# chenruduan/OAReactDiff

Hardware: AMD Instinct MI355X
Metric: denoising_steps_per_sec (higher is better)
Workload: dtype f32; 1 GPU; EGNNDynamics.forward (LEFTNet H=196 R=96 L=6), B=64 reactions/GPU x 3 objects x 23 atoms, complete graph per reaction (N=4416, E=300288), T=1000 sampler step shape; batch_per_gpu=64, atoms_per_object=23, parallelism=replica x1 (no collective), launch=eager

## Files before the change

### oareactdiff_amd/_capi.py

```python
from __future__ import annotations

import ctypes as C
import os

from .build import LIB

OARD_MAX_OBJECTS = 8
ABI_VERSION = 2040
OARD_OK, OARD_EINVAL, OARD_ENOTCOMPLETE, OARD_EHIP, OARD_ENOMEM = 0, -1, -2, -3, -4
ERRORS = {OARD_EINVAL: "invalid argument / unsupported configuration", OARD_ENOTCOMPLETE: "topology is not complete-per-sample",
          OARD_EHIP: "HIP runtime error", OARD_ENOMEM: "workspace too small"}

PREC_GCL_BF16X3, PREC_EQUI_BF16X3, PREC_TRAIN_BF16X3 = 1, 2, 4
TAP_S, TAP_VEC, TAP_EDGE, TAP_POS_FRAME, TAP_DPOS, TAP_HOUT, TAP_LABELS, TAP_NE1 = 1, 2, 3, 4, 5, 6, 7, 8

EXPORTS = ["oard_version", "oard_supported", "oard_param_count", "oard_packed_bytes", "oard_pack_weights",
           "oard_topology_create", "oard_topology_destroy", "oard_topology_num_nodes", "oard_topology_num_edges",
           "oard_topology_num_inner_edges", "oard_topology_num_samples", "oard_topology_check_edge_index",
           "oard_workspace_bytes", "oard_forward", "oard_active_inner_edges", "oard_debug_lin3u_table", "oard_sampler_step", "oard_sampler_step_dev", "oard_tap", "oard_debug_stop_after", "oard_debug_option", "oard_timing_enable", "oard_timing_reset",
           "oard_timing_get",
           "oard_topology_create_parts", "oard_topology_export", "oard_tape_bytes", "oard_tape_entry", "oard_forward_train",
           "oard_packed_bwd_bytes", "oard_pack_weights_bwd", "oard_gcl_backward_dx", "oard_edge_node_sums",
           "oard_equi_backward_dx", "oard_scalarize_backward", "oard_equi_msg_backward", "oard_lin3u_forward", "oard_lin3u_backward", "oard_wgrad_scratch_bytes", "oard_wgrad",
           "oard_train_scratch_bytes", "oard_train_scratch_poison", "oard_train_scratch_entry", "oard_train_tail_backward",
           "oard_train_layer_backward", "oard_train_init_backward", "oard_train_stage_backward",
           "oard_loss_prepare", "oard_loss_terms", "oard_adamw_step", "oard_adamw_step_dev", "oard_nan_replace",
           "oard_graph_create", "oard_graph_destroy", "oard_graph_num_nodes", "oard_graph_num_edges", "oard_graph_object_rows",
           "oard_graph_is_complete", "oard_graph_workspace_bytes", "oard_graph_forward", "oard_library_stream"]
STAGE_RECOMPUTE, STAGE_UPDATE, STAGE_MESSAGE, STAGE_GCL_NODE, STAGE_NODE_PRE, STAGE_GCL_EDGE, STAGE_EQUI_EDGE = range(7)
SCRATCH_XH, SCRATCH_XQ, SCRATCH_CR, SCRATCH_DCD, SCRATCH_DCR = range(1, 6)

TOPO_NODE_REF, TOPO_NODE_OBJ, TOPO_NODE_ROW, TOPO_NODE_SAMPLE, TOPO_NODE_TIDX, TOPO_SAMPLE_PTR, TOPO_GROUP_PTR, \
    TOPO_INNER_SRC, TOPO_INNER_TGT, TOPO_ROW_SRC, TOPO_ROW_TGT = range(1, 12)
TAPE_HIN, TAPE_GEO, TAPE_RBF, TAPE_PP0, TAPE_X1 = 1, 2, 3, 4, 5
TAPE_S_IN, TAPE_VEC_IN, TAPE_EW, TAPE_AGG, TAPE_S_MID, TAPE_Z1, TAPE_Z2, TAPE_ATT, TAPE_Z3, TAPE_ZD1, TAPE_CD, TAPE_S_A, TAPE_VEC_A = range(16, 29)


class OardConfig(C.Structure):
    _fields_ = [
        ("hidden", C.c_int32), ("num_radial", C.c_int32), ("num_layers", C.c_int32), ("in_hidden", C.c_int32),
        ("n_obj", C.c_int32), ("node_nf", C.c_int32 * OARD_MAX_OBJECTS), ("enc_alias", C.c_int32 * OARD_MAX_OBJECTS),
        ("condition_nf", C.c_int32), ("condition_time", C.c_int32), ("pos_dim", C.c_int32), ("cutoff", C.c_float),
        ("reflect_equiv", C.c_int32), ("precision", C.c_int32),
    ]


class OardError(RuntimeError):
    pass


def check(rc: int, what: str) -> None:
    if rc != OARD_OK:
        raise OardError(f"{what} failed: {ERRORS.get(rc, rc)}")


def ptr_array(tensors, n=None):
    if tensors is None:
        return None
    ptrs = [None if t is None else t.data_ptr() for t in tensors]
    return (C.c_void_p * (len(ptrs) if n is None else n))(*ptrs)


_lib = None


def lib() -> C.CDLL:
    global _lib
    if _lib is not None:
        return _lib
    if not os.path.exists(LIB):
        raise OardError(f"{LIB} not found: build it with `python -m oareactdiff_amd.build` "
                        "(there is no CPU fallback for the HIP backend)")
    L = C.CDLL(LIB)
    vp, i32, i64, sz = C.c_void_p, C.c_int32, C.c_int64, C.c_size_t
    cfgp = C.POINTER(OardConfig)
    L.oard_version.restype = C.c_int
    got = L.oard_version()
    if got != ABI_VERSION:
        raise OardError(f"{LIB} has ABI version {got}, this package expects {ABI_VERSION}: rebuild it "
                        "(`python -m oareactdiff_amd.build --force`, or the script that made the OARD_LIB build)")
    L.oard_supported.argtypes = [cfgp]; L.oard_supported.restype = C.c_int
    L.oard_param_count.argtypes = [cfgp]; L.oard_param_count.restype = sz
    L.oard_packed_bytes.argtypes = [cfgp]; L.oard_packed_bytes.restype = sz
    L.oard_pack_weights.argtypes = [cfgp, C.POINTER(vp), sz, vp, sz, vp]; L.oard_pack_weights.restype = C.c_int
    L.oard_topology_create.argtypes = [cfgp, C.POINTER(i64), C.POINTER(i64), i64, C.POINTER(vp)]
    L.oard_topology_create.restype = C.c_int
    L.oard_topology_destroy.argtypes = [vp]; L.oard_topology_destroy.restype = None
    for f in ("oard_topology_num_nodes", "oard_topology_num_edges", "oard_topology_num_inner_edges",
              "oard_topology_num_samples"):
        getattr(L, f).argtypes = [vp]; getattr(L, f).restype = i64
    L.oard_topology_check_edge_index.argtypes = [vp, vp, i64, vp, vp]; L.oard_topology_check_edge_index.restype = C.c_int
    L.oard_workspace_bytes.argtypes = [cfgp, vp]; L.oard_workspace_bytes.restype = sz
    L.oard_forward.argtypes = [cfgp, vp, vp, C.POINTER(vp), vp, C.c_int, vp, C.POINTER(vp), vp, sz, vp, vp]
    L.oard_forward.restype = C.c_int
    L.oard_debug_lin3u_table.argtypes = [cfgp, vp, C.c_int, vp, vp]; L.oard_debug_lin3u_table.restype = C.c_int
    L.oard_active_inner_edges.argtypes = [cfgp, vp, vp, sz, C.POINTER(i64), vp]; L.oard_active_inner_edges.restype = C.c_int
    L.oard_sampler_step.argtypes = [cfgp, vp, C.c_int, C.POINTER(vp), C.POINTER(vp), C.POINTER(vp), C.POINTER(vp),
                                    C.c_float, C.c_float, C.c_float, C.c_int, C.POINTER(vp), vp]
    L.oard_sampler_step.restype = C.c_int
    L.oard_sampler_step_dev.argtypes = [cfgp, vp, C.c_int, C.POINTER(vp), C.POINTER(vp), C.POINTER(vp), C.POINTER(vp), vp, C.c_int,
                                        C.POINTER(vp), vp]
    L.oard_sampler_step_dev.restype = C.c_int
    L.oard_tap.argtypes = [cfgp, vp, vp, C.c_int, C.c_int, vp, vp]; L.oard_tap.restype = C.c_int
    ci = C.c_int
    L.oard_topology_create_parts.argtypes = [cfgp, C.POINTER(i64), C.POINTER(i64), i64, ci, C.POINTER(vp)]
    L.oard_topology_create_parts.restype = ci
    L.oard_topology_export.argtypes = [vp, ci, vp, i64, vp]; L.oard_topology_export.restype = ci
    L.oard_tape_bytes.argtypes = [cfgp, vp]; L.oard_tape_bytes.restype = sz
    L.oard_tape_entry.argtypes = [cfgp, vp, ci, ci, C.POINTER(sz), C.POINTER(i64), C.POINTER(i64)]; L.oard_tape_entry.restype = ci
    L.oard_forward_train.argtypes = [cfgp, vp, vp, C.POINTER(vp), vp, ci, vp, C.POINTER(vp), vp, sz, vp, sz, vp, vp]
    L.oard_forward_train.restype = ci
    L.oard_packed_bwd_bytes.argtypes = [cfgp]; L.oard_packed_bwd_bytes.restype = sz
    L.oard_pack_weights_bwd.argtypes = [cfgp, C.POINTER(vp), sz, vp, sz, vp]; L.oard_pack_weights_bwd.restype = ci
    L.oard_gcl_backward_dx.argtypes = [cfgp, vp, vp, ci, vp, vp, vp, vp, vp, vp, vp, vp, vp]; L.oard_gcl_backward_dx.restype = ci
    L.oard_edge_node_sums.argtypes = [cfgp, vp, vp, vp, vp, vp]; L.oard_edge_node_sums.restype = ci
    L.oard_equi_backward_dx.argtypes = [cfgp, vp, vp, ci, vp, vp, vp, vp, vp]; L.oard_equi_backward_dx.restype = ci
    L.oard_scalarize_backward.argtypes = [cfgp, vp, vp, vp, vp, ci, vp, vp, vp, vp]; L.oard_scalarize_backward.restype = ci
    L.oard_equi_msg_backward.argtypes = [cfgp, vp, vp, ci, vp, vp, vp, vp, vp, vp, vp, vp, vp]; L.oard_equi_msg_backward.restype = ci
    L.oard_lin3u_forward.argtypes = [cfgp, vp, ci, vp, i64, vp, vp]; L.oard_lin3u_forward.restype = ci
    L.oard_lin3u_backward.argtypes = [cfgp, vp, ci, vp, vp, i64, vp, vp, vp, vp, vp, vp, vp]; L.oard_lin3u_backward.restype = ci
    L.oard_wgrad_scratch_bytes.argtypes = [ci, ci, i64]; L.oard_wgrad_scratch_bytes.restype = sz
    L.oard_wgrad.argtypes = [vp, ci, ci, ci, ci, ci, vp, ci, ci, ci, ci, ci, ci, i64, vp, vp, vp, sz, vp]; L.oard_wgrad.restype = ci
    pvp = C.POINTER(vp)
    L.oard_train_scratch_bytes.argtypes = [cfgp, vp]; L.oard_train_scratch_bytes.restype = sz
    L.oard_train_scratch_poison.argtypes = [cfgp, vp, vp, sz, vp]; L.oard_train_scratch_poison.restype = ci
    L.oard_train_scratch_entry.argtypes = [cfgp, vp, ci, C.POINTER(sz), C.POINTER(i64), C.POINTER(i64)]; L.oard_train_scratch_entry.restype = ci
    L.oard_train_tail_backward.argtypes = [cfgp, vp, vp, vp, vp, pvp, vp, vp, pvp, pvp, vp, sz, vp]; L.oard_train_tail_backward.restype = ci
    L.oard_train_layer_backward.argtypes = [cfgp, vp, vp, vp, vp, ci, vp, vp, vp, pvp, pvp, vp, sz, vp]; L.oard_train_layer_backward.restype = ci
    L.oard_train_init_backward.argtypes = [cfgp, vp, vp, vp, vp, pvp, vp, vp, pvp, pvp, vp, sz, vp]; L.oard_train_init_backward.restype = ci
    L.oard_train_stage_backward.argtypes = [cfgp, vp, vp, vp, vp, ci, ci, vp, vp, vp, vp, vp, vp, pvp, pvp, vp, sz, vp]
    L.oard_train_stage_backward.restype = ci
    L.oard_nan_replace.argtypes = [cfgp, vp, vp, pvp, pvp, vp]; L.oard_nan_replace.restype = ci
    pf, cf = C.POINTER(C.c_float), C.c_float
    L.oard_loss_prepare.argtypes = [cfgp, vp, pvp, pvp, pvp, pvp, vp, vp, ci, pf, pf, ci, ci, pvp, pvp, vp]; L.oard_loss_prepare.restype = ci
    L.oard_loss_terms.argtypes = [cfgp, vp, pvp, pvp, pvp, pvp, pvp, vp, vp, ci, pf, pf, pf, ci, ci, vp, vp, pvp, vp]; L.oard_loss_terms.restype = ci
    cd = C.c_double
    L.oard_adamw_step.argtypes = [vp, vp, vp, vp, vp, i64, cd, cd, cd, cd, cd, i64, ci, cd, vp]; L.oard_adamw_step.restype = ci
    L.oard_adamw_step_dev.argtypes = [vp, vp, vp, vp, vp, i64, cd, cd, cd, cd, cd, ci, ci, vp, ci, vp, vp, vp, vp]; L.oard_adamw_step_dev.restype = ci
    L.oard_library_stream.argtypes = [ci, pvp]; L.oard_library_stream.restype = ci
    L.oard_graph_create.argtypes = [cfgp, vp, vp, i64, vp, i64, pvp]; L.oard_graph_create.restype = ci
    L.oard_graph_destroy.argtypes = [vp]; L.oard_graph_destroy.restype = None
    L.oard_graph_num_nodes.argtypes = [vp]; L.oard_graph_num_nodes.restype = i64
    L.oard_graph_num_edges.argtypes = [vp]; L.oard_graph_num_edges.restype = i64
    L.oard_graph_object_rows.argtypes = [vp, ci]; L.oard_graph_object_rows.restype = i64
    L.oard_graph_is_complete.argtypes = [vp]; L.oard_graph_is_complete.restype = ci
    L.oard_graph_workspace_bytes.argtypes = [cfgp, vp]; L.oard_graph_workspace_bytes.restype = sz
    L.oard_graph_forward.argtypes = [cfgp, vp, pvp, sz, pvp, vp, ci, vp, pvp, vp, sz, vp, vp]; L.oard_graph_forward.restype = ci
    L.oard_debug_stop_after.argtypes = [C.c_int]; L.oard_debug_stop_after.restype = C.c_int
    L.oard_debug_option.argtypes = [C.c_char_p, C.c_int]; L.oard_debug_option.restype = C.c_int
    L.oard_timing_enable.argtypes = [C.c_int]; L.oard_timing_enable.restype = C.c_int
    L.oard_timing_reset.argtypes = []; L.oard_timing_reset.restype = C.c_int
    L.oard_timing_get.argtypes = [C.c_char_p, C.POINTER(C.c_double), C.POINTER(i64)]; L.oard_timing_get.restype = C.c_int
    for env, opt in (("OARD_GCL_VARIANT", b"gcl_variant"), ("OARD_EQUI_VARIANT", b"equi_variant"),
                     ("OARD_NODE_VARIANT", b"node_variant"), ("OARD_GCL_SKIP", b"gcl_skip"), ("OARD_EQUI_SKIP", b"equi_skip"), ("OARD_EQUI_L0_SKIP", b"equi_l0_skip"), ("OARD_GCL_MSUM", b"gcl_msum"), ("OARD_GCL_PERSIST", b"gcl_persist"), ("OARD_GCL_GRID", b"gcl_grid"), ("OARD_PARTS", b"parts"), ("OARD_SEQUENTIAL", b"sequential"), ("OARD_POISON", b"poison"), ("OARD_AUTO_SMALL", b"auto_small"), ("OARD_AUTO_TINY", b"auto_tiny"), ("OARD_NPB", b"npb"),
                     ("OARD_WGRAD_WGS", b"wgrad_wgs"), ("OARD_WGRAD_LDS", b"wgrad_lds"), ("OARD_WGRAD_T16", b"wgrad_t16"), ("OARD_WGRAD_QUEUE", b"wgrad_queue"), ("OARD_GATE_FOLD", b"gate_fold"), ("OARD_WGRAD_SHAPES", b"wgrad_shapes"), ("OARD_TRAIN_DUAL", b"train_dual"), ("OARD_SMALL_SPLIT", b"small_split"),
                     ("OARD_SKIP_FAMILIES", b"skip_families")):
        if os.environ.get(env) not in (None, ""):
            check(L.oard_debug_option(opt, int(os.environ[env])), f"oard_debug_option({opt.decode()})")
    _lib = L
    return L


def timing_get(family: str):
    ms, n = C.c_double(0.0), C.c_int64(0)
    check(lib().oard_timing_get(family.encode(), C.byref(ms), C.byref(n)), "oard_timing_get")
    return ms.value, n.value
```

### oareactdiff_amd/build.py

```python
from __future__ import annotations

import os
import subprocess
import sys

CSRC = os.path.join(os.path.dirname(os.path.abspath(__file__)), "csrc")
LIB = os.environ.get("OARD_LIB") or os.path.join(CSRC, "liboard_hip.so")
_EDGE = ["oard_engine.h", "oard_layout.h", "oard_kernels.h", "oard_edge_v1.h", "oard_inst.h"]
SOURCES = {
    "oard_hip.hip": None,
    "oard_general.hip": ["oard_general.h"],
    "oard_inst_gcl_p.hip": _EDGE + ["oard_edge_p.h"],
    "oard_inst_gcl_v1.hip": _EDGE + ["oard_node_v1.h", "oard_edge_small.h"],
    "oard_inst_b3.hip": _EDGE + ["oard_edge_b3.h"],
    "oard_inst_equi.hip": _EDGE + ["oard_node_v1.h", "oard_edge_bwd.h"],
    "oard_inst_wgrad.hip": _EDGE + ["oard_edge_bwd.h", "oard_wgrad_t16.h"],
    "oard_inst_node.hip": _EDGE + ["oard_node_v1.h", "oard_edge_bwd.h", "oard_node_bwd.h", "oard_rows.h"],
}
_OWNED = {"oard_general.h"}
_PUBLIC = os.path.join("..", "..", "include", "oard.h")


def _deps(src):
    own = SOURCES[src]
    hdrs = sorted(f for f in os.listdir(CSRC) if f.endswith(".h") and f not in _OWNED) if own is None else list(own)
    return [src] + hdrs + [_PUBLIC]


def _objdir():
    return os.path.join(os.path.dirname(os.path.abspath(LIB)), "build", os.path.basename(LIB))


def _obj(src):
    return os.path.join(_objdir(), os.path.splitext(src)[0] + ".o")


def _newer(paths, than):
    if not os.path.exists(than):
        return True
    t = os.path.getmtime(than)
    return any(os.path.getmtime(os.path.join(CSRC, f)) > t for f in paths)


def _stale() -> bool:
    return any(_newer(_deps(src), LIB) for src in SOURCES)


DEFAULT_DIMS = "196x96,32x8,32x32"


def dims_define(spec: str) -> str:
    pairs = []
    for item in spec.replace(" ", "").split(","):
        if not item:
            continue
        h, r = item.lower().split("x")
        h, r = int(h), int(r)
        if h % 4 or r % 4 or h < 16 or r < 4:
            raise ValueError(f"OARD_DIMS entry {item!r}: widths must be multiples of 4 (hidden >= 16)")
        if (h, r) not in pairs:
            pairs.append((h, r))
    if not pairs:
        raise ValueError("OARD_DIMS is empty")
    return "-DOARD_DIMS_LIST=" + "".join(f"X({h},{r})" for h, r in pairs)


def _dims_file() -> str:
    return LIB + ".dims"


def _built_dims() -> str:
    try:
        with open(_dims_file()) as f:
            return f.read().strip()
    except OSError:
        return ""


def build(force: bool = False, verbose: bool = False) -> str:
    dims = os.environ.get("OARD_DIMS", DEFAULT_DIMS)
    dims_define(dims)
    if not force and not _stale() and _built_dims() == dims:
        return LIB
    hipcc = os.environ.get("HIPCC", "/opt/rocm/bin/hipcc")
    if not os.path.exists(hipcc):
        hipcc = "hipcc"
    os.makedirs(_objdir(), exist_ok=True)
    flags = ["--offload-arch=gfx950", "-O3", "-std=c++17", "-fPIC", "-Wno-unused-result", dims_define(dims)]
    extra = os.environ.get("OARD_CXXFLAGS", "").split()
    tag = os.path.join(_objdir(), "flags.txt")
    flag_line = " ".join(flags + extra)
    try:
        same_flags = open(tag).read() == flag_line
    except OSError:
        same_flags = False
    todo = [src for src in SOURCES if force or not same_flags or _newer(_deps(src), _obj(src))]

    def compile_one(src):
        cmd = [hipcc] + flags + extra + ["-c", src, "-o", _obj(src)]
        if verbose:
            print(" ".join(cmd), file=sys.stderr)
        subprocess.run(cmd, cwd=CSRC, check=True)
    if todo:
        from concurrent.futures import ThreadPoolExecutor
        with ThreadPoolExecutor(max_workers=len(todo)) as pool:
            list(pool.map(compile_one, todo))
        with open(tag, "w") as f:
            f.write(flag_line)
    cmd = [hipcc, "--offload-arch=gfx950", "-shared", "-fPIC"] + [_obj(src) for src in SOURCES] + ["-o", LIB]
    if verbose:
        print(" ".join(cmd), file=sys.stderr)
    subprocess.run(cmd, cwd=CSRC, check=True)
    with open(_dims_file(), "w") as f:
        f.write(dims + "\n")
    return LIB


if __name__ == "__main__":
    print(build(force="--force" in sys.argv, verbose=True))
```

### oareactdiff_amd/csrc/oard_edge_v1.h

```cpp
#pragma once
#include "oard_kernels.h"

typedef __attribute__((address_space(3))) void* lds_ptr_t;
typedef const __attribute__((address_space(1))) void* gbl_ptr_t;
typedef int i4 __attribute__((ext_vector_type(4)));

OARD_DEV void glds16(const float* gsrc_lane, float* lds_chunk);
OARD_DEV void glds16u(const float* chunk_uniform, unsigned lane_byte_off, float* lds_chunk) {
    glds16(reinterpret_cast<const float*>(reinterpret_cast<const char*>(chunk_uniform) + lane_byte_off), lds_chunk);
}
OARD_DEV void glds16(const float* gsrc_lane, float* lds_chunk) {
#ifndef OARD_ABL_NODMA_INSTR
    __builtin_amdgcn_global_load_lds((gbl_ptr_t)gsrc_lane, (lds_ptr_t)lds_chunk, 16, 0, 0);
#else
    asm volatile("" :: "v"(gsrc_lane), "s"(lds_chunk));
#endif
}

OARD_DEV void phase_barrier() {
    asm volatile("s_waitcnt vmcnt(0)" ::: "memory");
#ifndef OARD_ABL_NOBARRIER
    __syncthreads();
#endif
}
// ... 344 lines not shown
    if (TRAIN) {
#pragma unroll
        for (int t = 0; t < HT; ++t) st_blk(tape.z1, e, D::HP, t, lane, h1[t]);
    }
#pragma unroll
    for (int t = 0; t < HT; ++t) h1[t] = silu4(h1[t]);
    const float h1_tail = TAIL1 ? tail_compact(h1[HT - 1], lane) : 0.f;

    f4 m[HT];
    f4 on[GP];
    f4 pz2[TRAIN ? GP : 1];
    float m_tail = 0.f;
#pragma unroll
    for (int p2 = 0; p2 < S::NP2; ++p2, ++p) {
        auto post = [&]() {
            TL(1);
            if (TRAIN && p2 > 0) {
#pragma unroll
                for (int gg = 0; gg < GP; ++gg)
                    if ((p2 - 1) * GP + gg < HT) st_blk(tape.z2, e, D::HP, (p2 - 1) * GP + gg, lane, pz2[gg]);
            }
            pf_begin(p + DIST);
            if (DO_S3 && p2 == S::NP2 - 1) {
#pragma unroll
                for (int gg = 0; gg < GP; ++gg)
                    on[gg] = gg < WB ? (DO_S1 ? ld_edge(erow + 16 * gg) : ld_f4(c0 + 16 * gg + 4 * g)) : f4zero();
            }
        };
        auto hook = [&]() { if (RING == 3 && bar_left > 0 && --bar_left == 0) { PHASE_BARRIER(); post(); } pf.tick(); };
        if (RING == 2) { PHASE_BARRIER(); post(); } else bar_left = BAR_AT;
#pragma unroll
        for (int gg = 0; gg < GP; ++gg) {
            const int tg = p2 * GP + gg;
            if (tg < S::NG2) {
                const f4 bias = A(p, gg * G2);
                TL(2);
                f4 acc;
                if (ROWS4 && tg >= HT - 1) {
                    acc = reduce_g(tg < HT ? chain_tile4<HT>(SL(p), gg * G2 + 1, h1, bias, hook)
                                           : chain_tile4<HT>(SL(p), gg * G2 + 1, m, bias, hook));
                    if (tg < HT && g != 0) acc = f4zero();
                } else {
                    acc = tg < HT ? chain_tile<HT, TAIL1>(SL(p), gg * G2 + 1, h1, bias, h1_tail, hook)
                                  : chain_tile<HT, TAIL1>(SL(p), gg * G2 + 1, m, bias, m_tail, hook);
                }
                TL(3);
                if (tg < HT) {
                    if (TRAIN) pz2[gg] = acc;
                    m[tg] = silu4(acc);
                    if (TAIL1 && tg == HT - 1) m_tail = tail_compact(m[HT - 1], lane);
                } else {
                    const float a = ROWS4 ? acc.x : __shfl(acc.x, lane & 15, 64);
                    if (TRAIN && g == 0) tape.att[e] = a;
                    const float gate = silu1(a);
#pragma unroll
                    for (int t = 0; t < HT; ++t) m[t] *= gate;
                    m_tail *= gate;
                }
            }
        }
        TL(4);
        if (RING == 3 && bar_left > 0) { bar_left = 0; PHASE_BARRIER(); post(); }
        pf.flush();
    }
    if (TRAIN) {
#pragma unroll
        for (int gg = 0; gg < GP; ++gg)
            if ((S::NP2 - 1) * GP + gg < HT) st_blk(tape.z2, e, D::HP, (S::NP2 - 1) * GP + gg, lane, pz2[gg]);
    }
    if (!DO_S3) {
        if (MSUM) st_msum<D>(mbuf, c, key, m, lane);
        else {
#pragma unroll
            for (int t = 0; t < HT; ++t) st_blk(mbuf, eid, D::HP, t, lane, m[t]);
        }
        PROBE_END(pf);
        TL_END();
        return;
    }
    f4 pend[GP], pendz[TRAIN ? GP : 1];
    f4 om[GP];
    auto s3_phase = [&](int p3, const f4 (&o)[GP], f4 (&onext)[GP]) {
        auto post = [&]() {
            TL(1);
            if (p3 == 0) {
                if (!MSUM) {
#pragma unroll
                    for (int t = 0; t < HT; ++t) st_blk(mbuf, eid, D::HP, t, lane, m[t]);
                }
            } else {
#pragma unroll
                for (int gg = 0; gg < GP; ++gg) {
                    st_f4(orow + 16 * ((p3 - 1) * GP + gg), pend[gg]);
                    if (TRAIN) st_f4(tape.z3 + e * D::WP + 4 * g + 16 * ((p3 - 1) * GP + gg), pendz[gg]);
                }
            }
            pf_begin(p + DIST);
            if (p3 + 1 < S::NP3) {
#pragma unroll
                for (int gg = 0; gg < GP; ++gg) {
                    const int t = (p3 + 1) * GP + gg;
                    if (t < WB)
                        onext[gg] = DO_S1 ? ld_edge(erow + 16 * t) : ld_f4(c0 + 16 * t + 4 * g);
                }
            }
        };
        auto hook = [&]() { if (RING == 3 && bar_left > 0 && --bar_left == 0) { PHASE_BARRIER(); post(); } pf.tick(); };
        if (RING == 2) { PHASE_BARRIER(); post(); } else bar_left = BAR_AT;
#pragma unroll
        for (int gg = 0; gg < GP; ++gg) {
            const int t = p3 * GP + gg;
            if (t < WB) {
                TL(2);
                const f4 z = chain_tile<HT, TAIL1>(SL(p), gg * G2 + 1, m, A(p, gg * G2), m_tail, hook);
                TL(3);
                if (TRAIN) pendz[gg] = z;
                pend[gg] = o[gg] + silu4(z);
            }
        }
        TL(4);
        if (RING == 3 && bar_left > 0) { bar_left = 0; PHASE_BARRIER(); post(); }
        if (MSUM && p3 == 0) st_msum<D>(mbuf, c, key, m, lane);
        pf.flush();
        ++p;
    };
    {
        int p3 = 0;
        for (; p3 + 1 < S::NP3; p3 += 2) { s3_phase(p3, on, om); s3_phase(p3 + 1, om, on); }
        if (p3 < S::NP3) s3_phase(p3, on, om);
    }
#pragma unroll
    for (int gg = 0; gg < GP; ++gg) {
        const int t = (S::NP3 - 1) * GP + gg;
        if (t < WB) {
            st_f4(orow + 16 * t, pend[gg]);
            if (TRAIN) st_f4(tape.z3 + e * D::WP + 4 * g + 16 * t, pendz[gg]);
        }
    }
    PROBE_END(pf);
    TL_END();
}

template <class D>
struct EquiStream {
    static constexpr int WB = D::WB, D1T = D::D1T, RB = D::RB, HT = D::HT;
    static constexpr int G1 = D1T, G2 = 1 + D1T + RB, NG2 = 3 * HT;
    static constexpr bool ROWS4 = (D::H % 16) >= 1 && (D::H % 16) <= 4;
    static constexpr int SLAB = G2 > G1 ? G2 : G1;
    static constexpr int NPH = WB + NG2;
    static constexpr int C1 = WB * G1, CHUNKS = C1 + NG2 * G2;
    static constexpr size_t LDS_BYTES = (size_t)2 * SLAB * 1024;
};

template <class D, int WAVES, bool TRAIN>
__global__ __launch_bounds__(WAVES * 64) void k_equi_edge_v1(TopoDev tp, const float* __restrict__ stream,
                                                             const float* __restrict__ dp0b,
                                                             const float* __restrict__ ew, const float* __restrict__ rbuf,
                                                             float* __restrict__ qbuf, float* __restrict__ zd1,
                                                             float* __restrict__ cdbuf, ActList al, int skip_mid) {
    extern __shared__ __attribute__((aligned(16))) float smem[];
    using S = EquiStream<D>;
    constexpr int WB = D::WB, D1T = D::D1T, RB = D::RB, HT = D::HT, G1 = S::G1, G2 = S::G2;
    const int lane = threadIdx.x & 63, g = lane >> 4;
    const int wave = __builtin_amdgcn_readfirstlane(threadIdx.x >> 6);

    SlabPrefetch<WAVES, S::SLAB, 0, 3> pf;
    pf.wave = wave;
    pf.lane_off = (unsigned)lane * 16u;
    const bool skip = !TRAIN && skip_mid != 0;
    auto pf_begin = [&](int ph) {
        pf.begin(stream, smem, ph, ph * G1, G1);
    };
    auto pf_begin_t2 = [&](int ph, int slot) {
        pf.begin(stream, smem, ph, S::C1 + slot * G2, slot < S::NG2 ? G2 : 0);
    };
    auto next_slot = [&](int i) -> int { return i + ((skip && i % 3 == 0) ? 2 : 1); };
    auto hook = [&]() { pf.tick(); };
    auto A = [&](int p, int j) -> f4 {
        return *reinterpret_cast<const f4*>(smem + ((size_t)(p & 1) * S::SLAB + j) * 256 + lane * 4);
    };
    auto SL = [&](int p) -> const float* { return smem + (size_t)(p & 1) * S::SLAB * 256 + lane * 4; };

    const long long n_cols = al.n != nullptr ? (long long)*al.n : tp.A;
    if ((long long)blockIdx.x * WAVES * 16 >= n_cols) return;
    const long long c = ((long long)blockIdx.x * WAVES + wave) * 16 + (lane & 15);
    const bool live = c < n_cols;
    const size_t a = (size_t)(live ? (al.rows != nullptr ? (long long)al.rows[c] : c) : tp.A);
    const float* erow = ew + (live ? a : (size_t)tp.E) * D::WP + 4 * g;
    f4 d1[D1T];
#pragma unroll
    for (int t = 0; t < D1T; ++t) d1[t] = ld_vec(dp0b, t, lane);
    f4 rb[RB];
#pragma unroll
    for (int b = 0; b < RB; ++b) rb[b] = ld_blk(rbuf, a, D::RP, b, lane);
    f4 xn = ld_f4(erow);
    pf_begin(0);
    pf.flush();

    int p = 0;
    for (int b = 0; b < WB; ++b, ++p) {
        phase_barrier();
        const f4 x = xn;
        if (b + 1 < WB) pf_begin(p + 1); else pf_begin_t2(p + 1, 0);
        if (b + 1 < WB) xn = ld_f4(erow + 16 * (b + 1));
        chain_kouter<D1T>(SL(p), 0, x, d1, hook);
        pf.flush();
    }
    if (TRAIN) {
#pragma unroll
        for (int t = 0; t < D1T; ++t) st_blk(zd1, a, D::D1P, t, lane, d1[t]);
    }
#pragma unroll
    for (int t = 0; t < D1T; ++t) d1[t] = silu4(d1[t]);

    float* qrow = qbuf + a * (size_t)(3 * D::HP) + 4 * g;
    float* cdrow = TRAIN ? cdbuf + a * (size_t)(3 * D::HP) + 4 * g : nullptr;
    f4 pend = f4zero(), pendc = f4zero();
    int pend_off = 0;
    auto t2_phase = [&](int i, auto rows4) {
        phase_barrier();
        if (i > 0) {
            st_f4(qrow + pend_off, pend);
            if (TRAIN) st_f4(cdrow + pend_off, pendc);
        }
        pf_begin_t2(p + 1, next_slot(i));
        const int tt = i / 3, th = i - 3 * tt;
        f4 cd, cr;
        if (decltype(rows4)::value) {
            cd = reduce_g(chain_tile4<D1T>(SL(p), 1, d1, A(p, 0), hook));
            cr = reduce_g(chain_tile4<RB>(SL(p), 1 + D1T, rb, f4zero(), hook));
            if (g != 0) { cd = f4zero(); cr = f4zero(); }
        } else {
            cd = chain_tile<D1T>(SL(p), 1, d1, A(p, 0), hook);
            cr = chain_tile<RB>(SL(p), 1 + D1T, rb, f4zero(), hook);
        }
        pf.flush();
        pend = cd * cr;
        if (TRAIN) pendc = cd;
        pend_off = th * D::HP + 16 * tt;
        ++p;
    };
    constexpr int N_FULL = S::ROWS4 ? S::NG2 - 3 : S::NG2;
    for (int i = 0; i < N_FULL; i = next_slot(i)) t2_phase(i, std::false_type{});
    for (int i = N_FULL; i < S::NG2; i = next_slot(i)) t2_phase(i, std::true_type{});
    st_f4(qrow + pend_off, pend);
    if (TRAIN) st_f4(cdrow + pend_off, pendc);
}

template <class D>
__global__ __launch_bounds__(256) void k_equi_agg_v1(TopoDev tp, const float* __restrict__ wb, LayerOff lo,
                                                     const float* __restrict__ qbuf, const float* __restrict__ xq,
                                                     const float* __restrict__ geo, const float* __restrict__ x1,
                                                     float* __restrict__ s, const float* __restrict__ vec_in,
                                                     float* __restrict__ vec_out, float* __restrict__ v2buf,
                                                     float* __restrict__ scal, float* __restrict__ vdot) {
    bool live; const ColId id = col_id(tp.N, live);
    if (!live) return;
    const int n = id.col, a0 = tp.act_ptr[n], cnt = tp.act_ptr[n + 1] - a0;
    const int mx = wave_max(cnt);
    const float inv_sqrt2 = 0.70710678118654752f, inv_sqrt3 = 0.57735026918962576f,
                inv_sqrt_h = 1.0f / sqrtf((float)D::H);
    f4 vx[3][D::HT], dx[D::HT];
#pragma unroll
    for (int t = 0; t < D::HT; ++t) { dx[t] = f4zero(); vx[0][t] = f4zero(); vx[1][t] = f4zero(); vx[2][t] = f4zero(); }
    for (int k = 0; k < mx; ++k)
        if (k < cnt) {
            const size_t a = (size_t)a0 + k;
            const int m = tp.act_src[a];
            const float* g = geo + a * GEO_STRIDE;
            const float ux = g[2], uy = g[3], uz = g[4];
            const float xc = lo.xcross ? 1.0f : 0.0f, cx = xc * g[5], cy = xc * g[6], cz = xc * g[7];
#pragma unroll
            for (int t = 0; t < D::HT; ++t) {
                const f4 q0 = ld_blk(qbuf, a, 3 * D::HP, t, id.lane);
                const f4 q1 = ld_blk(qbuf, a, 3 * D::HP, D::HT + t, id.lane);
                const f4 q2 = ld_blk(qbuf, a, 3 * D::HP, 2 * D::HT + t, id.lane);
                const f4 xs0 = ld_blk(xq, m, 3 * D::HP, t, id.lane) + ld_blk(xq, n, 3 * D::HP, t, id.lane);
                const f4 xs1 = ld_blk(xq, m, 3 * D::HP, D::HT + t, id.lane) + ld_blk(xq, n, 3 * D::HP, D::HT + t, id.lane);
                const f4 xs2 = ld_blk(xq, m, 3 * D::HP, 2 * D::HT + t, id.lane) + ld_blk(xq, n, 3 * D::HP, 2 * D::HT + t, id.lane);
                const f4 xm = xs0 * q0;
                dx[t] += xm;
                const f4 a2 = xs1 * q1 * inv_sqrt3, a3 = xs2 * q2;
                vx[0][t] += (ld_blk(vec_in, (size_t)m * 3 + 0, D::HP, t, id.lane) * a2 + a3 * ux + xm * cx) * inv_sqrt_h;
                vx[1][t] += (ld_blk(vec_in, (size_t)m * 3 + 1, D::HP, t, id.lane) * a2 + a3 * uy + xm * cy) * inv_sqrt_h;
                vx[2][t] += (ld_blk(vec_in, (size_t)m * 3 + 2, D::HP, t, id.lane) * a2 + a3 * uz + xm * cz) * inv_sqrt_h;
            }
        }
#pragma unroll
    for (int t = 0; t < D::HT; ++t) {
        const f4 sn = (ld_blk(s, n, D::HP, t, id.lane) + dx[t]) * inv_sqrt2;
        if (id.valid) st_blk(s, n, D::HP, t, id.lane, sn);
#pragma unroll
        for (int x = 0; x < 3; ++x) {
            vx[x][t] += ld_blk(vec_in, (size_t)n * 3 + x, D::HP, t, id.lane);
            if (id.valid) st_blk(vec_out, (size_t)n * 3 + x, D::HP, t, id.lane, vx[x][t]);
        }
    }
    const float fx = x1[n * 3], fy = x1[n * 3 + 1], fz = x1[n * 3 + 2];
    const float* l3 = wb + lo.l3u;
    for (int t = 0; t < D::HT; ++t) {
        f4 v1[3] = {f4zero(), f4zero(), f4zero()}, v2[3] = {f4zero(), f4zero(), f4zero()};
        const float* w1 = wb + lo.vp + ((size_t)t * D::HT * 64 + id.lane) * 4;
        const float* w2 = wb + lo.vp + ((size_t)(D::HT + t) * D::HT * 64 + id.lane) * 4;
#pragma unroll
        for (int b = 0; b < D::HT; ++b) {
            const f4 c1 = ld_f4(w1 + (size_t)b * 256), c2 = ld_f4(w2 + (size_t)b * 256);
#pragma unroll
            for (int x = 0; x < 3; ++x) {
                v1[x] = mma_chunk(c1, vx[x][b], v1[x]);
                v2[x] = mma_chunk(c2, vx[x][b], v2[x]);
            }
        }
        const f4 sc = v1[0] * fx + v1[1] * fy + v1[2] * fz;
        const f4 vd = (v1[0] * v2[0] + v1[1] * v2[1] + v1[2] * v2[2]) * inv_sqrt_h;
        f4 sca;
        const int f0 = 16 * t + 4 * id.g;
        sca.x = f0 + 0 < D::H ? lin3u(l3, sc.x) : 0.f;
        sca.y = f0 + 1 < D::H ? lin3u(l3, sc.y) : 0.f;
        sca.z = f0 + 2 < D::H ? lin3u(l3, sc.z) : 0.f;
        sca.w = f0 + 3 < D::H ? lin3u(l3, sc.w) : 0.f;
        if (id.valid) {
            st_blk(scal, n, D::HP, t, id.lane, sca);
            st_blk(vdot, n, D::HP, t, id.lane, vd);
            st_blk(v2buf, (size_t)n * 3 + 0, D::HP, t, id.lane, v2[0]);
            st_blk(v2buf, (size_t)n * 3 + 1, D::HP, t, id.lane, v2[1]);
            st_blk(v2buf, (size_t)n * 3 + 2, D::HP, t, id.lane, v2[2]);
        }
    }
}
```

### oareactdiff_amd/csrc/oard_hip.hip

```cpp
#include <algorithm>
#include <cmath>
#include <cstdio>
#include <cstring>
#include <map>
#include <string>
#include <vector>
#include <mutex>
#include <chrono>
#include <utility>

#include "oard_kernels.h"
#include "oard_edge_v1.h"
#include "oard_edge_p.h"
#include "oard_wgrad_t16.h"
#include "oard_edge_b3.h"
#ifdef OARD_EXPERIMENTS
#include "oard_edge_fp.h"
#endif
#include "oard_node_v1.h"
#include "oard_edge_small.h"
#include "oard_edge_bwd.h"
#include "oard_node_bwd.h"
#include "oard_rows.h"
#include "oard_plan.h"
#include "oard_inst.h"

#define OARD_VERSION 2040
#ifdef OARD_EXPERIMENTS
static constexpr bool kV0 = true;
#else
static constexpr bool kV0 = false;
#endif

#define HIP_TRY(x) do { hipError_t e_ = (x); if (e_ != hipSuccess) { \
    fprintf(stderr, "liboard_hip: %s failed: %s (%s:%d)\n", #x, hipGetErrorString(e_), __FILE__, __LINE__); \
    return OARD_EHIP; } } while (0)

namespace {
enum Family { F_GCL_EDGE = 0, F_EQUI_EDGE, F_NODE, F_INIT, F_OTHER, F_GCL_BWD, F_EQUI_BWD, F_WGRAD, F_COUNT };
const char* kFamilyNames[F_COUNT] = {"gcl_edge", "equi_edge", "node", "init", "other", "gcl_edge_bwd", "equi_edge_bwd", "wgrad"};
struct TimingRec { hipEvent_t a, b; int fam; };
struct Timing {
    bool on = false;
    std::vector<TimingRec> recs;
    std::vector<hipEvent_t> pool;
    double total_ms[F_COUNT] = {0};
    long long launches[F_COUNT] = {0};
    hipEvent_t get() {
        if (!pool.empty()) { hipEvent_t e = pool.back(); pool.pop_back(); return e; }
        hipEvent_t e; (void)hipEventCreate(&e); return e;
    }
    void flush() {
        for (auto& r : recs) {
            (void)hipEventSynchronize(r.b);
            float ms = 0.f;
            (void)hipEventElapsedTime(&ms, r.a, r.b);
            total_ms[r.fam] += ms; launches[r.fam] += 1;
            pool.push_back(r.a); pool.push_back(r.b);
        }
        recs.clear();
    }
} g_timing;
int g_stop_after = 0;
FwdOptions g_fwd;
int g_sequential = 0;
int g_npb = 0;
int g_poison = 0;
int g_gcl_msum_taken = 0;
int g_equi_l0_taken = 0;
int g_parts = 0;
int g_wgrad_shapes = 3;
int g_wgrad_t16 = 256;
int g_wgrad_lds = 256;
int g_wgrad_wgs = 512;
int g_skip_families = 0;

struct ScopedLaunch {
    hipStream_t st; hipEvent_t a; int fam; bool on;
    ScopedLaunch(int f, hipStream_t s) : st(s), fam(f), on(g_timing.on) {
        if (on) { a = g_timing.get(); (void)hipEventRecord(a, st); }
    }
    ~ScopedLaunch() {
        if (on) { hipEvent_t b = g_timing.get(); (void)hipEventRecord(b, st); g_timing.recs.push_back({a, b, fam}); }
    }
};
#define LAUNCH(fam, kern, grid, block, stream, ...) do { ScopedLaunch sl_(fam, stream); if (!((g_skip_families >> (fam)) & 1)) \
    hipLaunchKernelGGL(kern, dim3((unsigned)(grid)), dim3(block), 0, stream, __VA_ARGS__); } while (0)
#define LAUNCH2(fam, kern, gx, gy, block, stream, ...) do { ScopedLaunch sl_(fam, stream); if (!((g_skip_families >> (fam)) & 1)) \
    hipLaunchKernelGGL(kern, dim3((unsigned)(gx), (unsigned)(gy)), dim3(block), 0, stream, __VA_ARGS__); } while (0)

#ifndef OARD_DIMS_LIST
#define OARD_DIMS_LIST X(196, 96) X(32, 8) X(32, 32)
#endif

inline size_t align_up(size_t x, size_t a) { return (x + a - 1) / a * a; }
inline long long cdiv(long long a, long long b) { return (a + b - 1) / b; }

bool config_ok(const oard_config* c) {
    if (!c) return false;
    bool dims = false;
#define X(h, r) dims = dims || (c->hidden == (h) && c->num_radial == (r));
    OARD_DIMS_LIST
#undef X
    if (!dims) return false;
    if (c->num_layers < 1 || c->num_layers > OARD_MAX_LAYERS) return false;
    if (c->in_hidden < 1 || c->in_hidden > 16) return false;
    if (c->n_obj < 1 || c->n_obj > OARD_MAX_OBJECTS) return false;
    if (c->pos_dim != 3 || (c->reflect_equiv != 0 && c->reflect_equiv != 1)) return false;
    if (c->precision & ~(OARD_PREC_GCL_BF16X3 | OARD_PREC_EQUI_BF16X3 | OARD_PREC_TRAIN_BF16X3)) return false;
    const int emb = c->in_hidden - (c->condition_time ? 1 : 0) - (c->condition_nf > 0 ? c->condition_nf : 0);
    if (emb < 1) return false;
    for (int k = 0; k < c->n_obj; ++k) {
        const int d = c->node_nf[k] - 3;
        if (d < 1 || d > 16) return false;
        const int a = c->enc_alias[k];
        if (a < 0 || a >= c->n_obj || c->node_nf[a] != c->node_nf[k]) return false;
    }
    return true;
}
int embed_dim(const oard_config* c) {
    return c->in_hidden - (c->condition_time ? 1 : 0) - (c->condition_nf > 0 ? c->condition_nf : 0);
}

PackOff make_layout(const oard_config* c) {
    const RDims d(c->hidden, c->num_radial);
    PackOff po;
    memset(&po, 0, sizeof(po));
    size_t cur = 0;
    auto take = [&](size_t n) { size_t o = cur; cur = align_up(cur + n, 64); return o; };
    auto mat = [&](int MT, int KB) { return take((size_t)MT * KB * 256); };
    const int emb = embed_dim(c);
    po.emb = mat(d.HT, 1); po.emb_b = take(d.HP);
    po.nbemb = mat(d.HT, 1); po.nbemb_b = take(d.HP);
    po.s2v = mat(d.HT, d.HT); po.s2v_b = take(d.HP);
    po.rl0 = mat(d.HT, d.RB); po.rl0_b = take(d.HP);
    po.rl2 = mat(d.HT, d.HT); po.rl2_b = take(d.HP);
    po.lin3 = take((size_t)d.H4 * 5 + 1);
    po.pe0 = take((size_t)d.H2 * 3);
    po.pe1 = mat(d.HT, d.PB);
    po.embout = mat(1, d.HT); po.embout_b = take(16);
    po.v1p = mat(d.HT, d.HT); po.v2p = take(d.HP);
    po.un0 = mat(d.HT, 2 * d.HT); po.un0_b = take(d.HP);
    po.un2 = mat(1, d.HT); po.un2_b = take(16);
    po.c0row = take(d.WP);
    po.u0 = take(d.HP);
    po.rbf_means = take(d.RP); po.rbf_betas = take(d.RP);
    for (int k = 0; k < c->n_obj; ++k) {
        const int dd = c->node_nf[k] - 3;
        po.enc[k] = take((size_t)2 * dd * dd + 2 * dd + (size_t)emb * 2 * dd + emb);
        po.dec[k] = take((size_t)2 * dd * emb + 2 * dd + (size_t)dd * 2 * dd + dd);
    }
    for (int l = 0; l < c->num_layers; ++l) {
        LayerOff& lo = po.layer[l];
        lo.ln_g_w = take(d.HP); lo.ln_g_b = take(d.HP);
        lo.W1a = mat(d.HT, d.HT); lo.b1 = take(d.HP);
        lo.W1b = mat(d.HT, d.HT);
        lo.W1c = mat(d.HT, d.WB);
        lo.W2 = mat(d.HT, d.HT); lo.b2 = take(d.HP);
        lo.watt = take(d.HP); lo.batt = take(1);
        lo.W3 = mat(d.WB, d.HT); lo.b3 = take(d.WP);
        lo.nm0 = mat(d.HT, 2 * d.HT); lo.nm0b = take(d.HP);
        lo.nm1 = mat(d.HT, d.HT); lo.nm1b = take(d.HP);
        lo.ln_q_w = take(d.HP); lo.ln_q_b = take(d.HP);
        lo.xp0 = mat(d.HT, d.HT);
        lo.xp2 = mat(3 * d.HT, d.HT);
        lo.dp0 = mat(d.D1T, d.WB); lo.dp0b = take(d.D1P);
        lo.dp2 = mat(3 * d.HT, d.D1T); lo.dp2b = take(3 * d.HP);
        lo.rbfp = mat(3 * d.HT, d.RB);
        lo.vp = mat(2 * d.HT, d.HT);
        lo.xv0 = mat(d.HT, 2 * d.HT);
        lo.xv2 = mat(3 * d.HT, d.HT);
        lo.l3u = take(593);
        lo.l3t = take(L3T_FLOATS);
        lo.gcl_stream = take((size_t)(d.WB * d.HT + (d.HT + 1) * (d.HT + 1) + d.WB * (d.HT + 1)) * 256);
        lo.equi_stream = take((size_t)(d.WB * d.D1T + 3 * d.HT * (1 + d.D1T + d.RB)) * 256);
        {
            const int nbh = (d.HT + 1) / 2, nbw = (d.WB + 1) / 2;
            lo.gcl_b3 = take((size_t)(nbw * 3 * d.HT + (d.HT + 1) * (1 + 3 * nbh) + d.WB * (1 + 3 * nbh)) * 256);
            lo.equi_b3 = take((size_t)(nbw * 3 * d.D1T + ((d.RB + 1) / 2 + (d.D1T + 1) / 2) * 9 * d.HT) * 256);
        }
    }
    po.total = cur;
    po.signed_scal = c->reflect_equiv ? 0 : 1;
    for (int l = 0; l < c->num_layers; ++l) po.layer[l].xcross = c->reflect_equiv ? 0 : 1;
    return po;
}

struct ParamIdx {
    int emb_w, emb_b, embout_w, embout_b, means, betas, nbemb_w, nbemb_b, s2v_w, s2v_b, rl0_w, rl0_b, rl2_w, rl2_b,
        lin30_w, lin30_b, lin32_w, lin32_b, pe0_w, pe1_w;
    int gcl0, msg0, upd0, out0, enc0, dec0, count;
    explicit ParamIdx(const oard_config* c) {
        int i = 0;
        emb_w = i++; emb_b = i++; embout_w = i++; embout_b = i++; means = i++; betas = i++;
        nbemb_w = i++; nbemb_b = i++; s2v_w = i++; s2v_b = i++; rl0_w = i++; rl0_b = i++; rl2_w = i++; rl2_b = i++;
        lin30_w = i++; lin30_b = i++; lin32_w = i++; lin32_b = i++; pe0_w = i++; pe1_w = i++;
        i += 2;
        gcl0 = i; i += 14 * c->num_layers;
        msg0 = i; i += 9 * c->num_layers;
        upd0 = i; i += 9 * c->num_layers;
        i += 2;
        out0 = i; i += 6;
        enc0 = i; i += 4 * c->n_obj;
        dec0 = i; i += 4 * c->n_obj;
        count = i;
    }
};

struct Packer {
    const float* const* p; float* blob; hipStream_t st;
    std::vector<GenJob> jobs;
    long long blocks = 0;
    void push(GenJob j, size_t work) {
        j.block0 = blocks;
        blocks += cdiv((long long)std::max<size_t>(work, 1), 256);
        jobs.push_back(j);
    }
    void matrix(int src, int src_ld, int col_off, int msl, int msp, int ms, int ksl, int ksp, int ks, int MT, int KB,
                size_t dst, size_t tstride = 0, size_t bstride = 256, int perm_ht = 0, int transpose = 0, int tail_compact = 0,
                int rows4 = 0) {
        if (tstride == 0) tstride = (size_t)KB * 256;
        GenJob j;
        memset(&j, 0, sizeof(j));
        j.type = 0;
        j.m = PackJob{p[src], src_ld, col_off, msl, msp, ms, ksl, ksp, ks, MT, KB, dst, tstride, bstride, perm_ht, transpose, rows4, tail_compact};
        push(j, (size_t)MT * KB * 256);
    }
    void nat(int src, int src_ld, int col_off, int M, int K, int MT, int KB, size_t dst) {
        matrix(src, src_ld, col_off, M, MT * 16, 1, K, KB * 16, 1, MT, KB, dst);
    }
    void vec(int src, int sect_len, int sect_pad, int sects, int n_dst, size_t dst) {
        GenJob j;
        memset(&j, 0, sizeof(j));
        j.type = 1; j.src = src >= 0 ? p[src] : nullptr; j.dst = dst; j.sect_len = sect_len; j.sect_pad = sect_pad; j.sects = sects; j.n = n_dst;
        push(j, (size_t)n_dst);
    }
    void bias_chunks(int src, int sect_len, int sect_pad, int sects, int n_tiles, size_t dst, size_t tstride,
                     int perm_ht = 0) {
        GenJob j;
        memset(&j, 0, sizeof(j));
        j.type = 2; j.src = p[src]; j.dst = dst; j.sect_len = sect_len; j.sect_pad = sect_pad; j.sects = sects; j.n = n_tiles * 256;
        j.tstride = tstride; j.perm_ht = perm_ht;
        push(j, (size_t)n_tiles * 256);
    }
    void raw(int src, int n, size_t dst) {
        GenJob j;
        memset(&j, 0, sizeof(j));
        j.type = 3; j.src = p[src]; j.dst = dst; j.n = n;
        push(j, (size_t)n);
    }
    int flush() {
        if (jobs.empty()) return OARD_OK;
        struct Cached { std::vector<GenJob> host; GenJob* dev = nullptr; size_t cap = 0; };
        static std::mutex mu;
        static std::map<std::pair<const void*, int>, Cached> cache;
        int devid = 0;
        (void)hipGetDevice(&devid);
        const GenJob* table = nullptr;
        {
            std::lock_guard<std::mutex> lk(mu);
            Cached& c = cache[{(const void*)blob, devid}];
            const bool same = c.host.size() == jobs.size() && memcmp(c.host.data(), jobs.data(), jobs.size() * sizeof(GenJob)) == 0;
            if (!same) {
                HIP_TRY(hipStreamSynchronize(st));
                if (c.cap < jobs.size()) {
                    if (c.dev) (void)hipFree(c.dev);
                    HIP_TRY(hipMalloc((void**)&c.dev, jobs.size() * sizeof(GenJob)));
                    c.cap = jobs.size();
                }
                HIP_TRY(hipMemcpy(c.dev, jobs.data(), jobs.size() * sizeof(GenJob), hipMemcpyHostToDevice));
                c.host = jobs;
            }
            table = c.dev;
        }
        hipLaunchKernelGGL(k_pack_all, dim3((unsigned)blocks), dim3(256), 0, st, table, (int)jobs.size(), blob);
        jobs.clear();
        blocks = 0;
        return OARD_OK;
    }
};
#define OARD_SMALL_MAX_EDGES (512 * 16 * 16)
static WsOff make_ws(const oard_config* c, const TopoDev& td) {
    const RDims d(c->hidden, c->num_radial);
    const size_t N = td.N, E = td.E + 1, A = td.A + 1;
    WsOff w;
    size_t cur = 0;
    auto take = [&](size_t bytes) { size_t o = cur; cur = align_up(cur + bytes, 256); return o; };
    w.pos = take(N * 3 * 4); w.pf64 = take(N * 3 * 8); w.pf32 = take(N * 3 * 4); w.x1 = take(N * 3 * 4);
    w.pp0 = take(N * 4); w.labels = take(N * 4); w.hin = take(N * 16 * 4);
    w.zemb = take(N * d.HP * 4); w.nb = take(N * d.HP * 4); w.s = take(N * d.HP * 4); w.s1 = take(N * d.HP * 4);
    w.ne1 = take(N * 3 * d.HP * 4); w.xh = take(N * d.HP * 4); w.P = take(N * d.HP * 4); w.Q = take(N * d.HP * 4);
    w.xq = take(N * 3 * d.HP * 4); w.vec = take(N * 3 * d.HP * 4); w.vec2 = take(N * 3 * d.HP * 4); w.v2buf = take(N * 3 * d.HP * 4);
    w.sc0 = take(N * d.HP * 4); w.vdot = take(N * d.HP * 4);
    w.geo = take(A * GEO_STRIDE * 4); w.d64 = take(A * 8); w.rbuf = take(A * d.RP * 4);
    w.ew = take(E * d.WP * 4); w.mbuf = take(std::max(E, (size_t)(td.CI + td.CX) + 1) * d.HP * 4);
    w.xmsg = take(A * d.HP * 4); w.vmsg = take(A * 3 * d.HP * 4);
    w.dpos = take(N * 3 * 4); w.hout = take(N * 16 * 4);
    w.al_rows = take(A * 4); w.al_src = take(A * 4); w.al_pre = take(A * 4); w.al_cnt = take((size_t)cdiv((long long)td.A, 256) * 4 + 4); w.al_n = take(4);
    w.d1s = take((size_t)cdiv((long long)td.A, 128) * 8 * d.D1T * 1024);
    w.small_a = E <= (size_t)OARD_SMALL_MAX_EDGES ? take(A * d.D1P * 4) : 0;
    w.total = cur;
    return w;
}



template <class K>
int set_lds(K kernel, size_t bytes) {
    HIP_TRY(hipFuncSetAttribute((const void*)kernel, hipFuncAttributeMaxDynamicSharedMemorySize, (int)bytes));
    return OARD_OK;
}

#define LAUNCH_LDS(fam, kern, grid, block, lds, stream, ...) do { \
    static bool attr_done_[64] = {}; \
    int dev_ = 0; (void)hipGetDevice(&dev_); dev_ &= 63; \
    if (!attr_done_[dev_]) { int rc_ = set_lds(kern, lds); if (rc_ != OARD_OK) return rc_; attr_done_[dev_] = true; } \
    ScopedLaunch sl_(fam, stream); if (!((g_skip_families >> (fam)) & 1)) \
    hipLaunchKernelGGL(kern, dim3((unsigned)(grid)), dim3(block), lds, stream, __VA_ARGS__); } while (0)

static int device_cus() {
    static int cus[64] = {};
    int d = 0;
    (void)hipGetDevice(&d);
    d &= 63;
    if (!cus[d]) {
        int n = 0;
        if (hipDeviceGetAttribute(&n, hipDeviceAttributeMultiprocessorCount, d) != hipSuccess || n < 1) { (void)hipGetLastError(); n = 256; }
        cus[d] = n;
    }
    return cus[d];
}
struct GclArgs {
    const TopoDev& tp; const float* wb; const LayerOff& lo;
    const float *stream, *P, *Q, *u0, *c0; float *ew_in, *ew_out, *mbuf;
    GclTape tape; hipStream_t st;
};
template <class D, bool S1, bool S3>
int launch_gcl_v1s(const GclLaunch& L, bool msum, const GclArgs& a) {
    constexpr size_t RING3 = GclStream<D, 2>::LDS_BYTES / 2 * 3;
#define GCL_STREAMED(kern, waves, lds, w_) do { LAUNCH_LDS(F_GCL_EDGE, kern, L.grid, (waves) * 64, lds, a.st, a.tp, w_, a.P, a.Q, a.u0, a.c0, \
                                                           L.r0, L.r1, a.ew_in, a.ew_out, a.mbuf, a.tape); return OARD_OK; } while (0)
    switch ((int)L.shape) {
        case GCL_PERSIST:
            if (msum) GCL_STREAMED((k_gcl_edge_p<D, S1, S3, false, true>), 8, RING3, a.stream);
            GCL_STREAMED((k_gcl_edge_p<D, S1, S3>), 8, RING3, a.stream);
        case GCL_RING3:
            if (msum) GCL_STREAMED((k_gcl_edge_v1<D, 8, 2, S1, S3, false, true, 2, 3>), 8, RING3, a.stream);
            GCL_STREAMED((k_gcl_edge_v1<D, 8, 2, S1, S3, false, false, 2, 3>), 8, RING3, a.stream);
        case GCL_TRAIN_PERSIST: GCL_STREAMED((k_gcl_edge_p<D, S1, S3, true>), 8, RING3, a.stream);
        case GCL_TRAIN_RING3: GCL_STREAMED((k_gcl_edge_v1<D, 8, 2, S1, S3, true, false, 2, 3>), 8, RING3, a.stream);
        case GCL_B3: GCL_STREAMED((k_gcl_edge_b3<D, S1, S3>), 8, (GclB3Stream<D>::LDS_BYTES), a.wb + a.lo.gcl_b3);
        case GCL_TRAIN_B3: GCL_STREAMED((k_gcl_edge_b3<D, S1, S3, true>), 8, (GclB3Stream<D>::LDS_BYTES), a.wb + a.lo.gcl_b3);
        case GCL_W4: GCL_STREAMED((k_gcl_edge_v1<D, 4, 2, S1, S3, false>), 4, (GclStream<D, 2>::LDS_BYTES), a.stream);
        case GCL_SMALL:
            LAUNCH_LDS(F_GCL_EDGE, (k_gcl_edge_small<D, 8, S1, S3>), L.grid, 512, (GclSmall<D>::LDS_BYTES), a.st,
                       a.tp, a.wb, a.lo, a.P, a.Q, a.u0, a.c0, L.r0, L.r1, a.ew_out, a.mbuf);
            return OARD_OK;
#ifdef OARD_EXPERIMENTS
        case GCL_V0: LAUNCH(F_GCL_EDGE, (k_gcl_edge<D>), L.grid, 256, a.st, a.tp, a.wb, a.lo, a.P, a.Q, a.ew_in, a.mbuf); return OARD_OK;
        case GCL_X0 + 7: GCL_STREAMED((k_gcl_edge_v1<D, 8, 2, S1, S3, false>), 8, (GclStream<D, 2>::LDS_BYTES), a.stream);
        case GCL_X0 + 8: GCL_STREAMED((k_gcl_edge_v1<D, 8, 3, S1, S3, false>), 8, (GclStream<D, 3>::LDS_BYTES), a.stream);
        case GCL_X0 + 9: GCL_STREAMED((k_gcl_edge_v1<D, 8, 4, S1, S3, false>), 8, (GclStream<D, 4>::LDS_BYTES), a.stream);
        case GCL_X0 + 4: GCL_STREAMED((k_gcl_edge_fp<D, 8, 2, S1, S3, false>), 8, (GclRing<D, 2, 4>::LDS_BYTES), a.stream);
        case GCL_X0 + 5: GCL_STREAMED((k_gcl_edge_fp<D, 8, 2, S1, S3, false, 3>), 8, (GclRing<D, 2, 3>::LDS_BYTES), a.stream);
        case GCL_X0 + 10: GCL_STREAMED((k_gcl_edge_v1<D, 12, 1, S1, S3, false, false, 3>), 12, (GclStream<D, 1>::LDS_BYTES), a.stream);
        case GCL_X0 + 11: GCL_STREAMED((k_gcl_edge_v1<D, 12, 2, S1, S3, false, false, 3>), 12, (GclStream<D, 2>::LDS_BYTES), a.stream);
        case GCL_X0 + 12: GCL_STREAMED((k_gcl_edge_v1<D, 4, 1, S1, S3, false, false, 3>), 4, (GclStream<D, 1>::LDS_BYTES), a.stream);
#endif
        default: return OARD_EINVAL;
    }
#undef GCL_STREAMED
}
template <class D>
int launch_gcl_v1(const GclLayer& g, bool msum, const GclArgs& a) {
    for (int i = 0; i < g.n; ++i) {
        const GclLaunch& L = g.l[i];
        const int rc = L.s1 ? (L.s3 ? launch_gcl_v1s<D, true, true>(L, msum, a) : launch_gcl_v1s<D, true, false>(L, msum, a))
                            : (L.s3 ? launch_gcl_v1s<D, false, true>(L, msum, a) : launch_gcl_v1s<D, false, false>(L, msum, a));
        if (rc != OARD_OK) return rc;
    }
    return OARD_OK;
}
template <class D>
int launch_equi_v1(const FwdPlan& plan, int l, const TopoDev& tp, const float* wb, const LayerOff& lo, const float* stream, const float* dp0b,
                   const float* ew, const float* rbuf, float* qbuf, float* zd1, float* cd, hipStream_t st, float* d1s, float* small, ActList al) {
    const long long tiles = cdiv(tp.A, 16);
    switch (plan.equi) {
        case EQ_TRAIN_B3:
            LAUNCH_LDS(F_EQUI_EDGE, (k_equi_edge_b3<D, true>), cdiv(tp.A, 16 * 8), 8 * 64, (EquiB3Stream<D>::LDS_BYTES), st, tp, wb + lo.equi_b3,
                       dp0b, wb + lo.dp2b, ew, rbuf, qbuf, d1s, zd1, cd, ActList{});
            return OARD_OK;
        case EQ_TRAIN:
            LAUNCH_LDS(F_EQUI_EDGE, (k_equi_edge_v1<D, 8, true>), cdiv(tp.A, 16 * 8), 8 * 64, (EquiStream<D>::LDS_BYTES), st,
                       tp, stream, dp0b, ew, rbuf, qbuf, zd1, cd, ActList{}, 0);
            return OARD_OK;
        case EQ_SMALL_SPLIT:
            LAUNCH_LDS(F_EQUI_EDGE, (k_equi_small_s1<D, 8>), tiles * cdiv(D::D1T, 8), 512, (size_t)D::WB * 1024, st, tp, wb, lo, ew, small);
            LAUNCH_LDS(F_EQUI_EDGE, (k_equi_small_s2<D, 8>), tiles * cdiv(3 * D::HT, 8), 512, (size_t)(D::D1T + D::RB) * 1024, st,
                       tp, wb, lo, (const float*)small, rbuf, qbuf);
            return OARD_OK;
        case EQ_SMALL:
            LAUNCH_LDS(F_EQUI_EDGE, (k_equi_edge_small<D, 8>), tiles, 512, (EquiSmall<D>::LDS_BYTES), st, tp, wb, lo, ew, rbuf, qbuf);
            return OARD_OK;
        case EQ_B3:
            LAUNCH_LDS(F_EQUI_EDGE, (k_equi_edge_b3<D>), cdiv(tp.A, 16 * 8), 8 * 64, (EquiB3Stream<D>::LDS_BYTES), st, tp, wb + lo.equi_b3,
                       dp0b, wb + lo.dp2b, ew, rbuf, qbuf, d1s, nullptr, nullptr, al);
            return OARD_OK;
        case EQ_W4:
            LAUNCH_LDS(F_EQUI_EDGE, (k_equi_edge_v1<D, 4, false>), cdiv(tp.A, 16 * 4), 4 * 64, (EquiStream<D>::LDS_BYTES), st,
                       tp, stream, dp0b, ew, rbuf, qbuf, nullptr, nullptr, al, 0);
            return OARD_OK;
        case EQ_W8:
            LAUNCH_LDS(F_EQUI_EDGE, (k_equi_edge_v1<D, 8, false>), cdiv(tp.A, 16 * 8), 8 * 64, (EquiStream<D>::LDS_BYTES), st,
                       tp, stream, dp0b, ew, rbuf, qbuf, nullptr, nullptr, al, plan.l0_skip && l == 0 ? 1 : 0);
            return OARD_OK;
        default: return OARD_EINVAL;
    }
}

struct TapeOff {
    size_t hin, geo, rbuf, pp0, x1;
    size_t s_in[OARD_MAX_LAYERS + 1], vec_in[OARD_MAX_LAYERS + 1];
    size_t agg[OARD_MAX_LAYERS], s_mid[OARD_MAX_LAYERS];
    size_t s_a[OARD_MAX_LAYERS], vec_a[OARD_MAX_LAYERS];
    size_t ew[OARD_MAX_LAYERS + 1];
    size_t z1[OARD_MAX_LAYERS], z2[OARD_MAX_LAYERS], att[OARD_MAX_LAYERS], z3[OARD_MAX_LAYERS];
    size_t zd1[OARD_MAX_LAYERS], cd[OARD_MAX_LAYERS];
    size_t total;
};
static TapeOff make_tape(const oard_config* c, const TopoDev& td) {
    const RDims d(c->hidden, c->num_radial);
    const size_t N = td.N, E = td.E + 1, A = td.A + 1;
    TapeOff t;
    memset(&t, 0, sizeof(t));
    size_t cur = 0;
    auto take = [&](size_t bytes) { size_t o = cur; cur = align_up(cur + bytes, 256); return o; };
    t.hin = take(N * 16 * 4); t.geo = take(A * GEO_STRIDE * 4); t.rbuf = take(A * d.RP * 4); t.pp0 = take(N * 4); t.x1 = take(N * 3 * 4);
    for (int l = 0; l <= c->num_layers; ++l) {
        t.s_in[l] = take(N * d.HP * 4); t.vec_in[l] = take(N * 3 * d.HP * 4); t.ew[l] = take(E * d.WP * 4);
        if (l == c->num_layers) break;
        t.agg[l] = take(N * d.HP * 4); t.s_mid[l] = take(N * d.HP * 4);
        t.s_a[l] = take(N * d.HP * 4); t.vec_a[l] = take(N * 3 * d.HP * 4);
        t.z1[l] = take(E * d.HP * 4); t.z2[l] = take(E * d.HP * 4); t.att[l] = take(E * 4); t.z3[l] = take(E * d.WP * 4);
        t.zd1[l] = take(A * d.D1P * 4); t.cd[l] = take(A * 3 * d.HP * 4);
    }
    t.total = cur;
    return t;
}

template <class D>
static int forward_impl(const FwdOptions& opt, const oard_config* c, const TopoPart* topo, const float* wb, const float* const* xh,
                        const float* t, int t_scalar, const float* cond, float* const* out, char* ws, char* tape,
                        int* status, hipStream_t st) {
    const TopoDev& tp = topo->d;
    const PackOff po = make_layout(c);
    const WsOff w = make_ws(c, tp);
    const bool train = tape != nullptr;
    const TapeOff to = train ? make_tape(c, tp) : TapeOff{};
    const int emb = embed_dim(c);
    float* pos = (float*)(ws + w.pos); double* pf64 = (double*)(ws + w.pf64); float* pf32 = (float*)(ws + w.pf32);
    auto slot = [&](size_t ws_off, size_t tape_off) -> float* { return train ? (float*)(tape + tape_off) : (float*)(ws + ws_off); };
    float* x1 = slot(w.x1, to.x1); float* pp0 = slot(w.pp0, to.pp0); int* labels = (int*)(ws + w.labels);
    float* hin = slot(w.hin, to.hin); float* zemb = (float*)(ws + w.zemb); float* nb = (float*)(ws + w.nb);
    float* s = (float*)(ws + w.s); float* s1 = (float*)(ws + w.s1); float* ne1 = (float*)(ws + w.ne1);
    float* xhb = (float*)(ws + w.xh); float* P = (float*)(ws + w.P); float* Q = (float*)(ws + w.Q);
    float* xq = (float*)(ws + w.xq); float* vec = slot(w.vec, to.vec_in[0]); float* v2buf = (float*)(ws + w.v2buf);
    float* scal = (float*)(ws + w.sc0); float* vdot = (float*)(ws + w.vdot);
    float* geo = slot(w.geo, to.geo); double* d64 = (double*)(ws + w.d64); float* rbuf = slot(w.rbuf, to.rbuf);
    float* mbuf = (float*)(ws + w.mbuf); float* xmsg = (float*)(ws + w.xmsg);
    float* vmsg = (float*)(ws + w.vmsg); float* dpos = (float*)(ws + w.dpos); float* hout = (float*)(ws + w.hout);
    auto ew_at = [&](int l) -> float* { return train ? (float*)(tape + to.ew[l]) : (float*)(ws + w.ew); };
    float* ew = ew_at(0);
    auto s_at = [&](int l) -> float* { return train ? (float*)(tape + to.s_in[l]) : s; };
    auto s_mid_at = [&](int l) -> float* { return train ? (float*)(tape + to.s_mid[l]) : s; };

    ObjPtrs op;
    memset(&op, 0, sizeof(op));
    for (int k = 0; k < c->n_obj; ++k) {
        op.xh[k] = xh[k]; op.out[k] = out[k]; op.node_nf[k] = c->node_nf[k]; op.enc[k] = po.enc[k]; op.dec[k] = po.dec[k];
    }
    const long long N = tp.N, E = tp.E, A = tp.A;
    const unsigned gN = (unsigned)cdiv(N, 64), gA = (unsigned)cdiv(A, 64);
    const double cutoff = (double)c->cutoff;
    const FwdPlan plan = make_fwd_plan({opt, c->precision, train, topo->conc, tp.npb, device_cus(), A, E, tp.CI, tp.CX, c->num_layers, w.small_a != 0});
    const bool msum = plan.msum, use_al = plan.use_al, nv1 = plan.node != NODE_V0;
    const int stop_after = train ? 0 : g_stop_after;
    int* al_cnt = (int*)(ws + w.al_cnt);
    const ActList al = use_al ? ActList{(const int*)(ws + w.al_rows), (const int*)(ws + w.al_src), (const int*)(ws + w.al_pre), (const int*)(ws + w.al_n)}
                              : ActList{nullptr, nullptr, nullptr, nullptr};
    if (!use_al) HIP_TRY(hipMemsetAsync(ws + w.al_n, 0xff, sizeof(int), st));
    LAUNCH(F_OTHER, k_prep, cdiv(N, 128), 128, st, tp, op, wb, pos, hin, t, t_scalar, cond,
           c->condition_nf > 0 ? c->condition_nf : 0, c->condition_time, emb);
    LAUNCH(F_INIT, k_geom, tp.n_groups, 64, st, tp, (const float*)pos, cutoff, pf64, pf32, x1, pp0, labels);
    if (plan.fill_edges || stop_after == 1)
        LAUNCH(F_INIT, k_fill_edges, std::min<long long>(cdiv((E - A + 1) * (D::WP / 4), 256), 8192), 256, st,
               wb + po.c0row, ew + (size_t)A * D::WP, E - A + 1, D::WP);
    if (A > 0) {
        LAUNCH(F_INIT, k_edge_geo, cdiv(A, 256), 256, st, tp, (const float*)pos, (const double*)pf64, cutoff, geo, d64, use_al ? al_cnt : nullptr);
        if (use_al) LAUNCH(F_INIT, k_active_list, cdiv(A, 256), 256, st, tp, (const float*)geo, (const int*)al_cnt, (int*)al.rows, (int*)al.src, (int*)al.pre, (int*)al.n);
        LAUNCH(F_INIT, k_rbf, cdiv(A * D::RP, 256), 256, st, tp, (const double*)d64, (const float*)geo,
               wb + po.rbf_means, wb + po.rbf_betas, cutoff, rbuf, ew, D::R, D::RP, D::H, D::WP);
    }
    LAUNCH(F_INIT, (k_node_embed<D>), gN, 256, st, tp, wb, po, (const float*)hin, zemb, nb);
    if (A > 0) LAUNCH(F_INIT, (k_radial_lin<D>), gA, 256, st, tp, wb, po, (const float*)rbuf, (const float*)geo, ew);
    constexpr int NW = D::HT <= 16 ? D::HT : 8;
    const unsigned gNb = (unsigned)cdiv(N, tp.npb);
    if (plan.init_v1) {
        LAUNCH(F_INIT, (k_neighbor_v1<D, NW>), gNb, NW * 64, st, tp, wb, po, (const float*)zemb, (const float*)nb, (const float*)ew, s_at(0), s1);
        LAUNCH(F_INIT, (k_s2v_agg_v1<D, NW>), gNb, NW * 64, st, tp, (const float*)s1, (const float*)ew, (const float*)geo, ne1);
    } else if constexpr (kV0) {
        LAUNCH(F_INIT, (k_neighbor<D>), gN, 256, st, tp, wb, po, (const float*)zemb, (const float*)nb, (const float*)ew, s_at(0), s1);
        LAUNCH(F_INIT, (k_s2v_agg<D>), gN, 256, st, tp, (const float*)s1, (const float*)ew, (const float*)geo, ne1);
    } else return OARD_EINVAL;
    if (A > 0) LAUNCH2(F_INIT, (k_scalarize<D>), gA, (plan.scalarize_tiles ? D::HT : 1), 256, st, tp, wb, po, (const float*)ne1, (const float*)geo, ew);
    HIP_TRY(hipMemsetAsync(vec, 0, (size_t)N * 3 * D::HP * sizeof(float), st));
    if (stop_after == 1) return OARD_OK;

    float* vec2 = (float*)(ws + w.vec2);
    float* vcur = vec;
    float* vnext = vec2;
    g_gcl_msum_taken = msum;
    for (int l = 0; l < c->num_layers; ++l) {
        const LayerOff lo = po.layer[l];
        const unsigned gN16 = (unsigned)cdiv(N, tp.npb);
        float* ew_in = ew_at(l);
        float* ew_out = ew_at(l + 1);
        if (train) vnext = (float*)(tape + to.vec_in[l + 1]);

        if (nv1) LAUNCH(F_NODE, (k_node_pre_v1<D, NW>), gN16, NW * 64, st, tp, wb, po, lo, (const float*)s_at(l), (const float*)pp0, xhb, P, Q);
        else if constexpr (kV0) LAUNCH(F_NODE, (k_node_pre<D>), gN, 256, st, tp, wb, po, lo, (const float*)s, (const float*)pp0, xhb, P, Q);
        else return OARD_EINVAL;
        GclTape gt{};
        if (train) gt = GclTape{(float*)(tape + to.z1[l]), (float*)(tape + to.z2[l]), (float*)(tape + to.att[l]), (float*)(tape + to.z3[l])};
        int rc = launch_gcl_v1<D>(plan.gcl_at(l), msum, GclArgs{tp, wb, lo, wb + lo.gcl_stream, P, Q, wb + po.u0, wb + po.c0row, ew_in, ew_out, mbuf, gt, st});
        if (rc != OARD_OK) return rc;
        const bool rows = plan.node == NODE_ROWS;
        if (nv1 && rows) LAUNCH(F_NODE, (k_gcl_node_v1<D, NW, true>), gN16, NW * 64, st, tp, wb, lo, (const float*)xhb, (const float*)mbuf, s_mid_at(l), xq,
                                train ? (float*)(tape + to.agg[l]) : nullptr);
        else if (nv1 && msum) LAUNCH(F_NODE, (k_gcl_node_v1<D, NW, false, true>), gN16, NW * 64, st, tp, wb, lo, (const float*)xhb, (const float*)mbuf, s_mid_at(l), xq,
                                     (float*)nullptr);
        else if (nv1) LAUNCH(F_NODE, (k_gcl_node_v1<D, NW, false>), gN16, NW * 64, st, tp, wb, lo, (const float*)xhb, (const float*)mbuf, s_mid_at(l), xq,
                             train ? (float*)(tape + to.agg[l]) : nullptr);
        else if constexpr (kV0) LAUNCH(F_NODE, (k_gcl_node<D>), gN, 256, st, tp, wb, lo, (const float*)xhb, (const float*)mbuf, s, xq);
        else return OARD_EINVAL;
        if (stop_after == 100 + 10 * l + 1) { topo->vec_final = (size_t)((char*)vcur - ws); return OARD_OK; }
        if (plan.equi == EQ_V0) {
            if constexpr (kV0) {
                if (A > 0) LAUNCH(F_EQUI_EDGE, (k_equi_edge<D>), gA, 256, st, tp, wb, lo, (const float*)ew_out, (const float*)rbuf,
                                  (const float*)geo, (const float*)xq, (const float*)vcur, xmsg, vmsg);
                LAUNCH(F_NODE, (k_equi_agg<D>), gN, 256, st, tp, wb, lo, (const float*)xmsg, (const float*)vmsg, (const float*)x1,
                       s, vcur, v2buf, scal, vdot);
            } else return OARD_EINVAL;
        } else {
            const bool l0_skip = l == 0 && plan.l0_skip;
            if (l == 0) g_equi_l0_taken = l0_skip;
            if (A > 0) {
                rc = launch_equi_v1<D>(plan, l, tp, wb, lo, wb + lo.equi_stream, wb + lo.dp0b, ew_out, rbuf, vmsg,
                                       train ? (float*)(tape + to.zd1[l]) : nullptr, train ? (float*)(tape + to.cd[l]) : nullptr, st,
                                       (float*)(ws + w.d1s), (float*)(ws + w.small_a), al);
                if (rc != OARD_OK) return rc;
            }
#define EQUI_NODE_V1(D_, ROWS_, XC_) LAUNCH(F_NODE, (k_equi_node_v1<D_, NW, ROWS_, XC_>), gN16, NW * 64, st, tp, wb, lo, (const float*)vmsg, \
                       (const float*)xq, (const float*)geo, (const float*)x1, (const float*)s_mid_at(l), s_at(l + 1), (const float*)vcur, vnext, \
                       train ? (float*)(tape + to.s_a[l]) : nullptr, train ? (float*)(tape + to.vec_a[l]) : nullptr, al)
            if (nv1 && rows) {
                if (lo.xcross) EQUI_NODE_V1(D, true, true); else EQUI_NODE_V1(D, true, false);
            } else if (nv1 && l0_skip) {
                if (lo.xcross) EQUI_NODE_V1(Layer0<D>, false, true); else EQUI_NODE_V1(Layer0<D>, false, false);
            } else if (nv1) {
                if (lo.xcross) EQUI_NODE_V1(D, false, true); else EQUI_NODE_V1(D, false, false);
            } else if constexpr (kV0) {
                LAUNCH(F_NODE, (k_equi_agg_v1<D>), gN, 256, st, tp, wb, lo, (const float*)vmsg, (const float*)xq,
                       (const float*)geo, (const float*)x1, s, (const float*)vcur, vnext, v2buf, scal, vdot);
            } else return OARD_EINVAL;
            std::swap(vcur, vnext);
        }
        if constexpr (kV0) {
            if (!nv1) LAUNCH(F_NODE, (k_equi_upd<D>), gN, 256, st, tp, wb, lo, (const float*)scal, (const float*)vdot,
                             (const float*)v2buf, s, vcur);
        }
        if (stop_after == 100 + 10 * l + 2) { topo->vec_final = (size_t)((char*)vcur - ws); return OARD_OK; }
    }
    if (!train) topo->vec_final = (size_t)((char*)vcur - ws);
    if (train) {
        ZeroRows z;
        z.count = 0;
        auto add = [&](size_t off, size_t row, int ld) {
            if (z.count == 64) { LAUNCH(F_OTHER, k_zero_rows, 64, 256, st, z); z.count = 0; }
            z.p[z.count] = (float*)(tape + off) + row * (size_t)ld; z.n[z.count] = ld; ++z.count;
        };
        for (int l = 0; l <= c->num_layers; ++l) {
            add(to.ew[l], (size_t)E, D::WP);
            if (l == c->num_layers) break;
            add(to.z1[l], (size_t)E, D::HP); add(to.z2[l], (size_t)E, D::HP); add(to.att[l], (size_t)E, 1); add(to.z3[l], (size_t)E, D::WP);
            add(to.zd1[l], (size_t)A, D::D1P); add(to.cd[l], (size_t)A, 3 * D::HP);
        }
        add(to.geo, (size_t)A, GEO_STRIDE); add(to.rbuf, (size_t)A, D::RP);
        if (z.count > 0) LAUNCH(F_OTHER, k_zero_rows, z.count, 256, st, z);
    }
    if (plan.init_v1)
        LAUNCH(F_NODE, (k_out_v1<D, NW>), gNb, NW * 64, st, tp, wb, po, (const float*)s_at(c->num_layers), (const float*)vcur, dpos, hout, status);
    else if constexpr (kV0)
        LAUNCH(F_NODE, (k_out<D>), gN, 256, st, tp, wb, po, (const float*)s, (const float*)vcur, dpos, hout, status);
    else return OARD_EINVAL;
    LAUNCH(F_OTHER, k_post, cdiv(N, 128), 128, st, tp, op, wb, (const float*)dpos, (const float*)hout, emb);
    HIP_TRY(hipGetLastError());
    return OARD_OK;
}

template <class F> static int dispatch_dims(const oard_config* c, F&& f) {
#define X(h, r) if (c->hidden == (h) && c->num_radial == (r)) { f(Dims<(h), (r)>{}); return 0; }
    OARD_DIMS_LIST
#undef X
    return OARD_EINVAL;
}
#define DISPATCH_DIMS(c, CALL)                                                                         \
    do {                                                                                               \
        if (dispatch_dims((c), [&](auto d_) { using D = decltype(d_); CALL; }) != 0) return OARD_EINVAL; \
    } while (0)

struct BwdLayerOff { size_t gcl, equi, watt; };
struct BwdOff { BwdLayerOff layer[OARD_MAX_LAYERS]; size_t total; };
static BwdOff make_bwd_layout(const oard_config* c) {
    const RDims d(c->hidden, c->num_radial);
    BwdOff b;
    memset(&b, 0, sizeof(b));
    size_t cur = 0;
    auto take = [&](size_t n) { size_t o = cur; cur = align_up(cur + n, 64); return o; };
    for (int l = 0; l < c->num_layers; ++l) {
        b.layer[l].gcl = take((size_t)(2 * d.WB * d.HT + d.HT * d.HT) * 256);
        b.layer[l].equi = take((size_t)(3 * d.HT * d.D1T + d.WB * d.D1T) * 256);
        b.layer[l].watt = take(d.HP);
    }
    b.total = cur;
    return b;
}
template <class D>
static int gcl_backward_impl(const oard_config* c, const TopoDev& tp, const float* pb, const BwdLayerOff& bl, int layer,
                             const char* tape, const TapeOff& to, const float* dagg, float* dew, float* dz3, float* mout,
                             float* dz2, float* da, float* dz1, hipStream_t st, float* gate_part = nullptr, long long* gate_rows = nullptr) {
    GclBwdArgs a;
    a.gate_part = gate_part;
    a.z1 = (const float*)(tape + to.z1[layer]); a.z2 = (const float*)(tape + to.z2[layer]);
    a.att = (const float*)(tape + to.att[layer]); a.z3 = (const float*)(tape + to.z3[layer]);
    a.dagg = dagg; a.watt = pb + bl.watt; a.dew = dew; a.dz3 = dz3; a.mout = mout; a.dz2 = dz2; a.da = da; a.dz1 = dz1;
    const float* stream = pb + bl.gcl;
    const bool last = layer == c->num_layers - 1;
    const long long r_full = last ? tp.A : tp.E;
    long long rows = 0;
    if (r_full > 0) {
        LAUNCH_LDS(F_GCL_BWD, (k_gcl_edge_bwd<D, 8, 2, true>), cdiv(r_full, 128), 512, (GclBwdStream<D, 2>::LDS_BYTES), st,
                   tp, stream, 0LL, r_full, a);
        rows += cdiv(r_full, 128) * 8;
    }
    if (last && tp.E > tp.A) {
        if (a.gate_part) a.gate_part += (size_t)rows * D::HP;
        LAUNCH_LDS(F_GCL_BWD, (k_gcl_edge_bwd<D, 8, 2, false>), cdiv(tp.E - tp.A, 128), 512, (GclBwdStream<D, 2>::LDS_BYTES), st,
                   tp, stream, tp.A, tp.E, a);
        rows += cdiv(tp.E - tp.A, 128) * 8;
    }
    if (gate_rows) *gate_rows = rows;
    HIP_TRY(hipGetLastError());
    return OARD_OK;
}

template <class D>
static int equi_backward_impl(const TopoDev& tp, const float* stream, const float* dcd, const float* zd1, float* dew,
                              float* dzd1, hipStream_t st) {
    LAUNCH_LDS(F_EQUI_BWD, (k_equi_edge_bwd<D, 8>), cdiv(tp.A, 128), 512, (EquiBwdStream<D>::LDS_BYTES), st, tp, stream, dcd,
               zd1, dew, dzd1);
    HIP_TRY(hipGetLastError());
    return OARD_OK;
}

#ifndef OARD_SCAL_BWD_WAVES
#define OARD_SCAL_BWD_WAVES 2
#endif
template <class D>
static int scalarize_backward_impl(const oard_config* c, const TopoDev& tp, const float* wb, const char* tape, const TapeOff& to,
                                   const float* ne1, int ld, const float* dew, float* dne1, float* part, hipStream_t st) {
    const PackOff po = make_layout(c);
    constexpr int NW = OARD_SCAL_BWD_WAVES;
    if (po.signed_scal)
        LAUNCH(F_INIT, (k_scalarize_bwd<D, NW, true>), tp.N, NW * 64, st, tp, wb + po.lin3, ne1, ld, (const float*)(tape + to.geo), dew, dne1, part);
    else
        LAUNCH(F_INIT, (k_scalarize_bwd<D, NW, false>), tp.N, NW * 64, st, tp, wb + po.lin3, ne1, ld, (const float*)(tape + to.geo), dew, dne1, part);
    HIP_TRY(hipGetLastError());
    return OARD_OK;
}

template <class D>
static int equi_msg_backward_impl(const oard_config* c, const TopoDev& tp, const char* tape, const TapeOff& to, int layer, const float* xq, const float* cr,
                                  const float* gs, const float* gv, float* dcd, float* dcr, float* dxq, float* dvec, hipStream_t st) {
    const Strided3 xq3{xq, 3 * D::H, D::H}, vec3{(const float*)(tape + to.vec_in[layer]), 3 * D::HP, D::HP}, cr3{cr, 3 * D::H, D::H},
        gv3{gv, 3 * D::H, D::H};
    LAUNCH(F_NODE, (k_equi_msg_bwd<D>), tp.N, 256, st, tp, (const float*)(tape + to.geo), xq3, vec3, (const float*)(tape + to.cd[layer]), cr3,
           gs, D::H, gv3, dcd, dcr, dxq, dvec, D::H, c->reflect_equiv ? 0 : 1);
    HIP_TRY(hipGetLastError());
    return OARD_OK;
}

struct WgradPlan { int transposed, NT, nPB, nQG, PP, QP, gy; long long rpc; int n_chunks; int lds, PBW, QGW; };
struct WglShape { int NT, PBW, QGW; };
static const WglShape kWglShapes[2] = {{7, 4, 2}, {8, 4, 2}};
static WgradPlan wgrad_plan(int ncY, int ncX, long long rows) {
    WgradPlan p;
    p.transposed = ncX > ncY ? 1 : 0;
    const int ncP = p.transposed ? ncX : ncY, ncQ = p.transposed ? ncY : ncX;
    const int nQT = (int)cdiv(ncQ, 16);
    p.NT = (cdiv(nQT, 7) * 7 <= cdiv(nQT, 8) * 8) ? 7 : 8;
    p.nPB = (int)cdiv(ncP, 64); p.nQG = (int)cdiv(nQT, p.NT);
    p.PP = p.nPB * 64; p.QP = p.nQG * p.NT * 16;
// ... 232 lines not shown
}

struct TablePool {
    struct Free { void* p; size_t cap; };
    struct Pending { void* p; size_t cap; hipEvent_t ev[4]; int n_ev; int kind; };
    std::mutex m;
    std::vector<Free> free_[2];
    std::vector<Pending> pending;
    std::vector<hipEvent_t> spare_events;
};
static TablePool& table_pool() {
    static TablePool pools[64];
    int d = 0;
    (void)hipGetDevice(&d);
    return pools[d & 63];
}
static void pool_raw_free(void* p, int kind) { if (kind == 0) (void)hipFree(p); else (void)hipHostFree(p); }
static void pool_collect(TablePool& tp) {
    for (size_t i = 0; i < tp.pending.size();) {
        TablePool::Pending& q = tp.pending[i];
        bool done = true;
        for (int k = 0; k < q.n_ev && done; ++k) done = hipEventQuery(q.ev[k]) == hipSuccess;
        if (!done) { ++i; continue; }
        for (int k = 0; k < q.n_ev; ++k) tp.spare_events.push_back(q.ev[k]);
        tp.free_[q.kind].push_back({q.p, q.cap});
        tp.pending[i] = tp.pending.back();
        tp.pending.pop_back();
    }
    (void)hipGetLastError();
}
static void* pool_alloc(size_t bytes, size_t* cap, int kind = 0) {
    TablePool& tp = table_pool();
    std::lock_guard<std::mutex> lk(tp.m);
    pool_collect(tp);
    std::vector<TablePool::Free>& fl = tp.free_[kind];
    int best = -1;
    for (int i = 0; i < (int)fl.size(); ++i)
        if (fl[i].cap >= bytes && fl[i].cap <= 2 * bytes + (1u << 20) && (best < 0 || fl[i].cap < fl[best].cap)) best = i;
    if (best >= 0) {
        void* p = fl[best].p;
        *cap = fl[best].cap;
        fl[best] = fl.back();
        fl.pop_back();
        return p;
    }
    while (fl.size() > 16) {
        pool_raw_free(fl.front().p, kind);
        fl.erase(fl.begin());
    }
    void* p = nullptr;
    *cap = align_up(bytes + bytes / 8, (size_t)1 << 16);
    const hipError_t e = kind == 0 ? hipMalloc(&p, *cap) : hipHostMalloc(&p, *cap, hipHostMallocDefault);
    if (e != hipSuccess) { (void)hipGetLastError(); return nullptr; }
    return p;
}
static void pool_release(void* p, size_t cap, const hipStream_t* streams, int n_streams, bool sync_device, int kind = 0) {
    if (!p) return;
    TablePool& tp = table_pool();
    std::lock_guard<std::mutex> lk(tp.m);
    if (sync_device) { (void)hipDeviceSynchronize(); tp.free_[kind].push_back({p, cap}); return; }
    TablePool::Pending q{p, cap, {}, 0, kind};
    hipStream_t all[5] = {device_streams()[2]};
    int n = 1;
    for (int k = 0; k < n_streams && k < 4; ++k) if (streams[k] != all[0]) all[n++] = streams[k];
    for (int k = 0; k < n && q.n_ev < 4; ++k) {
        hipEvent_t e = nullptr;
        if (!tp.spare_events.empty()) { e = tp.spare_events.back(); tp.spare_events.pop_back(); }
        else if (hipEventCreateWithFlags(&e, hipEventDisableTiming) != hipSuccess) { (void)hipDeviceSynchronize(); tp.free_[kind].push_back({p, cap}); return; }
        (void)hipEventRecord(e, all[k]);
        q.ev[q.n_ev++] = e;
    }
    if (n > 4) { (void)hipDeviceSynchronize(); }
    tp.pending.push_back(q);
}
struct UploadItem { const void* src; size_t bytes; size_t off; };
static int pool_upload(void* dev, const std::vector<UploadItem>& items, size_t total, void** stage_out, size_t* stage_cap) {
    char* stage = (char*)pool_alloc(total, stage_cap, 1);
    if (!stage) return OARD_EHIP;
    for (const UploadItem& it : items) memcpy(stage + it.off, it.src, it.bytes);
    if (hipMemcpyAsync(dev, stage, total, hipMemcpyHostToDevice, device_streams()[2]) != hipSuccess) {
        (void)hipGetLastError();
        pool_release(stage, *stage_cap, nullptr, 0, true, 1);
        return OARD_EHIP;
    }
    *stage_out = stage;
    return OARD_OK;
}
static void topo_touch(const oard_topology* tp, hipStream_t st) {
    if (!tp) return;
    for (int i = 0; i < tp->n_used; ++i) if (tp->used_on[i] == st) return;
    if (tp->ready) (void)hipStreamWaitEvent(st, tp->ready, 0);
    if (tp->n_used < 4) tp->used_on[tp->n_used++] = st; else tp->used_many = true;
}

static int build_part(const oard_config* c, const int64_t* cm, const int64_t* nfs, int N_all, const std::vector<int>& obj_start,
                      const std::vector<int>& dense, const std::vector<long long>& ref_ptr_ref, int lo, int hi,
                      TopoPart& part, int& max_group, int& max_ns) {
    const int n_obj = c->n_obj, B = hi - lo;
    std::vector<int> order;
    for (int i = 0; i < N_all; ++i) if (dense[i] >= lo && dense[i] < hi) order.push_back(i);
    std::stable_sort(order.begin(), order.end(), [&](int a, int b) {
        if (dense[a] != dense[b]) return dense[a] < dense[b];
        return nfs[a] < nfs[b];
    });
    const int N = (int)order.size();
    if (N < 1) return OARD_EINVAL;
    std::vector<int> node_obj(N), node_row(N), node_ref(N), node_tidx(N), node_sample(N), sample_ptr(B + 1, 0),
        grp_ptr((size_t)B * n_obj + 1, 0), edge_ptr(N), act_ptr(N + 1, 0);
    for (int n = 0; n < N; ++n) {
        const int r = order[n], sb = dense[r] - lo;
        node_ref[n] = r; node_obj[n] = (int)nfs[r]; node_row[n] = r - obj_start[nfs[r]];
        node_tidx[n] = (int)cm[r]; node_sample[n] = sb;
        sample_ptr[sb + 1]++;
        grp_ptr[(size_t)sb * n_obj + nfs[r] + 1]++;
    }
    for (int b = 0; b < B; ++b) sample_ptr[b + 1] += sample_ptr[b];
    for (size_t q = 0; q < (size_t)B * n_obj; ++q) grp_ptr[q + 1] += grp_ptr[q];
    long long E = 0, A = 0;
    for (int b = 0; b < B; ++b) {
        const long long ns = sample_ptr[b + 1] - sample_ptr[b];
        max_ns = std::max(max_ns, (int)ns);
        for (int n = sample_ptr[b]; n < sample_ptr[b + 1]; ++n) { edge_ptr[n] = (int)E; E += ns - 1; }
        if (E > 0x7fffffffLL) return OARD_EINVAL;
    }
    for (size_t q = 0; q < (size_t)B * n_obj; ++q) {
        const long long ng = grp_ptr[q + 1] - grp_ptr[q];
        max_group = std::max(max_group, (int)ng);
        A += ng * (ng - 1);
    }
    if (max_group > OARD_MAX_GROUP || A > 0x7fffffffLL) return OARD_EINVAL;
    std::vector<int> edge_src((size_t)E + 1, 0), edge_tgt((size_t)E + 1, 0);
    for (int b = 0; b < B; ++b) {
        const int s0 = sample_ptr[b], s1 = sample_ptr[b + 1];
        for (int n = s0; n < s1; ++n) {
            size_t e = (size_t)edge_ptr[n];
            for (int m = s0; m < s1; ++m) if (m != n) { edge_src[e] = n; edge_tgt[e] = m; ++e; }
        }
    }
    std::vector<int> act_src((size_t)A + 1, 0), act_tgt((size_t)A + 1, 0), act_edge((size_t)A + 1, (int)E);
    {
        size_t a = 0;
        for (int n = 0; n < N; ++n) {
            const int q = node_sample[n] * n_obj + node_obj[n];
            const int g0 = grp_ptr[q], g1 = grp_ptr[q + 1], s0 = sample_ptr[node_sample[n]];
            act_ptr[n] = (int)a;
            for (int m = g0; m < g1; ++m) if (m != n) {
                act_src[a] = m; act_tgt[a] = n;
                act_edge[a] = edge_ptr[m] + (n - s0) - (n > m ? 1 : 0);
                ++a;
            }
        }
        act_ptr[N] = (int)a;
    }
    std::vector<int> edge_row((size_t)std::max<long long>(E, 1), -1), row_src((size_t)E + 1, 0), row_tgt((size_t)E + 1, 0),
        row_eid((size_t)E + 1, (int)E);
    {
        for (long long a = 0; a < A; ++a) {
            edge_row[act_edge[a]] = (int)a; row_src[a] = act_src[a]; row_tgt[a] = act_tgt[a]; row_eid[a] = act_edge[a];
        }
        long long r = A;
        for (long long e = 0; e < E; ++e)
            if (edge_row[e] < 0) { edge_row[e] = (int)r; row_src[r] = edge_src[e]; row_tgt[r] = edge_tgt[e]; row_eid[r] = (int)e; ++r; }
    }
    std::vector<long long> ref_edge_ptr(N);
    for (int n = 0; n < N; ++n) ref_edge_ptr[n] = ref_ptr_ref[node_ref[n]];
    std::vector<int> col_row, col_info, node_cols((size_t)N * 4, 0);
    long long CI = 0, CX = 0;
    {
        auto pad16 = [&]() { while (col_row.size() % 16) col_row.push_back((int)E); };
        for (int b = 0; b < B; ++b) {
            for (int n = sample_ptr[b]; n < sample_ptr[b + 1]; ++n) {
                const int q = node_sample[n] * n_obj + node_obj[n];
                const int g0 = grp_ptr[q], g1 = grp_ptr[q + 1];
                node_cols[4 * (size_t)n + 0] = (int)col_row.size();
                for (int m = g0; m < g1; ++m) if (m != n) col_row.push_back(act_ptr[m] + (n - g0) - (n > m ? 1 : 0));
                node_cols[4 * (size_t)n + 1] = (int)col_row.size();
            }
            pad16();
        }
        CI = (long long)col_row.size();
        for (int b = 0; b < B; ++b) {
            const int ns = sample_ptr[b + 1] - sample_ptr[b];
            for (int n = sample_ptr[b]; n < sample_ptr[b + 1]; ++n) {
                node_cols[4 * (size_t)n + 2] = (int)col_row.size();
                for (long long e = edge_ptr[n]; e < (long long)edge_ptr[n] + ns - 1; ++e) if (edge_row[e] >= A) col_row.push_back(edge_row[e]);
                node_cols[4 * (size_t)n + 3] = (int)col_row.size();
            }
            pad16();
        }
        CX = (long long)col_row.size() - CI;
        if (CI + CX > 0x7fffffffLL - 256) return OARD_EINVAL;
        if (col_row.empty()) col_row.push_back((int)E);
        col_info.resize(col_row.size() * 4);
        for (size_t k = 0; k < col_row.size(); ++k) {
            const int r = col_row[k];
            col_info[4 * k] = r; col_info[4 * k + 1] = row_src[r]; col_info[4 * k + 2] = row_tgt[r];
            col_info[4 * k + 3] = r == (int)E ? -1 : row_src[r] + 1;
        }
    }

    std::vector<UploadItem> items;
    size_t cur = 0;
    auto add = [&](const void* p, size_t bytes) { UploadItem it{p, bytes, cur}; cur = align_up(cur + bytes, 256); items.push_back(it); return it.off; };
    const size_t o_obj = add(node_obj.data(), N * 4), o_row = add(node_row.data(), N * 4), o_ref = add(node_ref.data(), N * 4),
                 o_tidx = add(node_tidx.data(), N * 4), o_smp = add(node_sample.data(), N * 4),
                 o_sptr = add(sample_ptr.data(), (B + 1) * 4), o_eptr = add(edge_ptr.data(), N * 4),
                 o_esrc = add(edge_src.data(), edge_src.size() * 4), o_etgt = add(edge_tgt.data(), edge_tgt.size() * 4),
                 o_gptr = add(grp_ptr.data(), grp_ptr.size() * 4), o_aptr = add(act_ptr.data(), (N + 1) * 4),
                 o_asrc = add(act_src.data(), act_src.size() * 4), o_atgt = add(act_tgt.data(), act_tgt.size() * 4),
                 o_aedge = add(act_edge.data(), act_edge.size() * 4), o_rptr = add(ref_edge_ptr.data(), N * 8),
                 o_erow = add(edge_row.data(), edge_row.size() * 4), o_rsrc = add(row_src.data(), row_src.size() * 4),
                 o_rtgt = add(row_tgt.data(), row_tgt.size() * 4), o_reid = add(row_eid.data(), row_eid.size() * 4),
                 o_crow = add(col_info.data(), col_info.size() * 4), o_ncol = add(node_cols.data(), node_cols.size() * 4);
    size_t cap = 0;
    char* dev = (char*)pool_alloc(cur, &cap);
    if (!dev) return OARD_EHIP;
    if (int rc = pool_upload(dev, items, cur, &part.stage, &part.stage_cap)) { pool_release(dev, cap, nullptr, 0, false); return rc; }
    part.dev_cap = cap;
    part.dev_block = dev;
    TopoDev& d = part.d;
    d.N = N; d.B = B; d.n_obj = n_obj; d.n_groups = B * n_obj; d.E = E; d.A = A;
    d.node_obj = (const int*)(dev + o_obj); d.node_row = (const int*)(dev + o_row); d.node_ref = (const int*)(dev + o_ref);
    d.node_tidx = (const int*)(dev + o_tidx); d.node_sample = (const int*)(dev + o_smp); d.sample_ptr = (const int*)(dev + o_sptr);
    d.edge_ptr = (const int*)(dev + o_eptr); d.edge_src = (const int*)(dev + o_esrc); d.edge_tgt = (const int*)(dev + o_etgt);
    d.grp_ptr = (const int*)(dev + o_gptr); d.act_ptr = (const int*)(dev + o_aptr); d.act_src = (const int*)(dev + o_asrc);
    d.act_tgt = (const int*)(dev + o_atgt); d.act_edge = (const int*)(dev + o_aedge);
    d.ref_edge_ptr = (const long long*)(dev + o_rptr);
    d.edge_row = (const int*)(dev + o_erow); d.row_src = (const int*)(dev + o_rsrc); d.row_tgt = (const int*)(dev + o_rtgt);
    d.row_eid = (const int*)(dev + o_reid);
    d.CI = CI; d.CX = CX; d.col_info = (const int*)(dev + o_crow); d.node_cols = (const int*)(dev + o_ncol);
    return OARD_OK;
}

int oard_topology_create(const oard_config* c, const int64_t* cm, const int64_t* nfs, int64_t n_nodes,
                         oard_topology** out) {
    return oard_topology_create_parts(c, cm, nfs, n_nodes, g_parts, out);
}

int oard_topology_create_parts(const oard_config* c, const int64_t* cm, const int64_t* nfs, int64_t n_nodes,
                               int parts, oard_topology** out) {
    if (!config_ok(c) || !cm || !nfs || !out || n_nodes < 1 || n_nodes > (1 << 24)) return OARD_EINVAL;
    const int N = (int)n_nodes, n_obj = c->n_obj;
    std::vector<int> obj_start(n_obj + 1, 0);
    for (int i = 0; i < N; ++i) {
        if (nfs[i] < 0 || nfs[i] >= n_obj) return OARD_EINVAL;
        if (i > 0 && nfs[i] < nfs[i - 1]) return OARD_EINVAL;
        obj_start[nfs[i] + 1]++;
    }
    for (int k = 0; k < n_obj; ++k) obj_start[k + 1] += obj_start[k];
    std::vector<int64_t> samples(cm, cm + N);
    std::sort(samples.begin(), samples.end());
    samples.erase(std::unique(samples.begin(), samples.end()), samples.end());
    const int B = (int)samples.size();
    if (samples.front() < 0 || samples.back() > (1 << 30)) return OARD_EINVAL;
    std::vector<int> dense(N), ns_of(B, 0);
    for (int i = 0; i < N; ++i) {
        dense[i] = (int)(std::lower_bound(samples.begin(), samples.end(), cm[i]) - samples.begin());
        ns_of[dense[i]]++;
    }
    std::vector<long long> ref_ptr_ref(N);
    long long E_all = 0;
    for (int r = 0; r < N; ++r) { ref_ptr_ref[r] = E_all; E_all += ns_of[dense[r]] - 1; }

    int n_parts = parts > 0 ? parts : (B >= 32 ? 4 : (B >= 16 ? 2 : 1));
    n_parts = std::max(1, std::min(std::min(n_parts, OARD_MAX_PARTS), B));
    oard_topology* tp = new oard_topology();
    (void)hipGetDevice(&tp->device);
    tp->n_obj = n_obj; tp->B = B; tp->n_parts = n_parts;
    {
        std::vector<int> tab(2 * (size_t)N), seen(B, 0);
        for (int r = 0; r < N; ++r) { tab[r] = dense[r]; tab[(size_t)N + r] = seen[dense[r]]++; }
        const size_t b_int = 2 * (size_t)N * sizeof(int), b_all = align_up(b_int, 8) + (size_t)N * sizeof(long long);
        tp->ref_block = pool_alloc(b_all, &tp->ref_cap);
        if (!tp->ref_block) { delete tp; return OARD_EHIP; }
        const std::vector<UploadItem> ref_items = {{tab.data(), b_int, 0}, {ref_ptr_ref.data(), (size_t)N * sizeof(long long), align_up(b_int, 8)}};
        if (int rc = pool_upload(tp->ref_block, ref_items, b_all, &tp->ref_stage, &tp->ref_stage_cap)) { oard_topology_destroy(tp); return rc; }
        tp->ref_sample = (const int*)tp->ref_block; tp->ref_rank = tp->ref_sample + N;
        tp->ref_ptr = (const long long*)((char*)tp->ref_block + align_up(b_int, 8));
        tp->N_ref = N;
    }
    for (int k = 0; k <= n_obj && k <= OARD_MAX_OBJECTS; ++k) tp->obj_start[k] = obj_start[k];
    for (int p = 0; p < n_parts; ++p) {
        const int lo = (int)((long long)B * p / n_parts), hi = (int)((long long)B * (p + 1) / n_parts);
        int rc = build_part(c, cm, nfs, N, obj_start, dense, ref_ptr_ref, lo, hi, tp->parts[p], tp->max_group, tp->max_ns);
        if (rc != OARD_OK) { oard_topology_destroy(tp); return rc; }
        tp->N += tp->parts[p].d.N; tp->E += tp->parts[p].d.E; tp->A += tp->parts[p].d.A;
        tp->parts[p].conc = n_parts;
    }
    {
        const int npb = g_npb > 0 ? g_npb : (int)std::max<long long>(1, std::min<long long>(16, cdiv(tp->N, 256)));
        for (int p = 0; p < n_parts; ++p) tp->parts[p].d.npb = npb;
    }
    if (n_parts > 1) {
        HIP_TRY(hipEventCreateWithFlags(&tp->ev_fork, hipEventDisableTiming));
        for (int p = 1; p < n_parts; ++p) {
            tp->side[p] = device_streams()[(p - 1) % 3];
            if (!tp->side[p]) { oard_topology_destroy(tp); return OARD_EHIP; }
            HIP_TRY(hipEventCreateWithFlags(&tp->ev_join[p], hipEventDisableTiming));
        }
    }
    HIP_TRY(hipEventCreateWithFlags(&tp->ready, hipEventDisableTiming));
    HIP_TRY(hipEventRecord(tp->ready, device_streams()[2]));
    *out = tp;
    return OARD_OK;
}

void oard_topology_destroy(oard_topology* tp) {
    if (!tp) return;
    int cur = tp->device;
    (void)hipGetDevice(&cur);
    if (cur != tp->device) (void)hipSetDevice(tp->device);
    struct Restore { int cur, dev; ~Restore() { if (cur != dev) (void)hipSetDevice(cur); } } restore_{cur, tp->device};
    for (int p = 0; p < OARD_MAX_PARTS; ++p) {
        pool_release(tp->parts[p].dev_block, tp->parts[p].dev_cap, tp->used_on, tp->n_used, tp->used_many);
        pool_release(tp->parts[p].stage, tp->parts[p].stage_cap, nullptr, 0, false, 1);
        if (tp->ev_join[p]) (void)hipEventDestroy(tp->ev_join[p]);
    }
    if (tp->ev_fork) (void)hipEventDestroy(tp->ev_fork);
    pool_release(tp->ref_block, tp->ref_cap, tp->used_on, tp->n_used, tp->used_many);
    pool_release(tp->ref_stage, tp->ref_stage_cap, nullptr, 0, false, 1);
    if (tp->ready) (void)hipEventDestroy(tp->ready);
    delete tp;
}
int64_t oard_topology_num_nodes(const oard_topology* tp) { return tp ? tp->N : 0; }
int64_t oard_topology_num_edges(const oard_topology* tp) { return tp ? tp->E : 0; }
int64_t oard_topology_num_inner_edges(const oard_topology* tp) { return tp ? tp->A : 0; }
int64_t oard_topology_num_samples(const oard_topology* tp) { return tp ? tp->B : 0; }

int oard_topology_check_edge_index(const oard_topology* tp, const int64_t* ei, int64_t n_edges, int32_t* ok,
                                   oard_stream_t stream) {
    topo_touch(tp, (hipStream_t)stream);
    if (!tp || !ok) return OARD_EINVAL;
    hipStream_t st = (hipStream_t)stream;
    const int one = (n_edges == tp->E) ? 1 : 0;
    HIP_TRY(hipMemcpyAsync(ok, &one, sizeof(int), hipMemcpyHostToDevice, st));
    HIP_TRY(hipStreamSynchronize(st));
    if (one && tp->E > 0) {
        if (!ei) return OARD_EINVAL;
        unsigned* bitmap = nullptr;
        const size_t words = (size_t)cdiv(tp->E, 32);
        HIP_TRY(hipMalloc(&bitmap, words * sizeof(unsigned)));
        hipError_t e1 = hipMemsetAsync(bitmap, 0, words * sizeof(unsigned), st);
        if (e1 == hipSuccess) {
            hipLaunchKernelGGL(k_check_edge_set, dim3((unsigned)cdiv(n_edges, 256)), dim3(256), 0, st, tp->ref_sample, tp->ref_rank,
                               tp->ref_ptr, tp->N_ref, (const long long*)ei, (long long)n_edges, bitmap, (int*)ok);
            e1 = hipGetLastError();
        }
        const hipError_t e2 = hipStreamSynchronize(st);
        (void)hipFree(bitmap);
        HIP_TRY(e1);
        HIP_TRY(e2);
    }
    return OARD_OK;
}

static size_t ws_total(const oard_config* c, const oard_topology* tp) {
    size_t cur = 0;
    for (int p = 0; p < tp->n_parts; ++p) {
        const_cast<TopoPart&>(tp->parts[p]).ws_off = cur;
        cur = align_up(cur + make_ws(c, tp->parts[p].d).total, 4096);
    }
    return cur;
}
size_t oard_workspace_bytes(const oard_config* c, const oard_topology* tp) {
    if (!config_ok(c) || !tp) return 0;
    return ws_total(c, tp);
}

int oard_debug_lin3u_table(const oard_config* c, const void* packed, int layer, float* out, oard_stream_t stream) {
    static_assert(OARD_L3T_FLOATS == L3T_FLOATS, "include/oard.h and csrc/oard_layout.h disagree on the table size");
    if (!config_ok(c) || !packed || !out || layer < 0 || layer >= c->num_layers) return OARD_EINVAL;
    const PackOff po = make_layout(c);
    HIP_TRY(hipMemcpyAsync(out, (const float*)packed + po.layer[layer].l3t, (size_t)L3T_FLOATS * sizeof(float), hipMemcpyDeviceToDevice,
                           (hipStream_t)stream));
    return OARD_OK;
}

int oard_active_inner_edges(const oard_config* c, const oard_topology* topo, const void* ws, size_t ws_bytes, int64_t* n_active,
                            oard_stream_t stream) {
    if (!config_ok(c) || !topo || !ws || !n_active) return OARD_EINVAL;
    if (ws_bytes < ws_total(c, topo)) return OARD_ENOMEM;
    hipStream_t st = (hipStream_t)stream;
    long long total = 0;
// ... 647 lines not shown
}

int oard_nan_replace(const oard_config* c, const oard_topology* topo, const int32_t* status, const float* const* noise,
                     float* const* out, oard_stream_t stream) {
    topo_touch(topo, (hipStream_t)stream);
    if (!config_ok(c) || !topo || !status || !noise || !out || c->n_obj != topo->n_obj) return OARD_EINVAL;
    NanPtrs np;
    memset(&np, 0, sizeof(np));
    for (int k = 0; k < c->n_obj; ++k) { np.noise[k] = noise[k]; np.out[k] = out[k]; np.node_nf[k] = c->node_nf[k]; }
    for (int p = 0; p < topo->n_parts; ++p)
        LAUNCH(F_OTHER, k_nan_replace, cdiv(topo->parts[p].d.N, 128), 128, (hipStream_t)stream, topo->parts[p].d, np, (const int*)status);
    HIP_TRY(hipGetLastError());
    return OARD_OK;
}

static LossCfg make_loss_cfg(const oard_config* c, const float* norm_values, const float* norm_biases, const float* scales, int pos_only,
                             int fixed_mask, int T) {
    LossCfg lc;
    memset(&lc, 0, sizeof(lc));
    for (int i = 0; i < 3; ++i) { lc.norm_value[i] = norm_values ? norm_values[i] : 1.0f; lc.norm_bias[i] = norm_biases ? norm_biases[i] : 0.0f; }
    for (int k = 0; k < c->n_obj; ++k) lc.scale[k] = scales ? scales[k] : 1.0f;
    lc.pos_only = pos_only; lc.fixed_mask = fixed_mask; lc.T = T;
    return lc;
}
int oard_loss_prepare(const oard_config* c, const oard_topology* topo, const float* const* pos, const int64_t* const* one_hot,
                      const int64_t* const* charge, const float* const* noise, const float* t_int, const float* gamma, int T,
                      const float* norm_values, const float* norm_biases, int pos_only, int fixed_mask, float* const* z,
                      float* const* eps, oard_stream_t stream) {
    topo_touch(topo, (hipStream_t)stream);
    if (!config_ok(c) || !topo || topo->n_parts != 1 || !pos || !one_hot || !charge || !noise || !t_int || !gamma || !z || !eps)
        return OARD_EINVAL;
    LossPtrs lp;
    memset(&lp, 0, sizeof(lp));
    for (int k = 0; k < c->n_obj; ++k) {
        if (c->node_nf[k] < 5 || c->node_nf[k] - 4 > 16) return OARD_EINVAL;
        lp.pos[k] = pos[k]; lp.one_hot[k] = (const long long*)one_hot[k]; lp.charge[k] = (const long long*)charge[k];
        lp.noise[k] = noise[k]; lp.z[k] = z[k]; lp.eps[k] = eps[k]; lp.node_nf[k] = c->node_nf[k];
    }
    const TopoDev& tp = topo->parts[0].d;
    LAUNCH(F_OTHER, k_loss_prep, cdiv(tp.N, 128), 128, (hipStream_t)stream, tp, lp,
           make_loss_cfg(c, norm_values, norm_biases, nullptr, pos_only, fixed_mask, T), t_int, gamma);
    HIP_TRY(hipGetLastError());
    return OARD_OK;
}
int oard_loss_terms(const oard_config* c, const oard_topology* topo, const float* const* eps, const float* const* net,
                    const float* const* z, const int64_t* const* one_hot, const int64_t* const* charge, const float* t_int,
                    const float* gamma, int T, const float* norm_values, const float* norm_biases, const float* scales, int pos_only,
                    int B, float* nll, float* terms, float* const* dnet, oard_stream_t stream) {
    topo_touch(topo, (hipStream_t)stream);
    if (!config_ok(c) || !topo || topo->n_parts != 1 || !eps || !net || !z || !one_hot || !charge || !t_int || !gamma || !nll || !terms ||
        !dnet || B < 1)
        return OARD_EINVAL;
    LossPtrs lp;
    memset(&lp, 0, sizeof(lp));
    for (int k = 0; k < c->n_obj; ++k) {
        if (c->node_nf[k] < 5 || c->node_nf[k] - 4 > 16) return OARD_EINVAL;
        lp.eps[k] = (float*)eps[k]; lp.net[k] = net[k]; lp.z[k] = (float*)z[k]; lp.one_hot[k] = (const long long*)one_hot[k];
        lp.charge[k] = (const long long*)charge[k]; lp.dnet[k] = dnet[k]; lp.node_nf[k] = c->node_nf[k];
    }
    const TopoDev& tp = topo->parts[0].d;
    LAUNCH(F_OTHER, k_loss_terms, tp.B, 64, (hipStream_t)stream, tp, lp, make_loss_cfg(c, norm_values, norm_biases, scales, pos_only, 0, T),
           t_int, gamma, B, nll, terms);
    HIP_TRY(hipGetLastError());
    return OARD_OK;
}
int oard_adamw_step(float* param, const float* grad, float* exp_avg, float* exp_avg_sq, float* max_exp_avg_sq, int64_t n, double lr,
                    double beta1, double beta2, double eps, double weight_decay, int64_t step, int amsgrad, double grad_scale,
                    oard_stream_t stream) {
    if (!param || !grad || !exp_avg || !exp_avg_sq || (amsgrad && !max_exp_avg_sq) || n < 0 || step < 1) return OARD_EINVAL;
    if (n == 0) return OARD_OK;
    const double bc1 = 1.0 - pow(beta1, (double)step), bc2 = 1.0 - pow(beta2, (double)step);
    LAUNCH(F_OTHER, k_adamw, cdiv(n, 256), 256, (hipStream_t)stream, param, grad, exp_avg, exp_avg_sq, max_exp_avg_sq, (long long)n,
           (float)(1.0 - lr * weight_decay), (float)(1.0 - beta1), (float)beta2, (float)(1.0 - beta2), (float)eps, (float)(lr / bc1),
           (float)(1.0 / sqrt(bc2)), amsgrad, (float)grad_scale);
    HIP_TRY(hipGetLastError());
    return OARD_OK;
}

int oard_adamw_step_dev(float* param, const float* grad, float* exp_avg, float* exp_avg_sq, float* max_exp_avg_sq, int64_t n, double lr,
                        double beta1, double beta2, double eps, double weight_decay, int amsgrad, int clip, double* clip_state,
                        int capacity, const float* grad_norm, const float* flag, float* out4, oard_stream_t stream) {
    if (!param || !grad || !exp_avg || !exp_avg_sq || (amsgrad && !max_exp_avg_sq) || n < 0 || !clip_state || capacity < 1 || capacity > 64 ||
        !grad_norm || !flag || !out4)
        return OARD_EINVAL;
    LAUNCH(F_OTHER, k_clip_decide, 1, 64, (hipStream_t)stream, clip_state, capacity, grad_norm, flag, clip, lr, beta1, beta2, eps, weight_decay, out4);
    if (n > 0)
        LAUNCH(F_OTHER, k_adamw_dev, cdiv(n, 256), 256, (hipStream_t)stream, param, grad, exp_avg, exp_avg_sq, max_exp_avg_sq, (long long)n, amsgrad,
               reinterpret_cast<const AdamScal*>(clip_state + 4 + capacity));
    HIP_TRY(hipGetLastError());
    return OARD_OK;
}

int oard_train_scratch_entry(const oard_config* c, const oard_topology* topo, int which, size_t* offset_bytes, int64_t* rows,
                             int64_t* row_floats) {
    if (!config_ok(c) || !topo || topo->n_parts != 1 || !offset_bytes || !rows || !row_floats) return OARD_EINVAL;
    const TopoDev& d = topo->parts[0].d;
    const TrainWs w = make_train_ws(c, d);
    const RDims r(c->hidden, c->num_radial);
    switch (which) {
        case OARD_SCRATCH_XH: *offset_bytes = w.xh; *rows = d.N; *row_floats = r.HP; break;
        case OARD_SCRATCH_XQ: *offset_bytes = w.xq; *rows = d.N; *row_floats = 3 * r.HP; break;
        case OARD_SCRATCH_CR: *offset_bytes = w.cr; *rows = d.A + 1; *row_floats = 3 * r.HP; break;
        case OARD_SCRATCH_DCD: *offset_bytes = w.dcd; *rows = d.A + 1; *row_floats = 3 * r.HP; break;
        case OARD_SCRATCH_DCR: *offset_bytes = w.dcr; *rows = d.A + 1; *row_floats = 3 * r.HP; break;
        default: return OARD_EINVAL;
    }
    return OARD_OK;
}

int oard_tap(const oard_config* c, const oard_topology* topo, const void* ws_, int which, int layer, float* dst,
             oard_stream_t stream) {
    topo_touch(topo, (hipStream_t)stream);
    if (!config_ok(c) || !topo || !ws_ || !dst || layer != 0) return OARD_EINVAL;
    const RDims d(c->hidden, c->num_radial);
    ws_total(c, topo);
    hipStream_t st = (hipStream_t)stream;
    for (int p = 0; p < topo->n_parts; ++p) {
        const TopoDev& tp = topo->parts[p].d;
        const WsOff w = make_ws(c, tp);
        const char* ws = (const char*)ws_ + topo->parts[p].ws_off;
        auto nodes = [&](const float* src, int ld, int sections, int sect_pad, int sect_len) {
            const long long tot = (long long)tp.N * sections * sect_len;
            hipLaunchKernelGGL(k_tap_nodes, dim3((unsigned)cdiv(tot, 256)), dim3(256), 0, st, tp, src, ld, sections, sect_pad, sect_len, dst);
        };
        switch (which) {
            case OARD_TAP_S: nodes((const float*)(ws + w.s), d.HP, 1, d.HP, d.H); break;
            case OARD_TAP_VEC: nodes((const float*)(ws + topo->parts[p].vec_final), 3 * d.HP, 3, d.HP, d.H); break;
            case OARD_TAP_NE1: nodes((const float*)(ws + w.ne1), 3 * d.HP, 3, d.HP, d.H); break;
            case OARD_TAP_POS_FRAME: nodes((const float*)(ws + w.pf32), 3, 1, 3, 3); break;
            case OARD_TAP_DPOS: nodes((const float*)(ws + w.dpos), 3, 1, 3, 3); break;
            case OARD_TAP_HOUT: nodes((const float*)(ws + w.hout), 16, 1, 16, c->in_hidden); break;
            case OARD_TAP_LABELS:
                hipLaunchKernelGGL(k_tap_labels, dim3((unsigned)cdiv(tp.N, 256)), dim3(256), 0, st, tp, (const int*)(ws + w.labels), dst);
                break;
            case OARD_TAP_EDGE:
                if (tp.E > 0)
                    hipLaunchKernelGGL(k_tap_edges, dim3((unsigned)cdiv(tp.E * d.W, 256)), dim3(256), 0, st, tp,
                                       (const float*)(ws + w.ew), d.WP, d.W, dst);
                break;
            default: return OARD_EINVAL;
        }
    }
    HIP_TRY(hipGetLastError());
    return OARD_OK;
}

int oard_debug_stop_after(int code) { g_stop_after = code; return OARD_OK; }
int oard_debug_option(const char* name, int value) {
    if (!name) return OARD_EINVAL;
    static const struct { const char* name; int* value; } table[] = {
        {"gcl_variant", &g_fwd.gcl_variant}, {"equi_variant", &g_fwd.equi_variant}, {"node_variant", &g_fwd.node_variant},
        {"auto_small", &g_fwd.auto_small}, {"auto_tiny", &g_fwd.auto_tiny}, {"small_split", &g_fwd.small_split},
        {"gcl_persist", &g_fwd.gcl_persist}, {"gcl_grid", &g_fwd.gcl_grid}, {"gcl_skip", &g_fwd.gcl_skip}, {"equi_skip", &g_fwd.equi_skip},
        {"equi_l0_skip", &g_fwd.equi_l0_skip}, {"gcl_msum", &g_fwd.gcl_msum},
        {"skip_families", &g_skip_families}, {"parts", &g_parts}, {"sequential", &g_sequential}, {"poison", &g_poison}, {"npb", &g_npb},
        {"wgrad_wgs", &g_wgrad_wgs}, {"wgrad_t16", &g_wgrad_t16}, {"wgrad_queue", &g_wgrad_queue}, {"gate_fold", &g_gate_fold},
        {"wgrad_lds", &g_wgrad_lds}, {"wgrad_shapes", &g_wgrad_shapes}, {"train_dual", &g_train_dual}};
    if (strcmp(name, "experiments") == 0) return kV0 ? OARD_OK : OARD_EINVAL;
    if (strcmp(name, "gcl_msum_taken") == 0) return g_gcl_msum_taken ? OARD_OK : OARD_EINVAL;
    if (strcmp(name, "equi_l0_taken") == 0) return g_equi_l0_taken ? OARD_OK : OARD_EINVAL;
    for (const auto& e : table) {
        if (strcmp(name, e.name) != 0) continue;
        if (!kV0 && value == 0 && strstr(name, "_variant")) return OARD_EINVAL;
        *e.value = e.value == &g_wgrad_shapes ? value & 3 : value;
        return OARD_OK;
    }
    return OARD_EINVAL;
}
#ifdef OARD_PHASE_PROBE
int oard_debug_probe_read(unsigned long long* out8) {
    if (!out8) return OARD_EINVAL;
    HIP_TRY(hipDeviceSynchronize());
    HIP_TRY(hipMemcpyFromSymbol(out8, HIP_SYMBOL(g_phase_probe), 8 * sizeof(unsigned long long)));
    unsigned long long z[8] = {};
    HIP_TRY(hipMemcpyToSymbol(HIP_SYMBOL(g_phase_probe), z, sizeof(z)));
    return OARD_OK;
}
#endif
#ifdef OARD_TIMELINE
int oard_debug_timeline_read(long long* out, int waves) {
    if (!out || waves < 1 || waves > 16) return OARD_EINVAL;
    HIP_TRY(hipDeviceSynchronize());
    HIP_TRY(hipMemcpyFromSymbol(out, HIP_SYMBOL(g_timeline), (size_t)waves * TL_MAX * sizeof(long long)));
    return OARD_OK;
}
#endif
#ifdef OARD_EXPERIMENTS
int oard_debug_fp_timeouts(unsigned int* out) {
    if (!out) return OARD_EINVAL;
    HIP_TRY(hipDeviceSynchronize());
    HIP_TRY(hipMemcpyFromSymbol(out, HIP_SYMBOL(g_fp_timeouts), sizeof(unsigned int)));
    return OARD_OK;
}
#endif
int oard_timing_enable(int on) { g_timing.on = on != 0; return OARD_OK; }
int oard_timing_reset(void) {
    g_timing.flush();
    for (int f = 0; f < F_COUNT; ++f) { g_timing.total_ms[f] = 0; g_timing.launches[f] = 0; }
    return OARD_OK;
}
int oard_timing_get(const char* family, double* total_ms, int64_t* launches) {
    if (!family || !total_ms || !launches) return OARD_EINVAL;
    g_timing.flush();
    for (int f = 0; f < F_COUNT; ++f)
        if (strcmp(family, kFamilyNames[f]) == 0) { *total_ms = g_timing.total_ms[f]; *launches = g_timing.launches[f]; return OARD_OK; }
    return OARD_EINVAL;
}

}
```

### oareactdiff_amd/csrc/oard_inst.h

```cpp
#pragma once
#if !defined(OARD_EXPERIMENTS) && !defined(OARD_SINGLE_TU)

#define OARD_UNPAREN(...) __VA_ARGS__
#ifdef OARD_INST_DEFINE
#define OARD_INST(K, ARGS) template __global__ void OARD_UNPAREN K ARGS;
#else
#define OARD_INST(K, ARGS) extern template __global__ void OARD_UNPAREN K ARGS;
#endif
#ifndef OARD_DIMS_LIST
#define OARD_DIMS_LIST X(196, 96) X(32, 8) X(32, 32)
#endif
#define OARD_BOOL4(M, D) M(D, true, true) M(D, false, true) M(D, true, false) M(D, false, false)

#define OARD_NW(h) (((h) + 15) / 16 <= 16 ? ((h) + 15) / 16 : 8)
#define OARD_A_GCL (TopoDev, const float*, const float*, const float*, const float*, const float*, long long, long long, const float*, float*, float*, GclTape)

#if !defined(OARD_INST_DEFINE) || defined(OARD_INST_UNIT_GCL_P)
#define OARD_I_GCL_P(D, S1, S3) OARD_INST((k_gcl_edge_p<OARD_UNPAREN D, S1, S3, false>), OARD_A_GCL) OARD_INST((k_gcl_edge_p<OARD_UNPAREN D, S1, S3, true>), OARD_A_GCL) \
    OARD_INST((k_gcl_edge_p<OARD_UNPAREN D, S1, S3, false, true>), OARD_A_GCL)
#define X(h, r) OARD_BOOL4(OARD_I_GCL_P, (Dims<h, r>))
OARD_DIMS_LIST
#undef X
#endif

#if !defined(OARD_INST_DEFINE) || defined(OARD_INST_UNIT_GCL_V1)
#define OARD_I_GCL_V1(D, S1, S3) \
    OARD_INST((k_gcl_edge_v1<OARD_UNPAREN D, 8, 2, S1, S3, false, false, 2, 3>), OARD_A_GCL) OARD_INST((k_gcl_edge_v1<OARD_UNPAREN D, 8, 2, S1, S3, true, false, 2, 3>), OARD_A_GCL) \
    OARD_INST((k_gcl_edge_v1<OARD_UNPAREN D, 8, 2, S1, S3, false, true, 2, 3>), OARD_A_GCL) \
    OARD_INST((k_gcl_edge_v1<OARD_UNPAREN D, 4, 2, S1, S3, false, false, 2, 2>), OARD_A_GCL) \
    OARD_INST((k_gcl_edge_small<OARD_UNPAREN D, 8, S1, S3>), (TopoDev, const float*, LayerOff, const float*, const float*, const float*, const float*, long long, long long, float*, float*))
#define X(h, r) OARD_BOOL4(OARD_I_GCL_V1, (Dims<h, r>))
OARD_DIMS_LIST
#undef X
#endif

#if !defined(OARD_INST_DEFINE) || defined(OARD_INST_UNIT_B3)
#define OARD_A_EQUI_B3 (TopoDev, const float*, const float*, const float*, const float*, const float*, float*, float*, float*, float*, ActList)
#define OARD_I_GCL_B3(D, S1, S3) OARD_INST((k_gcl_edge_b3<OARD_UNPAREN D, S1, S3, false>), OARD_A_GCL) OARD_INST((k_gcl_edge_b3<OARD_UNPAREN D, S1, S3, true>), OARD_A_GCL)
#define X(h, r) OARD_BOOL4(OARD_I_GCL_B3, (Dims<h, r>)) OARD_INST((k_equi_edge_b3<Dims<h, r>, false>), OARD_A_EQUI_B3) OARD_INST((k_equi_edge_b3<Dims<h, r>, true>), OARD_A_EQUI_B3)
OARD_DIMS_LIST
#undef X
#endif

#if !defined(OARD_INST_DEFINE) || defined(OARD_INST_UNIT_EQUI)
#define OARD_A_EQUI (TopoDev, const float*, const float*, const float*, const float*, float*, float*, float*, ActList, int)
#define OARD_A_EQUI_NODE (TopoDev, const float*, LayerOff, const float*, const float*, const float*, const float*, const float*, float*, const float*, float*, float*, float*, ActList)
#define X(h, r) \
    OARD_INST((k_equi_edge_v1<Dims<h, r>, 8, false>), OARD_A_EQUI) OARD_INST((k_equi_edge_v1<Dims<h, r>, 8, true>), OARD_A_EQUI) \
    OARD_INST((k_equi_edge_v1<Dims<h, r>, 4, false>), OARD_A_EQUI) \
    OARD_INST((k_equi_node_v1<Dims<h, r>, OARD_NW(h), false, false>), OARD_A_EQUI_NODE) OARD_INST((k_equi_node_v1<Dims<h, r>, OARD_NW(h), false, true>), OARD_A_EQUI_NODE) \
    OARD_INST((k_equi_node_v1<Dims<h, r>, OARD_NW(h), true, false>), OARD_A_EQUI_NODE) OARD_INST((k_equi_node_v1<Dims<h, r>, OARD_NW(h), true, true>), OARD_A_EQUI_NODE) \
    OARD_INST((k_equi_node_v1<Layer0<Dims<h, r> >, OARD_NW(h), false, false>), OARD_A_EQUI_NODE) OARD_INST((k_equi_node_v1<Layer0<Dims<h, r> >, OARD_NW(h), false, true>), OARD_A_EQUI_NODE) \
    OARD_INST((k_gcl_edge_bwd<Dims<h, r>, 8, 2, true>), (TopoDev, const float*, long long, long long, GclBwdArgs)) \
    OARD_INST((k_gcl_edge_bwd<Dims<h, r>, 8, 2, false>), (TopoDev, const float*, long long, long long, GclBwdArgs)) \
    OARD_INST((k_equi_edge_bwd<Dims<h, r>, 8>), (TopoDev, const float*, const float*, const float*, float*, float*))
OARD_DIMS_LIST
#undef X
#endif

#if !defined(OARD_INST_DEFINE) || defined(OARD_INST_UNIT_NODE)
#define OARD_A_GCL_NODE (TopoDev, const float*, LayerOff, const float*, const float*, float*, float*, float*)
#define OARD_A_OUT (TopoDev, const float*, PackOff, const float*, const float*, float*, float*, int*)
#define OARD_A_SCAL_BWD (TopoDev, const float*, const float*, int, const float*, const float*, float*, float*)
#define OARD_A_MSG_BWD (TopoDev, const float*, Strided3, Strided3, const float*, Strided3, const float*, int, Strided3, float*, float*, float*, float*, int, int, int)
#define X(h, r) \
    OARD_INST((k_gcl_node_v1<Dims<h, r>, OARD_NW(h), false>), OARD_A_GCL_NODE) OARD_INST((k_gcl_node_v1<Dims<h, r>, OARD_NW(h), true>), OARD_A_GCL_NODE) \
    OARD_INST((k_gcl_node_v1<Dims<h, r>, OARD_NW(h), false, true>), OARD_A_GCL_NODE) \
    OARD_INST((k_out_v1<Dims<h, r>, OARD_NW(h)>), OARD_A_OUT) \
    OARD_INST((k_scalarize_bwd<Dims<h, r>, 2, false>), OARD_A_SCAL_BWD) OARD_INST((k_scalarize_bwd<Dims<h, r>, 2, true>), OARD_A_SCAL_BWD) \
    OARD_INST((k_equi_msg_bwd<Dims<h, r> >), OARD_A_MSG_BWD)
OARD_DIMS_LIST
#undef X
OARD_INST((k_lin3u_bwd_fused<4>), (const float*, const float*, const float*, long long, float*, float*))
#define OARD_I_ROWS(KB, EPI) OARD_INST((k_rows_dense<KB, EPI, 8>), (RowsDense)) OARD_INST((k_rows_dense_long<KB, EPI, 8, 4>), (RowsDense))
OARD_I_ROWS(13, 0) OARD_I_ROWS(13, 2) OARD_I_ROWS(13, 3) OARD_I_ROWS(7, 3) OARD_I_ROWS(6, 0) OARD_I_ROWS(6, 1) OARD_I_ROWS(4, 1) OARD_I_ROWS(4, 3)
OARD_INST((k_rows_dense<26, 1, 8>), (RowsDense)) OARD_INST((k_rows_dense<26, 3, 8>), (RowsDense))
OARD_INST((k_rows_dense2<13, 1, 8, 13>), (RowsDense2)) OARD_INST((k_rows_dense2<13, 2, 8, 13>), (RowsDense2))
OARD_INST((k_rows_dense2<26, 1, 8, 13>), (RowsDense2)) OARD_INST((k_rows_dense2<39, 2, 8, 13>), (RowsDense2))
#endif

#if !defined(OARD_INST_DEFINE) || defined(OARD_INST_UNIT_WGRAD)
#define OARD_A_WG (const float*, int, int, const float*, int, int, long long, long long, long long, int, int, float*, float*, float*)
OARD_INST((k_wgrad_t16<4, 7, false>), (WgtArgs)) OARD_INST((k_wgrad_t16<4, 7, true>), (WgtArgs)) OARD_INST((k_wgrad_t16<5, 3, false>), (WgtArgs))
OARD_INST((k_wgrad_t16<5, 5, true>), (WgtArgs)) OARD_INST((k_wgrad_t16<5, 7, true>), (WgtArgs)) OARD_INST((k_wgrad_t16<6, 5, false>), (WgtArgs))
OARD_INST((k_wgrad_t16<6, 7, false>), (WgtArgs))
OARD_INST((k_wgrad<false, 7>), OARD_A_WG) OARD_INST((k_wgrad<false, 8>), OARD_A_WG) OARD_INST((k_wgrad<true, 7>), OARD_A_WG) OARD_INST((k_wgrad<true, 8>), OARD_A_WG)
OARD_INST((k_wgrad_lds<false, 7, 4, 2>), OARD_A_WG) OARD_INST((k_wgrad_lds<false, 8, 4, 2>), OARD_A_WG)
OARD_INST((k_wgrad_lds<true, 7, 4, 2>), OARD_A_WG) OARD_INST((k_wgrad_lds<true, 8, 4, 2>), OARD_A_WG)
#endif

#endif
```

### oareactdiff_amd/csrc/oard_kernels.h

```cpp
#pragma once
#include "oard_engine.h"
#include "oard_layout.h"

#define GEO_STRIDE 12
#define EPSF 1e-6

struct ColId {
    int lane, g, col;
    bool valid;
    long long c;
};
OARD_DEV ColId col_id(long long ncols, bool& wave_live) {
    ColId id;
    id.lane = threadIdx.x & 63;
    id.g = id.lane >> 4;
    const long long cb = (long long)blockIdx.x * 4 + (threadIdx.x >> 6);
    wave_live = cb * 16 < ncols;
    const long long c = cb * 16 + (id.lane & 15);
    id.valid = c < ncols;
    id.c = id.valid ? c : (ncols > 0 ? ncols - 1 : 0);
    id.col = (int)id.c;
    return id;
}

// ... 345 lines not shown
    const long long a = (long long)blockIdx.x * blockDim.x + threadIdx.x;
    if (blk_cnt != nullptr) {
        int in = 0;
        if (a < tp.A) {
            const int i = tp.act_src[a], j = tp.act_tgt[a];
            const double rx = (double)pos[i * 3] - (double)pos[j * 3], ry = (double)pos[i * 3 + 1] - (double)pos[j * 3 + 1],
                         rz = (double)pos[i * 3 + 2] - (double)pos[j * 3 + 2];
            in = sqrt(rx * rx + ry * ry + rz * rz) < cutoff ? 1 : 0;
        }
        const int cnt = __syncthreads_count(in);
        if (threadIdx.x == 0) blk_cnt[blockIdx.x] = cnt;
    }
    if (a >= tp.A) return;
    const int i = tp.act_src[a], j = tp.act_tgt[a];
    const double rx = (double)pos[i * 3] - (double)pos[j * 3], ry = (double)pos[i * 3 + 1] - (double)pos[j * 3 + 1],
                 rz = (double)pos[i * 3 + 2] - (double)pos[j * 3 + 2];
    const double m = sqrt(rx * rx + ry * ry + rz * rz) < cutoff ? 1.0 : 0.0;
    const double ax = pf64[i * 3], ay = pf64[i * 3 + 1], az = pf64[i * 3 + 2];
    const double bx = pf64[j * 3], by = pf64[j * 3 + 1], bz = pf64[j * 3 + 2];
    const double dx = ax - bx, dy = ay - by, dz = az - bz;
    const double dist = sqrt(dx * dx + dy * dy + dz * dz);
    const double nr = dist + EPSF;
    double ux = dx / nr, uy = dy / nr, uz = dz / nr;
    double cx = ay * bz - az * by, cy = az * bx - ax * bz, cz = ax * by - ay * bx;
    const double cn = sqrt(cx * cx + cy * cy + cz * cz) + EPSF;
    cx /= cn; cy /= cn; cz /= cn;
    double vx = uy * cz - uz * cy, vy = uz * cx - ux * cz, vz = ux * cy - uy * cx;
    const double d = dist * m;
    const double env = 0.5 * (cos(d * M_PI / cutoff) + 1.0);
    float* g = geo + a * GEO_STRIDE;
    g[0] = (float)d; g[1] = (float)env;
    g[2] = (float)(ux * m); g[3] = (float)(uy * m); g[4] = (float)(uz * m);
    g[5] = (float)(cx * m); g[6] = (float)(cy * m); g[7] = (float)(cz * m);
    g[8] = (float)(vx * m); g[9] = (float)(vy * m); g[10] = (float)(vz * m);
    g[11] = (float)m;
    d64[a] = d;
}

__device__ inline void lin3u_f64(const float* __restrict__ p, double x, double& f, double& df) {
    double h[48], dh[48];
    for (int k = 0; k < 48; ++k) {
        const double w = (double)p[3 * k], z = w * x + (double)p[144 + k], s = 1.0 / (1.0 + exp(-z));
        h[k] = z * s; dh[k] = w * s * (1.0 + z * (1.0 - s));
    }
    f = (double)p[592]; df = 0.0;
    for (int j = 0; j < 8; ++j) {
        double z = (double)p[576 + j], dz = 0.0;
        for (int k = 0; k < 48; ++k) { const double w = (double)p[192 + j * 48 + k]; z += w * h[k]; dz += w * dh[k]; }
        const double s = 1.0 / (1.0 + exp(-z));
        f += (double)p[584 + j] * z * s; df += (double)p[584 + j] * dz * s * (1.0 + z * (1.0 - s));
    }
}
OARD_DEV float lin3u_table_eval(const float* __restrict__ tab, float x) {
    const float u = x * (1.0f / L3T_H), fl = floorf(u), t = u - fl;
    const int i = (int)fl + L3T_N / 2;
    const float f0 = tab[2 * i], d0 = tab[2 * i + 1], f1 = tab[2 * i + 2], d1 = tab[2 * i + 3];
    const float t2 = t * t, t3 = t2 * t;
    return (2.f * t3 - 3.f * t2 + 1.f) * f0 + (t3 - 2.f * t2 + t) * d0 + (3.f * t2 - 2.f * t3) * f1 + (t3 - t2) * d1;
}
struct L3tJobs { size_t l3u[OARD_MAX_LAYERS], l3t[OARD_MAX_LAYERS]; };
OARD_KERNEL __global__ __launch_bounds__(256) void k_lin3u_table_fill(float* __restrict__ blob, L3tJobs j) {
    const float* p = blob + j.l3u[blockIdx.y];
    float* tab = blob + j.l3t[blockIdx.y];
    const int i = blockIdx.x * 256 + threadIdx.x;
    double f, df;
    lin3u_f64(p, ((double)i - L3T_N / 2) * (double)L3T_H, f, df);
    tab[2 * i] = (float)f; tab[2 * i + 1] = (float)(df * (double)L3T_H);
    if (i == 0) {
        lin3u_f64(p, (double)L3T_X, f, df);
        tab[2 * L3T_N] = (float)f; tab[2 * L3T_N + 1] = (float)(df * (double)L3T_H);
        tab[2 * (L3T_N + 1)] = 0.f; tab[2 * (L3T_N + 1) + 1] = 0.f; tab[2 * (L3T_N + 1) + 2] = 0.f; tab[2 * (L3T_N + 1) + 3] = 0.f;
    }
}
OARD_KERNEL __global__ __launch_bounds__(256) void k_lin3u_table_check(float* __restrict__ blob, L3tJobs j) {
    __shared__ float red_e[256], red_f[256];
    const float* p = blob + j.l3u[blockIdx.y];
    float* tab = blob + j.l3t[blockIdx.y];
    const int i = blockIdx.x * 256 + threadIdx.x, t = threadIdx.x;
    const double x = ((double)i - L3T_N / 2 + 0.5) * (double)L3T_H;
    double f, df;
    lin3u_f64(p, x, f, df);
    red_e[t] = fabsf(lin3u_table_eval(tab, (float)x) - (float)f);
    red_f[t] = fmaxf(fabsf(tab[2 * i]), fabsf((float)f));
    __syncthreads();
    for (int d = 128; d >= 1; d >>= 1) {
        if (t < d) { red_e[t] = fmaxf(red_e[t], red_e[t + d]); red_f[t] = fmaxf(red_f[t], red_f[t + d]); }
        __syncthreads();
    }
    if (t == 0) {
        unsigned* u = reinterpret_cast<unsigned*>(tab + 2 * (L3T_N + 1));
        atomicMax(u + 1, __float_as_uint(red_e[0]));
        atomicMax(u + 2, __float_as_uint(red_f[0]));
        __threadfence();
        if (atomicAdd(u + 3, 1u) == gridDim.x - 1) {
            __threadfence();
            const float e = __uint_as_float(atomicMax(u + 1, 0u)), fm = __uint_as_float(atomicMax(u + 2, 0u));
            tab[2 * (L3T_N + 1)] = (e <= 2e-7f * fmaxf(fm, 1e-30f) && fm < 3e38f) ? 1.0f : 0.0f;
        }
    }
}
struct ZeroRows { float* p[64]; int n[64]; int count; };
OARD_KERNEL __global__ __launch_bounds__(256) void k_zero_rows(ZeroRows z) {
    if ((int)blockIdx.x >= z.count) return;
    float* p = z.p[blockIdx.x];
    for (int i = threadIdx.x; i < z.n[blockIdx.x]; i += 256) p[i] = 0.f;
}
OARD_KERNEL __global__ __launch_bounds__(256) void k_active_list(TopoDev tp, const float* __restrict__ geo, const int* __restrict__ blk_cnt,
                                                     int* __restrict__ rows, int* __restrict__ src, int* __restrict__ pre, int* __restrict__ n_act) {
    __shared__ int red[256];
    __shared__ int wsum[4];
    int base = 0;
    for (int b = threadIdx.x; b < (int)blockIdx.x; b += 256) base += blk_cnt[b];
    red[threadIdx.x] = base;
    __syncthreads();
    for (int d = 128; d >= 1; d >>= 1) {
        if ((int)threadIdx.x < d) red[threadIdx.x] += red[threadIdx.x + d];
        __syncthreads();
    }
    base = red[0];
    const long long a = (long long)blockIdx.x * 256 + threadIdx.x;
    const bool on = a < tp.A && geo[a * GEO_STRIDE + 11] > 0.f;
    const unsigned long long bal = __ballot(on);
    const int lane = threadIdx.x & 63, wave = threadIdx.x >> 6;
    const int in_wave = __popcll(bal & ((1ull << lane) - 1ull));
    if (lane == 0) wsum[wave] = __popcll(bal);
    __syncthreads();
    int off = base + in_wave;
    for (int w = 0; w < wave; ++w) off += wsum[w];
    if (a < tp.A) pre[a] = off;
    if (on) { rows[off] = (int)a; src[off] = tp.act_src[a]; }
    if (a == tp.A - 1) { const int tot = off + (on ? 1 : 0); pre[tp.A] = tot; *n_act = tot; }
}
OARD_KERNEL __global__ void k_rbf(TopoDev tp, const double* __restrict__ d64, const float* __restrict__ geo,
                      const float* __restrict__ means, const float* __restrict__ betas, double cutoff,
                      float* __restrict__ rbuf, float* __restrict__ ew, int R, int RP, int H, int WP) {
    const long long i = (long long)blockIdx.x * blockDim.x + threadIdx.x;
    if (i >= tp.A * RP) return;
    const long long a = i / RP;
    const int k = (int)(i % RP);
    float v = 0.f;
    if (k < R) {
        const double d = d64[a], m = (double)geo[a * GEO_STRIDE + 11];
        double rb = 0.5 * (cos(d * M_PI / cutoff) + 1.0);
        rb = d < cutoff ? rb : 0.0;
        const double q = exp(-d) - (double)means[k];
        v = (float)(rb * exp(-(double)betas[k] * q * q) * m);
        ew[(size_t)a * WP + 3 * H + k] = v;
        if (k == 0)
            for (int c = 3 * H + R; c < WP; ++c) ew[(size_t)a * WP + c] = 0.f;
    }
    rbuf[i] = v;
}

OARD_KERNEL __global__ void k_fill_edges(const float* __restrict__ c0, float* __restrict__ ew, long long E, int WP) {
    const int per = WP / 4;
    const long long total = E * per;
    for (long long i = (long long)blockIdx.x * blockDim.x + threadIdx.x; i < total; i += (long long)gridDim.x * blockDim.x)
        st_f4(ew + i * 4, ld_f4(c0 + (i % per) * 4));
}

template <class D>
__global__ __launch_bounds__(256) void k_node_embed(TopoDev tp, const float* __restrict__ wb, PackOff po,
                                                    const float* __restrict__ hin, float* __restrict__ zemb,
                                                    float* __restrict__ nb) {
    bool live; const ColId id = col_id(tp.N, live);
    if (!live) return;
    f4 in[1] = {ld_blk(hin, id.c, 16, 0, id.lane)};
    f4 v[D::HT];
#pragma unroll
    for (int t = 0; t < D::HT; ++t) {
        f4 z = dense_tile<1>(wb + po.emb, t, in, id.lane, ld_vec(wb + po.emb_b, t, id.lane));
        if (id.valid) st_blk(zemb, id.c, D::HP, t, id.lane, z);
        v[t] = dense_tile<1>(wb + po.nbemb, t, in, id.lane, ld_vec(wb + po.nbemb_b, t, id.lane));
    }
    layer_norm<D::HT, D::H, false>(v, nullptr, nullptr, id.lane);
    if (id.valid)
#pragma unroll
        for (int t = 0; t < D::HT; ++t) st_blk(nb, id.c, D::HP, t, id.lane, v[t]);
}

template <class D>
__global__ __launch_bounds__(256) void k_radial_lin(TopoDev tp, const float* __restrict__ wb, PackOff po,
                                                    const float* __restrict__ rbuf, const float* __restrict__ geo,
                                                    float* __restrict__ ew) {
    bool live; const ColId id = col_id(tp.A, live);
    if (!live) return;
    f4 rb[D::RB];
#pragma unroll
    for (int b = 0; b < D::RB; ++b) rb[b] = ld_blk(rbuf, id.c, D::RP, b, id.lane);
    f4 h1[D::HT];
    dense_regs<D::RB, D::HT, true, true>(wb + po.rl0, wb + po.rl0_b, rb, h1, id.lane);
    const float env = geo[id.c * GEO_STRIDE + 1];
    const size_t row = (size_t)id.c * D::WP + 2 * D::H;
#pragma unroll
    for (int t = 0; t < D::HT; ++t) {
        f4 f = dense_tile<D::HT>(wb + po.rl2, t, h1, id.lane, ld_vec(wb + po.rl2_b, t, id.lane));
        if (id.valid && 16 * t + 4 * id.g < D::H) st_f4(ew + row + 16 * t + 4 * id.g, f * env);
    }
}

template <class D>
__global__ __launch_bounds__(256) void k_neighbor(TopoDev tp, const float* __restrict__ wb, PackOff po,
                                                  const float* __restrict__ zemb, const float* __restrict__ nb,
                                                  const float* __restrict__ ew, float* __restrict__ s,
                                                  float* __restrict__ s1) {
    bool live; const ColId id = col_id(tp.N, live);
    if (!live) return;
    const int n = id.col, smp = tp.node_sample[n], s0 = tp.sample_ptr[smp], ns = tp.sample_ptr[smp + 1] - s0;
    f4 acc[D::HT];
#pragma unroll
    for (int t = 0; t < D::HT; ++t) acc[t] = f4zero();
    const int mx = wave_max(ns);
    for (int k = 0; k < mx; ++k) {
        const int m = s0 + k;
        if (k < ns && m != n) {
            const int r = tp.edge_row[tp.edge_ptr[m] + (n - s0) - (n > m ? 1 : 0)];
            const float* frow = (r < tp.A ? ew + (size_t)r * D::WP : wb + po.c0row) + 2 * D::H;
#pragma unroll
            for (int t = 0; t < D::HT; ++t)
                if (16 * t + 4 * id.g < D::H)
                    acc[t] += ld_f4(frow + 16 * t + 4 * id.g) * ld_blk(nb, m, D::HP, t, id.lane);
        }
    }
#pragma unroll
    for (int t = 0; t < D::HT; ++t) acc[t] += ld_blk(zemb, n, D::HP, t, id.lane);
    if (id.valid)
#pragma unroll
        for (int t = 0; t < D::HT; ++t) st_blk(s, n, D::HP, t, id.lane, acc[t]);
    f4 y[D::HT];
    dense_regs<D::HT, D::HT, false, true>(wb + po.s2v, wb + po.s2v_b, acc, y, id.lane);
    layer_norm<D::HT, D::H, false>(y, nullptr, nullptr, id.lane);
    if (id.valid)
#pragma unroll
        for (int t = 0; t < D::HT; ++t) st_blk(s1, n, D::HP, t, id.lane, silu4(y[t]));
}

template <class D>
__global__ __launch_bounds__(256) void k_s2v_agg(TopoDev tp, const float* __restrict__ s1, const float* __restrict__ ew,
                                                 const float* __restrict__ geo, float* __restrict__ ne1) {
    bool live; const ColId id = col_id(tp.N, live);
    if (!live) return;
    const int n = id.col, a0 = tp.act_ptr[n], cnt = tp.act_ptr[n + 1] - a0;
    const int mx = wave_max(cnt);
    const bool fok = true;
    for (int t = 0; t < D::HT; ++t) {
        f4 ax = f4zero(), ay = f4zero(), az = f4zero();
        if (16 * t + 4 * id.g < D::H && fok) {
            for (int k = 0; k < mx; ++k) {
                if (k < cnt) {
                    const int a = a0 + k, m = tp.act_src[a];
                    const float* g = geo + (size_t)a * GEO_STRIDE;
                    const f4 p = ld_f4(ew + (size_t)a * D::WP + 2 * D::H + 16 * t + 4 * id.g) *
                                 ld_blk(s1, m, D::HP, t, id.lane);
                    ax += p * g[2]; ay += p * g[3]; az += p * g[4];
                }
            }
        }
        if (id.valid) {
            st_blk(ne1, (size_t)n * 3 + 0, D::HP, t, id.lane, ax);
            st_blk(ne1, (size_t)n * 3 + 1, D::HP, t, id.lane, ay);
            st_blk(ne1, (size_t)n * 3 + 2, D::HP, t, id.lane, az);
        }
    }
}

template <class D>
__global__ __launch_bounds__(256) void k_scalarize(TopoDev tp, const float* __restrict__ wb, PackOff po,
                                                   const float* __restrict__ ne1, const float* __restrict__ geo,
                                                   float* __restrict__ ew) {
    bool live; const ColId id = col_id(tp.A, live);
    if (!live) return;
    const long long a = id.c;
    const int ni = tp.act_src[a], nj = tp.act_tgt[a];
    const float* g = geo + (size_t)a * GEO_STRIDE;
    const float env = g[1];
    const float ux = g[2], uy = g[3], uz = g[4], cx = g[5], cy = g[6], cz = g[7], vx = g[8], vy = g[9], vz = g[10];
    const float* l3 = wb + po.lin3;
    const float* w0 = l3;
    const float* b0 = l3 + D::H4 * 3;
    const float* w2 = b0 + D::H4;
    const float b2 = w2[D::H4];
    const size_t row = (size_t)a * D::WP;
    for (int t = blockIdx.y; t < D::HT; t += gridDim.y) {
        if (16 * t + 4 * id.g >= D::H) continue;
#pragma unroll
        for (int side = 0; side < 2; ++side) {
            const int node = side == 0 ? ni : nj;
            const f4 n0 = ld_blk(ne1, (size_t)node * 3 + 0, D::HP, t, id.lane);
            const f4 n1 = ld_blk(ne1, (size_t)node * 3 + 1, D::HP, t, id.lane);
            const f4 n2 = ld_blk(ne1, (size_t)node * 3 + 2, D::HP, t, id.lane);
            const f4 S0 = n0 * ux + n1 * uy + n2 * uz;
            f4 S1 = n0 * cx + n1 * cy + n2 * cz;
            const f4 S2 = n0 * vx + n1 * vy + n2 * vz;
            if (!po.signed_scal) S1 = (f4){fabsf(S1.x), fabsf(S1.y), fabsf(S1.z), fabsf(S1.w)};
            f4 o = (f4){b2, b2, b2, b2};
            for (int k = 0; k < D::H4; ++k) {
                const float wa = w0[3 * k], wbb = w0[3 * k + 1], wc = w0[3 * k + 2], bb = b0[k], ww = w2[k];
                o += silu4(S0 * wa + S1 * wbb + S2 * wc + bb) * ww;
            }
            o = (o + S0) * env;
            if (id.valid) st_f4(ew + row + side * D::H + 16 * t + 4 * id.g, o);
        }
    }
}

template <class D>
__global__ __launch_bounds__(256) void k_node_pre(TopoDev tp, const float* __restrict__ wb, PackOff po, LayerOff lo,
                                                  const float* __restrict__ s, const float* __restrict__ pp0,
                                                  float* __restrict__ xh, float* __restrict__ P, float* __restrict__ Q) {
    bool live; const ColId id = col_id(tp.N, live);
    if (!live) return;
    const int n = id.col;
    const float pp = pp0[n];
    f4 hid[D::PB];
#pragma unroll
    for (int b = 0; b < D::PB; ++b) {
        const int k0 = 16 * b + 4 * id.g;
        const float* w = wb + po.pe0;
        hid[b].x = k0 + 0 < D::H2 ? silu1(w[(k0 + 0) * 3] * pp) : 0.f;
        hid[b].y = k0 + 1 < D::H2 ? silu1(w[(k0 + 1) * 3] * pp) : 0.f;
        hid[b].z = k0 + 2 < D::H2 ? silu1(w[(k0 + 2) * 3] * pp) : 0.f;
        hid[b].w = k0 + 3 < D::H2 ? silu1(w[(k0 + 3) * 3] * pp) : 0.f;
    }
    f4 v[D::HT];
#pragma unroll
    for (int t = 0; t < D::HT; ++t)
        v[t] = ld_blk(s, n, D::HP, t, id.lane) + dense_tile<D::PB>(wb + po.pe1, t, hid, id.lane, f4zero());
    layer_norm<D::HT, D::H, true>(v, wb + lo.ln_g_w, wb + lo.ln_g_b, id.lane);
#pragma unroll
    for (int t = 0; t < D::HT; ++t)
        if (id.valid) st_blk(xh, n, D::HP, t, id.lane, v[t]);
    for (int t = 0; t < D::HT; t += 1) {
        f4 p = ld_vec(wb + lo.b1, t, id.lane), q = f4zero();
        p = dense_tile<D::HT>(wb + lo.W1a, t, v, id.lane, p);
        q = dense_tile<D::HT>(wb + lo.W1b, t, v, id.lane, q);
        if (id.valid) { st_blk(P, n, D::HP, t, id.lane, p); st_blk(Q, n, D::HP, t, id.lane, q); }
    }
}

template <class D>
__global__ __launch_bounds__(256) void k_gcl_node(TopoDev tp, const float* __restrict__ wb, LayerOff lo,
                                                  const float* __restrict__ xh, const float* __restrict__ mbuf,
                                                  float* __restrict__ s, float* __restrict__ xq) {
    bool live; const ColId id = col_id(tp.N, live);
    if (!live) return;
    const int n = id.col, smp = tp.node_sample[n];
    const int deg = tp.sample_ptr[smp + 1] - tp.sample_ptr[smp] - 1;
    const size_t e0 = (size_t)tp.edge_ptr[n];
    f4 in[2 * D::HT];
#pragma unroll
// ... 318 lines not shown
```

### oareactdiff_amd/csrc/oard_layout.h

```cpp
#pragma once
#include <hip/hip_runtime.h>
#include <stdint.h>
#include <stddef.h>
#include "../../include/oard.h"

#define OARD_MAX_LAYERS 16
#define OARD_MAX_GROUP 1024

template <int H_, int R_>
struct Dims {
    static constexpr int H = H_, R = R_;
    static constexpr int HT = (H + 15) / 16, HP = HT * 16;
    static constexpr int W = 3 * H + R, WB = (W + 15) / 16, WP = WB * 16;
    static constexpr int RB = (R + 15) / 16, RP = RB * 16;
    static constexpr int H2 = H / 2, PB = (H2 + 15) / 16, PP = PB * 16;
    static constexpr int D1T = (3 * H + 15) / 16, D1P = D1T * 16;
    static constexpr int H4 = H / 4;
    static_assert(H % 4 == 0 && R % 4 == 0, "feature widths must be multiples of 4");
};

struct RDims {
    int H, R, HT, HP, W, WB, WP, RB, RP, H2, PB, PP, D1T, D1P, H4;
    explicit RDims(int h, int r) {
        H = h; R = r; HT = (H + 15) / 16; HP = HT * 16; W = 3 * H + R; WB = (W + 15) / 16; WP = WB * 16;
        RB = (R + 15) / 16; RP = RB * 16; H2 = H / 2; PB = (H2 + 15) / 16; PP = PB * 16;
        D1T = (3 * H + 15) / 16; D1P = D1T * 16; H4 = H / 4;
    }
};

#define L3T_X 16.0f
#define L3T_H 0.03125f
#define L3T_N 1024
#define L3T_FLOATS (2 * (L3T_N + 1) + 4)

struct LayerOff {
    size_t ln_g_w, ln_g_b, W1a, b1, W1b, W1c, W2, b2, watt, batt, W3, b3, nm0, nm0b, nm1, nm1b;
    size_t ln_q_w, ln_q_b, xp0, xp2, dp0, dp0b, dp2, dp2b, rbfp;
    size_t vp, xv0, xv2, l3u;
    size_t l3t;
    size_t gcl_stream, equi_stream;
    size_t gcl_b3, equi_b3;
    int xcross;
};
struct PackOff {
    size_t emb, emb_b, nbemb, nbemb_b, s2v, s2v_b, rl0, rl0_b, rl2, rl2_b;
    size_t lin3;
    size_t pe0;
    size_t pe1, embout, embout_b, v1p, v2p, un0, un0_b, un2, un2_b;
    size_t c0row;
    size_t u0;
    size_t rbf_means, rbf_betas;
    size_t enc[OARD_MAX_OBJECTS], dec[OARD_MAX_OBJECTS];
    LayerOff layer[OARD_MAX_LAYERS];
    size_t total;
    int signed_scal;
};

struct TopoDev {
    int N, B, n_obj, n_groups;
    int npb;
    long long E, A;
    const int *node_obj, *node_row, *node_ref, *node_tidx, *node_sample, *sample_ptr;
    const int *edge_ptr, *edge_src, *edge_tgt;
    const int *edge_row;
    const int *row_src, *row_tgt;
    const int *row_eid;
    const int *grp_ptr;
    const int *act_ptr, *act_src, *act_tgt, *act_edge;
    const long long *ref_edge_ptr;
    long long CI, CX;
    const int *col_info;
    const int *node_cols;
};

struct ActList {
    const int* rows;
    const int* src;
    const int* pre;
    const int* n;
};

#define OARD_MAX_PARTS 8
struct TopoPart {
    TopoDev d;
    void* dev_block = nullptr;
    size_t dev_cap = 0;
    void* stage = nullptr;
    size_t stage_cap = 0;
    size_t ws_off = 0;
    int conc = 1;
    mutable size_t vec_final = 0;
};
struct oard_topology {
    int device = 0;
    int n_parts = 0;
    TopoPart parts[OARD_MAX_PARTS];
    int n_obj = 0, B = 0;
    long long N = 0, E = 0, A = 0;
    int max_group = 0, max_ns = 0;
    int obj_start[OARD_MAX_OBJECTS + 1] = {};
    hipStream_t side[OARD_MAX_PARTS] = {};
    hipEvent_t ev_fork = nullptr, ev_join[OARD_MAX_PARTS] = {};
    void* ref_block = nullptr;
    size_t ref_cap = 0;
    void* ref_stage = nullptr;
    size_t ref_stage_cap = 0;
    hipEvent_t ready = nullptr;
    mutable hipStream_t used_on[4] = {};
    mutable int n_used = 0;
    mutable bool used_many = false;
    const int *ref_sample = nullptr, *ref_rank = nullptr;
    const long long* ref_ptr = nullptr;
    int N_ref = 0;
};

struct WsOff {
    size_t pos, pf64, pf32, x1, pp0, labels, hin, zemb, nb, s, s1, ne1, xh, P, Q, xq, vec, vec2, v2buf, sc0, vdot,
        geo, d64, rbuf, ew, mbuf, xmsg, vmsg, dpos, hout, total;
    size_t al_rows, al_src, al_pre, al_cnt, al_n;
    size_t d1s;
    size_t small_a;
};
```

### oareactdiff_amd/csrc/oard_plan.h

```cpp
#pragma once
#include <algorithm>
#include "../../include/oard.h"

struct FwdOptions {
    int gcl_variant = 2;
    int equi_variant = 2;
    int node_variant = 1;
    int auto_small = 4;
    int auto_tiny = 8;
    int small_split = 128;
    int gcl_persist = 1;
    int gcl_grid = 0;
    int gcl_skip = 1;
    int equi_skip = 1;
    int equi_l0_skip = 1;
    int gcl_msum = 1;
};

enum GclShape {
    GCL_INVALID = 0,
    GCL_V0,
    GCL_PERSIST, GCL_RING3,
    GCL_W4, GCL_SMALL, GCL_B3,
    GCL_TRAIN_PERSIST, GCL_TRAIN_RING3, GCL_TRAIN_B3,
    GCL_X0 = 100
};
enum EquiShape { EQ_INVALID = 0, EQ_V0, EQ_W8, EQ_W4, EQ_SMALL, EQ_SMALL_SPLIT, EQ_B3, EQ_TRAIN, EQ_TRAIN_B3 };
enum NodeForm { NODE_V0 = 0, NODE_ROWS, NODE_LARGE };

struct GclLaunch { long long r0, r1; bool s1, s3; GclShape shape; long long grid; };
struct GclLayer { int n; GclLaunch l[2]; };
struct FwdPlanIn {
    FwdOptions opt;
    int precision;
    bool train;
    int conc, npb, cus;
    long long A, E, CI, CX;
    int num_layers;
    bool scratch;
};
struct FwdPlan {
    int num_layers;
    bool fill_edges;
    bool init_v1;
    bool scalarize_tiles;
    bool msum;
    GclLayer gcl[4];
    EquiShape equi;
    bool use_al;
    NodeForm node;
    bool l0_skip;
    const GclLayer& gcl_at(int l) const { return gcl[(l == 0 ? 1 : 0) | (l == num_layers - 1 ? 2 : 0)]; }
};

inline long long plan_cdiv(long long a, long long b) { return (a + b - 1) / b; }
inline int plan_demote(const FwdPlanIn& in, int v, long long n, long long small_tiles, int w4, int lat) {
    const long long load = plan_cdiv(n, 16) * in.conc;
    if (v == 2 && load <= small_tiles * in.opt.auto_small) v = w4;
    if ((v == 2 || v == w4) && load <= 512LL * in.opt.auto_tiny) v = lat;
    return v;
}
inline GclShape plan_gcl_shape(const FwdPlanIn& in, long long n) {
    const int persist = in.opt.gcl_persist;
    if (in.train) return (in.precision & OARD_PREC_TRAIN_BF16X3) ? GCL_TRAIN_B3 : persist ? GCL_TRAIN_PERSIST : GCL_TRAIN_RING3;
    const int v = plan_demote(in, in.opt.gcl_variant, n, 1024, 3, 6);
    switch (v) {
        case 0: return GCL_V0;
        case 2: return (in.precision & OARD_PREC_GCL_BF16X3) ? GCL_B3 : (persist > 1 || (persist == 1 && in.conc == 1)) ? GCL_PERSIST : GCL_RING3;
        case 3: return GCL_W4;
        case 6: return GCL_SMALL;
#ifdef OARD_EXPERIMENTS
        case 4: case 5: case 7: case 8: case 9: case 10: case 11: case 12: return GclShape(GCL_X0 + v);
#endif
        default: return GCL_INVALID;
    }
}
inline long long plan_gcl_grid(const FwdPlanIn& in, GclShape s, long long n) {
    if (s == GCL_PERSIST || s == GCL_TRAIN_PERSIST) {
        const long long nhalf = plan_cdiv(plan_cdiv(n, 16), 4), g = in.opt.gcl_grid;
        return std::min(nhalf, g > 0 ? g : g < 0 ? plan_cdiv(nhalf, 2 * -g) : in.conc > 1 ? std::max(1, in.cus / 2) : in.cus);
    }
    return plan_cdiv(n, s == GCL_SMALL ? 16 : (s == GCL_V0 || s == GCL_W4 || s == GCL_X0 + 12) ? 64 : (s == GCL_X0 + 10 || s == GCL_X0 + 11) ? 192 : 128);
}
inline EquiShape plan_equi_shape(const FwdPlanIn& in) {
    if (in.train) return (in.precision & OARD_PREC_TRAIN_BF16X3) ? EQ_TRAIN_B3 : EQ_TRAIN;
    switch (plan_demote(in, in.opt.equi_variant, in.A, 512, 1, 4)) {
        case 0: return EQ_V0;
        case 1: return EQ_W4;
        case 2: return (in.precision & OARD_PREC_EQUI_BF16X3) ? EQ_B3 : EQ_W8;
        case 4: return in.scratch && plan_cdiv(in.A, 16) * in.conc <= in.opt.small_split ? EQ_SMALL_SPLIT : EQ_SMALL;
        default: return EQ_INVALID;
    }
}
inline FwdPlan make_fwd_plan(FwdPlanIn in) {
    if (in.train) { in.opt.gcl_variant = in.opt.equi_variant = 2; in.opt.node_variant = 1; in.opt.gcl_skip = 1; }
    const FwdOptions& o = in.opt;
    const bool nv1 = o.node_variant == 1 && o.equi_variant != 0, skip = o.gcl_skip && o.gcl_variant != 0;
    FwdPlan p = {};
    p.num_layers = in.num_layers;
    p.fill_edges = !skip;
    p.init_v1 = o.node_variant >= 1;
    p.scalarize_tiles = plan_cdiv(in.A, 64) * in.conc <= 2048;
    p.node = !nv1 ? NODE_V0 : in.npb <= 4 ? NODE_ROWS : NODE_LARGE;
    p.equi = plan_equi_shape(in);
    p.use_al = !in.train && o.equi_skip && in.A > 0 && nv1;
    p.l0_skip = !in.train && o.equi_l0_skip && in.A > 0 && p.node == NODE_LARGE && p.equi == EQ_W8;
    auto throughput = [&](long long n) { const GclShape s = plan_gcl_shape(in, n); return n == 0 || s == GCL_PERSIST || s == GCL_RING3; };
    p.msum = !in.train && o.gcl_msum && in.E > 0 && o.gcl_variant == 2 && p.node == NODE_LARGE && throughput(in.CI) && throughput(in.CX);
    const long long inner = p.msum ? in.CI : in.A, all = p.msum ? in.CI + in.CX : in.E;
    for (int k = 0; k < 4; ++k) {
        GclLayer& g = p.gcl[k];
        auto add = [&](long long r0, long long r1, bool s1, bool s3) {
            const GclShape s = plan_gcl_shape(in, r1 - r0);
            if (r1 > r0) g.l[g.n++] = GclLaunch{r0, r1, s1, s3, s, plan_gcl_grid(in, s, r1 - r0)};
        };
        const bool s1 = !(skip && (k & 1)), s3 = !(skip && (k & 2));
        if (s1 && s3) add(0, all, true, true);
        else { add(0, inner, true, true); add(inner, all, s1, s3); }
    }
    return p;
}
```

Measured before the change: 3703 reaction-steps/s.

## Compute radial terms once per symmetric edge pair and precompute RBF projection

Exploits that the RBF features and the radial linear projections depend only on distance, so they are identical for the edges (m,n) and (n,m). The change computes them once per unordered pair and writes the result to both rows, and adds a pair-level kernel that precomputes the RBF projection (cr) for the equivariant edge kernel, which then loads it instead of running the RB chain per edge. This roughly halves radial work and shrinks the weight stream the equi kernel prefetches. The cost is an extra launch, a new crbuf workspace, and extra pair-index tables built on the host at topology creation.

```diff
diff --git a/oareactdiff_amd/_capi.py b/oareactdiff_amd/_capi.py
--- a/oareactdiff_amd/_capi.py
+++ b/oareactdiff_amd/_capi.py
@@ -152,7 +152,7 @@
     L.oard_timing_reset.argtypes = []; L.oard_timing_reset.restype = C.c_int
     L.oard_timing_get.argtypes = [C.c_char_p, C.POINTER(C.c_double), C.POINTER(i64)]; L.oard_timing_get.restype = C.c_int
     for env, opt in (("OARD_GCL_VARIANT", b"gcl_variant"), ("OARD_EQUI_VARIANT", b"equi_variant"),
-                     ("OARD_NODE_VARIANT", b"node_variant"), ("OARD_GCL_SKIP", b"gcl_skip"), ("OARD_EQUI_SKIP", b"equi_skip"), ("OARD_EQUI_L0_SKIP", b"equi_l0_skip"), ("OARD_GCL_MSUM", b"gcl_msum"), ("OARD_GCL_PERSIST", b"gcl_persist"), ("OARD_GCL_GRID", b"gcl_grid"), ("OARD_PARTS", b"parts"), ("OARD_SEQUENTIAL", b"sequential"), ("OARD_POISON", b"poison"), ("OARD_AUTO_SMALL", b"auto_small"), ("OARD_AUTO_TINY", b"auto_tiny"), ("OARD_NPB", b"npb"),
+                     ("OARD_NODE_VARIANT", b"node_variant"), ("OARD_GCL_SKIP", b"gcl_skip"), ("OARD_EQUI_SKIP", b"equi_skip"), ("OARD_EQUI_L0_SKIP", b"equi_l0_skip"), ("OARD_GCL_MSUM", b"gcl_msum"), ("OARD_PAIR_TERMS", b"pair_terms"), ("OARD_GCL_PERSIST", b"gcl_persist"), ("OARD_GCL_GRID", b"gcl_grid"), ("OARD_PARTS", b"parts"), ("OARD_SEQUENTIAL", b"sequential"), ("OARD_POISON", b"poison"), ("OARD_AUTO_SMALL", b"auto_small"), ("OARD_AUTO_TINY", b"auto_tiny"), ("OARD_NPB", b"npb"),
                      ("OARD_WGRAD_WGS", b"wgrad_wgs"), ("OARD_WGRAD_LDS", b"wgrad_lds"), ("OARD_WGRAD_T16", b"wgrad_t16"), ("OARD_WGRAD_QUEUE", b"wgrad_queue"), ("OARD_GATE_FOLD", b"gate_fold"), ("OARD_WGRAD_SHAPES", b"wgrad_shapes"), ("OARD_TRAIN_DUAL", b"train_dual"), ("OARD_SMALL_SPLIT", b"small_split"),
                      ("OARD_SKIP_FAMILIES", b"skip_families")):
         if os.environ.get(env) not in (None, ""):
diff --git a/oareactdiff_amd/build.py b/oareactdiff_amd/build.py
--- a/oareactdiff_amd/build.py
+++ b/oareactdiff_amd/build.py
@@ -14,6 +14,7 @@
     "oard_inst_gcl_v1.hip": _EDGE + ["oard_node_v1.h", "oard_edge_small.h"],
     "oard_inst_b3.hip": _EDGE + ["oard_edge_b3.h"],
     "oard_inst_equi.hip": _EDGE + ["oard_node_v1.h", "oard_edge_bwd.h"],
+    "oard_inst_pairs.hip": _EDGE,
     "oard_inst_wgrad.hip": _EDGE + ["oard_edge_bwd.h", "oard_wgrad_t16.h"],
     "oard_inst_node.hip": _EDGE + ["oard_node_v1.h", "oard_edge_bwd.h", "oard_node_bwd.h", "oard_rows.h"],
 }
diff --git a/oareactdiff_amd/csrc/oard_edge_v1.h b/oareactdiff_amd/csrc/oard_edge_v1.h
--- a/oareactdiff_amd/csrc/oard_edge_v1.h
+++ b/oareactdiff_amd/csrc/oard_edge_v1.h
@@ -520,12 +520,14 @@
     static constexpr size_t LDS_BYTES = (size_t)2 * SLAB * 1024;
 };
 
-template <class D, int WAVES, bool TRAIN>
+template <class D, int WAVES, bool TRAIN, bool CRPRE = false>
 __global__ __launch_bounds__(WAVES * 64) void k_equi_edge_v1(TopoDev tp, const float* __restrict__ stream,
                                                              const float* __restrict__ dp0b,
                                                              const float* __restrict__ ew, const float* __restrict__ rbuf,
                                                              float* __restrict__ qbuf, float* __restrict__ zd1,
-                                                             float* __restrict__ cdbuf, ActList al, int skip_mid) {
+                                                             float* __restrict__ cdbuf, ActList al, int skip_mid,
+                                                             const float* __restrict__ crbuf) {
+    static_assert(!CRPRE || !TRAIN, "the training-mode forward forms rbf_proj itself");
     extern __shared__ __attribute__((aligned(16))) float smem[];
     using S = EquiStream<D>;
     constexpr int WB = D::WB, D1T = D::D1T, RB = D::RB, HT = D::HT, G1 = S::G1, G2 = S::G2;
@@ -540,7 +542,7 @@
         pf.begin(stream, smem, ph, ph * G1, G1);
     };
     auto pf_begin_t2 = [&](int ph, int slot) {
-        pf.begin(stream, smem, ph, S::C1 + slot * G2, slot < S::NG2 ? G2 : 0);
+        pf.begin(stream, smem, ph, S::C1 + slot * G2, slot < S::NG2 ? (CRPRE ? G2 - RB : G2) : 0);
     };
     auto next_slot = [&](int i) -> int { return i + ((skip && i % 3 == 0) ? 2 : 1); };
     auto hook = [&]() { pf.tick(); };
@@ -558,9 +560,14 @@
     f4 d1[D1T];
 #pragma unroll
     for (int t = 0; t < D1T; ++t) d1[t] = ld_vec(dp0b, t, lane);
-    f4 rb[RB];
-#pragma unroll
-    for (int b = 0; b < RB; ++b) rb[b] = ld_blk(rbuf, a, D::RP, b, lane);
+    f4 rb[CRPRE ? 1 : RB];
+    if constexpr (!CRPRE) {
+#pragma unroll
+        for (int b = 0; b < RB; ++b) rb[b] = ld_blk(rbuf, a, D::RP, b, lane);
+    }
+    const float* crrow = CRPRE ? crbuf + (size_t)tp.cr_row[a] * (size_t)(3 * D::HP) + 4 * g : nullptr;
+    auto slot_off = [&](int i) -> int { const int tt = i / 3; return (i - 3 * tt) * D::HP + 16 * tt; };
+    f4 crn = f4zero();
     f4 xn = ld_f4(erow);
     pf_begin(0);
     pf.flush();
@@ -571,6 +578,7 @@
         const f4 x = xn;
         if (b + 1 < WB) pf_begin(p + 1); else pf_begin_t2(p + 1, 0);
         if (b + 1 < WB) xn = ld_f4(erow + 16 * (b + 1));
+        else if (CRPRE) crn = ld_f4(crrow);
         chain_kouter<D1T>(SL(p), 0, x, d1, hook);
         pf.flush();
     }
@@ -594,13 +602,17 @@
         pf_begin_t2(p + 1, next_slot(i));
         const int tt = i / 3, th = i - 3 * tt;
         f4 cd, cr;
+        if (CRPRE) {
+            cr = crn;
+            if (next_slot(i) < S::NG2) crn = ld_f4(crrow + slot_off(next_slot(i)));
+        }
         if (decltype(rows4)::value) {
             cd = reduce_g(chain_tile4<D1T>(SL(p), 1, d1, A(p, 0), hook));
-            cr = reduce_g(chain_tile4<RB>(SL(p), 1 + D1T, rb, f4zero(), hook));
-            if (g != 0) { cd = f4zero(); cr = f4zero(); }
+            if constexpr (!CRPRE) cr = reduce_g(chain_tile4<RB>(SL(p), 1 + D1T, rb, f4zero(), hook));
+            if (g != 0) { cd = f4zero(); if (!CRPRE) cr = f4zero(); }
         } else {
             cd = chain_tile<D1T>(SL(p), 1, d1, A(p, 0), hook);
-            cr = chain_tile<RB>(SL(p), 1 + D1T, rb, f4zero(), hook);
+            if constexpr (!CRPRE) cr = chain_tile<RB>(SL(p), 1 + D1T, rb, f4zero(), hook);
         }
         pf.flush();
         pend = cd * cr;
@@ -613,6 +625,75 @@
     for (int i = N_FULL; i < S::NG2; i = next_slot(i)) t2_phase(i, std::true_type{});
     st_f4(qrow + pend_off, pend);
     if (TRAIN) st_f4(cdrow + pend_off, pendc);
+}
+
+template <class D>
+__global__ __launch_bounds__(512) void k_rbf_proj_pairs(TopoDev tp, const float* __restrict__ stream, const float* __restrict__ rbuf,
+                                                        const float* __restrict__ geo, float* __restrict__ crbuf, int all_rows,
+                                                        int skip_mid) {
+    extern __shared__ __attribute__((aligned(16))) float smem[];
+    using S = EquiStream<D>;
+    constexpr int WAVES = 8, RB = D::RB, HT = D::HT, SLAB = 3 * RB;
+    const int lane = threadIdx.x & 63, g = lane >> 4;
+    const int wave = __builtin_amdgcn_readfirstlane(threadIdx.x >> 6);
+    const unsigned lane_off = (unsigned)lane * 16u;
+    const long long k = ((long long)blockIdx.x * WAVES + wave) * 16 + (lane & 15);
+    const bool live = k < tp.NC;
+    const size_t pr = (size_t)(live ? k : tp.NC);
+    const size_t a = (size_t)tp.pair_rows[2 * pr];
+    const bool on = live && (all_rows != 0 || geo[a * GEO_STRIDE + 11] > 0.f);
+    if (!__syncthreads_or(on ? 1 : 0)) return;
+    const bool wave_on = __ballot(on) != 0ull;
+    f4 rb[RB];
+#pragma unroll
+    for (int b = 0; b < RB; ++b) rb[b] = ld_blk(rbuf, a, D::RP, b, lane);
+    const int nth = skip_mid != 0 ? 2 : 3;
+    int pj = 0, ptt = 0;
+    auto issue_one = [&]() {
+        if (pj < nth * RB) {
+            const int s = pj / RB, th = skip_mid != 0 ? 2 * s : s;
+            glds16u(stream + ((size_t)S::C1 + (size_t)(3 * ptt + th) * S::G2 + 1 + D::D1T + (pj - s * RB)) * 256, lane_off,
+                    smem + ((size_t)(ptt & 1) * SLAB + pj) * 256);
+            pj += WAVES;
+        }
+    };
+    auto pf_begin = [&](int tt) { ptt = tt; pj = tt < HT ? wave : nth * RB; };
+    auto pf_flush = [&]() { while (pj < nth * RB) issue_one(); };
+    auto SL = [&](int p) -> const float* { return smem + (size_t)(p & 1) * SLAB * 256 + lane * 4; };
+    pf_begin(0);
+    pf_flush();
+    float* crow = crbuf + pr * (size_t)(3 * D::HP) + 4 * g;
+    f4 pend[3] = {f4zero(), f4zero(), f4zero()};
+    auto phase = [&](int tt, auto rows4) {
+        phase_barrier();
+        if (tt > 0 && wave_on) {
+#pragma unroll
+            for (int s = 0; s < 3; ++s)
+                if (s < nth) st_f4(crow + (skip_mid != 0 ? 2 * s : s) * D::HP + 16 * (tt - 1), pend[s]);
+        }
+        pf_begin(tt + 1);
+        pf_flush();
+        if (wave_on) {
+#pragma unroll
+            for (int s = 0; s < 3; ++s)
+                if (s < nth) {
+                    if (decltype(rows4)::value) {
+                        pend[s] = reduce_g(chain_tile4<RB>(SL(tt), s * RB, rb, f4zero()));
+                        if (g != 0) pend[s] = f4zero();
+                    } else {
+                        pend[s] = chain_tile<RB>(SL(tt), s * RB, rb, f4zero());
+                    }
+                }
+        }
+    };
+    constexpr int N_FULL = S::ROWS4 ? HT - 1 : HT;
+    for (int tt = 0; tt < N_FULL; ++tt) phase(tt, std::false_type{});
+    for (int tt = N_FULL; tt < HT; ++tt) phase(tt, std::true_type{});
+    if (wave_on) {
+#pragma unroll
+        for (int s = 0; s < 3; ++s)
+            if (s < nth) st_f4(crow + (skip_mid != 0 ? 2 * s : s) * D::HP + 16 * (HT - 1), pend[s]);
+    }
 }
 
 template <class D>
diff --git a/oareactdiff_amd/csrc/oard_hip.hip b/oareactdiff_amd/csrc/oard_hip.hip
--- a/oareactdiff_amd/csrc/oard_hip.hip
+++ b/oareactdiff_amd/csrc/oard_hip.hip
@@ -67,6 +67,7 @@
 int g_npb = 0;
 int g_poison = 0;
 int g_gcl_msum_taken = 0;
+int g_pair_terms_taken = 0;
 int g_equi_l0_taken = 0;
 int g_parts = 0;
 int g_wgrad_shapes = 3;
@@ -299,6 +300,7 @@
     w.al_rows = take(A * 4); w.al_src = take(A * 4); w.al_pre = take(A * 4); w.al_cnt = take((size_t)cdiv((long long)td.A, 256) * 4 + 4); w.al_n = take(4);
     w.d1s = take((size_t)cdiv((long long)td.A, 128) * 8 * d.D1T * 1024);
     w.small_a = E <= (size_t)OARD_SMALL_MAX_EDGES ? take(A * d.D1P * 4) : 0;
+    w.crbuf = take(((size_t)td.NC + 1) * 3 * d.HP * 4);
     w.total = cur;
     return w;
 }
@@ -383,7 +385,8 @@
 }
 template <class D>
 int launch_equi_v1(const FwdPlan& plan, int l, const TopoDev& tp, const float* wb, const LayerOff& lo, const float* stream, const float* dp0b,
-                   const float* ew, const float* rbuf, float* qbuf, float* zd1, float* cd, hipStream_t st, float* d1s, float* small, ActList al) {
+                   const float* ew, const float* rbuf, float* qbuf, float* zd1, float* cd, hipStream_t st, float* d1s, float* small, ActList al,
+                   const float* geo, float* crbuf) {
     const long long tiles = cdiv(tp.A, 16);
     switch (plan.equi) {
         case EQ_TRAIN_B3:
@@ -392,7 +395,7 @@
             return OARD_OK;
         case EQ_TRAIN:
             LAUNCH_LDS(F_EQUI_EDGE, (k_equi_edge_v1<D, 8, true>), cdiv(tp.A, 16 * 8), 8 * 64, (EquiStream<D>::LDS_BYTES), st,
-                       tp, stream, dp0b, ew, rbuf, qbuf, zd1, cd, ActList{}, 0);
+                       tp, stream, dp0b, ew, rbuf, qbuf, zd1, cd, ActList{}, 0, (const float*)nullptr);
             return OARD_OK;
         case EQ_SMALL_SPLIT:
             LAUNCH_LDS(F_EQUI_EDGE, (k_equi_small_s1<D, 8>), tiles * cdiv(D::D1T, 8), 512, (size_t)D::WB * 1024, st, tp, wb, lo, ew, small);
@@ -408,11 +411,18 @@
             return OARD_OK;
         case EQ_W4:
             LAUNCH_LDS(F_EQUI_EDGE, (k_equi_edge_v1<D, 4, false>), cdiv(tp.A, 16 * 4), 4 * 64, (EquiStream<D>::LDS_BYTES), st,
-                       tp, stream, dp0b, ew, rbuf, qbuf, nullptr, nullptr, al, 0);
+                       tp, stream, dp0b, ew, rbuf, qbuf, nullptr, nullptr, al, 0, (const float*)nullptr);
             return OARD_OK;
         case EQ_W8:
+            if (plan.pair_terms) {
+                LAUNCH_LDS(F_EQUI_EDGE, (k_rbf_proj_pairs<D>), cdiv(tp.NC, 16 * 8), 8 * 64, (size_t)2 * 3 * D::RB * 1024, st,
+                           tp, stream, rbuf, geo, crbuf, al.rows == nullptr ? 1 : 0, plan.l0_skip && l == 0 ? 1 : 0);
+                LAUNCH_LDS(F_EQUI_EDGE, (k_equi_edge_v1<D, 8, false, true>), cdiv(tp.A, 16 * 8), 8 * 64, (EquiStream<D>::LDS_BYTES), st,
+                           tp, stream, dp0b, ew, rbuf, qbuf, nullptr, nullptr, al, plan.l0_skip && l == 0 ? 1 : 0, (const float*)crbuf);
+                return OARD_OK;
+            }
             LAUNCH_LDS(F_EQUI_EDGE, (k_equi_edge_v1<D, 8, false>), cdiv(tp.A, 16 * 8), 8 * 64, (EquiStream<D>::LDS_BYTES), st,
-                       tp, stream, dp0b, ew, rbuf, qbuf, nullptr, nullptr, al, plan.l0_skip && l == 0 ? 1 : 0);
+                       tp, stream, dp0b, ew, rbuf, qbuf, nullptr, nullptr, al, plan.l0_skip && l == 0 ? 1 : 0, (const float*)nullptr);
             return OARD_OK;
         default: return OARD_EINVAL;
     }
@@ -498,11 +508,14 @@
     if (A > 0) {
         LAUNCH(F_INIT, k_edge_geo, cdiv(A, 256), 256, st, tp, (const float*)pos, (const double*)pf64, cutoff, geo, d64, use_al ? al_cnt : nullptr);
         if (use_al) LAUNCH(F_INIT, k_active_list, cdiv(A, 256), 256, st, tp, (const float*)geo, (const int*)al_cnt, (int*)al.rows, (int*)al.src, (int*)al.pre, (int*)al.n);
-        LAUNCH(F_INIT, k_rbf, cdiv(A * D::RP, 256), 256, st, tp, (const double*)d64, (const float*)geo,
-               wb + po.rbf_means, wb + po.rbf_betas, cutoff, rbuf, ew, D::R, D::RP, D::H, D::WP);
+        if (plan.pair_terms) LAUNCH(F_INIT, k_rbf_pairs, cdiv(tp.NC * D::RP, 256), 256, st, tp, (const double*)d64, (const float*)geo,
+                                    wb + po.rbf_means, wb + po.rbf_betas, cutoff, rbuf, ew, D::R, D::RP, D::H, D::WP);
+        else LAUNCH(F_INIT, k_rbf, cdiv(A * D::RP, 256), 256, st, tp, (const double*)d64, (const float*)geo,
+                    wb + po.rbf_means, wb + po.rbf_betas, cutoff, rbuf, ew, D::R, D::RP, D::H, D::WP);
     }
     LAUNCH(F_INIT, (k_node_embed<D>), gN, 256, st, tp, wb, po, (const float*)hin, zemb, nb);
-    if (A > 0) LAUNCH(F_INIT, (k_radial_lin<D>), gA, 256, st, tp, wb, po, (const float*)rbuf, (const float*)geo, ew);
+    if (A > 0 && plan.pair_terms) LAUNCH(F_INIT, (k_radial_lin_pairs<D>), cdiv(tp.NC, 64), 256, st, tp, wb, po, (const float*)rbuf, (const float*)geo, ew);
+    else if (A > 0) LAUNCH(F_INIT, (k_radial_lin<D>), gA, 256, st, tp, wb, po, (const float*)rbuf, (const float*)geo, ew);
     constexpr int NW = D::HT <= 16 ? D::HT : 8;
     const unsigned gNb = (unsigned)cdiv(N, tp.npb);
     if (plan.init_v1) {
@@ -519,6 +532,7 @@
     float* vec2 = (float*)(ws + w.vec2);
     float* vcur = vec;
     float* vnext = vec2;
+    g_pair_terms_taken = plan.pair_terms;
     g_gcl_msum_taken = msum;
     for (int l = 0; l < c->num_layers; ++l) {
         const LayerOff lo = po.layer[l];
@@ -557,7 +571,7 @@
             if (A > 0) {
                 rc = launch_equi_v1<D>(plan, l, tp, wb, lo, wb + lo.equi_stream, wb + lo.dp0b, ew_out, rbuf, vmsg,
                                        train ? (float*)(tape + to.zd1[l]) : nullptr, train ? (float*)(tape + to.cd[l]) : nullptr, st,
-                                       (float*)(ws + w.d1s), (float*)(ws + w.small_a), al);
+                                       (float*)(ws + w.d1s), (float*)(ws + w.small_a), al, (const float*)geo, (float*)(ws + w.crbuf));
                 if (rc != OARD_OK) return rc;
             }
 #define EQUI_NODE_V1(D_, ROWS_, XC_) LAUNCH(F_NODE, (k_equi_node_v1<D_, NW, ROWS_, XC_>), gN16, NW * 64, st, tp, wb, lo, (const float*)vmsg, \
@@ -1096,6 +1110,21 @@
         }
         act_ptr[N] = (int)a;
     }
+    const long long NC = A / 2;
+    std::vector<int> pair_rows((size_t)(NC + 1) * 2, (int)A), cr_row((size_t)A + 1, (int)NC);
+    {
+        size_t k = 0;
+        for (long long a = 0; a < A; ++a) {
+            const int m = act_src[a], n = act_tgt[a];
+            if (m > n) continue;
+            const int g0 = grp_ptr[node_sample[n] * n_obj + node_obj[n]];
+            const int partner = act_ptr[m] + (n - g0) - 1;
+            pair_rows[2 * k] = (int)a; pair_rows[2 * k + 1] = partner;
+            cr_row[a] = cr_row[partner] = (int)k;
+            ++k;
+        }
+        if ((long long)k != NC) return OARD_EINVAL;
+    }
     std::vector<int> edge_row((size_t)std::max<long long>(E, 1), -1), row_src((size_t)E + 1, 0), row_tgt((size_t)E + 1, 0),
         row_eid((size_t)E + 1, (int)E);
     {
@@ -1155,7 +1184,8 @@
                  o_aedge = add(act_edge.data(), act_edge.size() * 4), o_rptr = add(ref_edge_ptr.data(), N * 8),
                  o_erow = add(edge_row.data(), edge_row.size() * 4), o_rsrc = add(row_src.data(), row_src.size() * 4),
                  o_rtgt = add(row_tgt.data(), row_tgt.size() * 4), o_reid = add(row_eid.data(), row_eid.size() * 4),
-                 o_crow = add(col_info.data(), col_info.size() * 4), o_ncol = add(node_cols.data(), node_cols.size() * 4);
+                 o_crow = add(col_info.data(), col_info.size() * 4), o_ncol = add(node_cols.data(), node_cols.size() * 4),
+                 o_prow = add(pair_rows.data(), pair_rows.size() * 4), o_crr = add(cr_row.data(), cr_row.size() * 4);
     size_t cap = 0;
     char* dev = (char*)pool_alloc(cur, &cap);
     if (!dev) return OARD_EHIP;
@@ -1173,6 +1203,7 @@
     d.edge_row = (const int*)(dev + o_erow); d.row_src = (const int*)(dev + o_rsrc); d.row_tgt = (const int*)(dev + o_rtgt);
     d.row_eid = (const int*)(dev + o_reid);
     d.CI = CI; d.CX = CX; d.col_info = (const int*)(dev + o_crow); d.node_cols = (const int*)(dev + o_ncol);
+    d.NC = NC; d.pair_rows = (const int*)(dev + o_prow); d.cr_row = (const int*)(dev + o_crr);
     return OARD_OK;
 }
 
@@ -2126,13 +2157,14 @@
         {"gcl_variant", &g_fwd.gcl_variant}, {"equi_variant", &g_fwd.equi_variant}, {"node_variant", &g_fwd.node_variant},
         {"auto_small", &g_fwd.auto_small}, {"auto_tiny", &g_fwd.auto_tiny}, {"small_split", &g_fwd.small_split},
         {"gcl_persist", &g_fwd.gcl_persist}, {"gcl_grid", &g_fwd.gcl_grid}, {"gcl_skip", &g_fwd.gcl_skip}, {"equi_skip", &g_fwd.equi_skip},
-        {"equi_l0_skip", &g_fwd.equi_l0_skip}, {"gcl_msum", &g_fwd.gcl_msum},
+        {"equi_l0_skip", &g_fwd.equi_l0_skip}, {"gcl_msum", &g_fwd.gcl_msum}, {"pair_terms", &g_fwd.pair_terms},
         {"skip_families", &g_skip_families}, {"parts", &g_parts}, {"sequential", &g_sequential}, {"poison", &g_poison}, {"npb", &g_npb},
         {"wgrad_wgs", &g_wgrad_wgs}, {"wgrad_t16", &g_wgrad_t16}, {"wgrad_queue", &g_wgrad_queue}, {"gate_fold", &g_gate_fold},
         {"wgrad_lds", &g_wgrad_lds}, {"wgrad_shapes", &g_wgrad_shapes}, {"train_dual", &g_train_dual}};
     if (strcmp(name, "experiments") == 0) return kV0 ? OARD_OK : OARD_EINVAL;
     if (strcmp(name, "gcl_msum_taken") == 0) return g_gcl_msum_taken ? OARD_OK : OARD_EINVAL;
     if (strcmp(name, "equi_l0_taken") == 0) return g_equi_l0_taken ? OARD_OK : OARD_EINVAL;
+    if (strcmp(name, "pair_terms_taken") == 0) return g_pair_terms_taken ? OARD_OK : OARD_EINVAL;
     for (const auto& e : table) {
         if (strcmp(name, e.name) != 0) continue;
         if (!kV0 && value == 0 && strstr(name, "_variant")) return OARD_EINVAL;
diff --git a/oareactdiff_amd/csrc/oard_inst.h b/oareactdiff_amd/csrc/oard_inst.h
--- a/oareactdiff_amd/csrc/oard_inst.h
+++ b/oareactdiff_amd/csrc/oard_inst.h
@@ -43,17 +43,23 @@
 #endif
 
 #if !defined(OARD_INST_DEFINE) || defined(OARD_INST_UNIT_EQUI)
-#define OARD_A_EQUI (TopoDev, const float*, const float*, const float*, const float*, float*, float*, float*, ActList, int)
+#define OARD_A_EQUI (TopoDev, const float*, const float*, const float*, const float*, float*, float*, float*, ActList, int, const float*)
 #define OARD_A_EQUI_NODE (TopoDev, const float*, LayerOff, const float*, const float*, const float*, const float*, const float*, float*, const float*, float*, float*, float*, ActList)
 #define X(h, r) \
     OARD_INST((k_equi_edge_v1<Dims<h, r>, 8, false>), OARD_A_EQUI) OARD_INST((k_equi_edge_v1<Dims<h, r>, 8, true>), OARD_A_EQUI) \
-    OARD_INST((k_equi_edge_v1<Dims<h, r>, 4, false>), OARD_A_EQUI) \
+    OARD_INST((k_equi_edge_v1<Dims<h, r>, 4, false>), OARD_A_EQUI) OARD_INST((k_equi_edge_v1<Dims<h, r>, 8, false, true>), OARD_A_EQUI) \
     OARD_INST((k_equi_node_v1<Dims<h, r>, OARD_NW(h), false, false>), OARD_A_EQUI_NODE) OARD_INST((k_equi_node_v1<Dims<h, r>, OARD_NW(h), false, true>), OARD_A_EQUI_NODE) \
     OARD_INST((k_equi_node_v1<Dims<h, r>, OARD_NW(h), true, false>), OARD_A_EQUI_NODE) OARD_INST((k_equi_node_v1<Dims<h, r>, OARD_NW(h), true, true>), OARD_A_EQUI_NODE) \
     OARD_INST((k_equi_node_v1<Layer0<Dims<h, r> >, OARD_NW(h), false, false>), OARD_A_EQUI_NODE) OARD_INST((k_equi_node_v1<Layer0<Dims<h, r> >, OARD_NW(h), false, true>), OARD_A_EQUI_NODE) \
     OARD_INST((k_gcl_edge_bwd<Dims<h, r>, 8, 2, true>), (TopoDev, const float*, long long, long long, GclBwdArgs)) \
     OARD_INST((k_gcl_edge_bwd<Dims<h, r>, 8, 2, false>), (TopoDev, const float*, long long, long long, GclBwdArgs)) \
     OARD_INST((k_equi_edge_bwd<Dims<h, r>, 8>), (TopoDev, const float*, const float*, const float*, float*, float*))
+OARD_DIMS_LIST
+#undef X
+#endif
+
+#if !defined(OARD_INST_DEFINE) || defined(OARD_INST_UNIT_PAIRS)
+#define X(h, r) OARD_INST((k_rbf_proj_pairs<Dims<h, r> >), (TopoDev, const float*, const float*, const float*, float*, int, int))
 OARD_DIMS_LIST
 #undef X
 #endif
diff --git a/oareactdiff_amd/csrc/oard_inst_pairs.hip b/oareactdiff_amd/csrc/oard_inst_pairs.hip
--- /dev/null
+++ b/oareactdiff_amd/csrc/oard_inst_pairs.hip
@@ -0,0 +1,5 @@
+#define OARD_INST_TU
+#define OARD_INST_DEFINE
+#define OARD_INST_UNIT_PAIRS
+#include "oard_edge_v1.h"
+#include "oard_inst.h"
diff --git a/oareactdiff_amd/csrc/oard_kernels.h b/oareactdiff_amd/csrc/oard_kernels.h
--- a/oareactdiff_amd/csrc/oard_kernels.h
+++ b/oareactdiff_amd/csrc/oard_kernels.h
@@ -521,6 +521,30 @@
     rbuf[i] = v;
 }
 
+OARD_KERNEL __global__ void k_rbf_pairs(TopoDev tp, const double* __restrict__ d64, const float* __restrict__ geo,
+                            const float* __restrict__ means, const float* __restrict__ betas, double cutoff,
+                            float* __restrict__ rbuf, float* __restrict__ ew, int R, int RP, int H, int WP) {
+    const long long i = (long long)blockIdx.x * blockDim.x + threadIdx.x;
+    if (i >= tp.NC * RP) return;
+    const long long pr = i / RP;
+    const int k = (int)(i % RP);
+    const size_t a = (size_t)tp.pair_rows[2 * pr], b = (size_t)tp.pair_rows[2 * pr + 1];
+    float v = 0.f;
+    if (k < R) {
+        const double d = d64[a], m = (double)geo[a * GEO_STRIDE + 11];
+        double rb = 0.5 * (cos(d * M_PI / cutoff) + 1.0);
+        rb = d < cutoff ? rb : 0.0;
+        const double q = exp(-d) - (double)means[k];
+        v = (float)(rb * exp(-(double)betas[k] * q * q) * m);
+        ew[a * WP + 3 * H + k] = v;
+        ew[b * WP + 3 * H + k] = v;
+        if (k == 0)
+            for (int c = 3 * H + R; c < WP; ++c) { ew[a * WP + c] = 0.f; ew[b * WP + c] = 0.f; }
+    }
+    rbuf[a * RP + k] = v;
+    rbuf[b * RP + k] = v;
+}
+
 OARD_KERNEL __global__ void k_fill_edges(const float* __restrict__ c0, float* __restrict__ ew, long long E, int WP) {
     const int per = WP / 4;
     const long long total = E * per;
@@ -565,6 +589,29 @@
     for (int t = 0; t < D::HT; ++t) {
         f4 f = dense_tile<D::HT>(wb + po.rl2, t, h1, id.lane, ld_vec(wb + po.rl2_b, t, id.lane));
         if (id.valid && 16 * t + 4 * id.g < D::H) st_f4(ew + row + 16 * t + 4 * id.g, f * env);
+    }
+}
+
+template <class D>
+__global__ __launch_bounds__(256) void k_radial_lin_pairs(TopoDev tp, const float* __restrict__ wb, PackOff po,
+                                                          const float* __restrict__ rbuf, const float* __restrict__ geo,
+                                                          float* __restrict__ ew) {
+    bool live; const ColId id = col_id(tp.NC, live);
+    if (!live) return;
+    const size_t a = (size_t)tp.pair_rows[2 * id.c], b = (size_t)tp.pair_rows[2 * id.c + 1];
+    f4 rb[D::RB];
+#pragma unroll
+    for (int t = 0; t < D::RB; ++t) rb[t] = ld_blk(rbuf, a, D::RP, t, id.lane);
+    f4 h1[D::HT];
+    dense_regs<D::RB, D::HT, true, true>(wb + po.rl0, wb + po.rl0_b, rb, h1, id.lane);
+    const float env = geo[a * GEO_STRIDE + 1];
+#pragma unroll
+    for (int t = 0; t < D::HT; ++t) {
+        f4 f = dense_tile<D::HT>(wb + po.rl2, t, h1, id.lane, ld_vec(wb + po.rl2_b, t, id.lane));
+        if (id.valid && 16 * t + 4 * id.g < D::H) {
+            st_f4(ew + a * D::WP + 2 * D::H + 16 * t + 4 * id.g, f * env);
+            st_f4(ew + b * D::WP + 2 * D::H + 16 * t + 4 * id.g, f * env);
+        }
     }
 }
 
diff --git a/oareactdiff_amd/csrc/oard_layout.h b/oareactdiff_amd/csrc/oard_layout.h
--- a/oareactdiff_amd/csrc/oard_layout.h
+++ b/oareactdiff_amd/csrc/oard_layout.h
@@ -71,6 +71,9 @@
     long long CI, CX;
     const int *col_info;
     const int *node_cols;
+    long long NC;
+    const int *pair_rows;
+    const int *cr_row;
 };
 
 struct ActList {
@@ -120,4 +123,5 @@
     size_t al_rows, al_src, al_pre, al_cnt, al_n;
     size_t d1s;
     size_t small_a;
+    size_t crbuf;
 };
diff --git a/oareactdiff_amd/csrc/oard_plan.h b/oareactdiff_amd/csrc/oard_plan.h
--- a/oareactdiff_amd/csrc/oard_plan.h
+++ b/oareactdiff_amd/csrc/oard_plan.h
@@ -15,6 +15,7 @@
     int equi_skip = 1;
     int equi_l0_skip = 1;
     int gcl_msum = 1;
+    int pair_terms = 1;
 };
 
 enum GclShape {
@@ -50,6 +51,7 @@
     bool use_al;
     NodeForm node;
     bool l0_skip;
+    bool pair_terms;
     const GclLayer& gcl_at(int l) const { return gcl[(l == 0 ? 1 : 0) | (l == num_layers - 1 ? 2 : 0)]; }
 };
 
@@ -105,6 +107,7 @@
     p.equi = plan_equi_shape(in);
     p.use_al = !in.train && o.equi_skip && in.A > 0 && nv1;
     p.l0_skip = !in.train && o.equi_l0_skip && in.A > 0 && p.node == NODE_LARGE && p.equi == EQ_W8;
+    p.pair_terms = !in.train && o.pair_terms && in.A > 0 && p.equi == EQ_W8;
     auto throughput = [&](long long n) { const GclShape s = plan_gcl_shape(in, n); return n == 0 || s == GCL_PERSIST || s == GCL_RING3; };
     p.msum = !in.train && o.gcl_msum && in.E > 0 && o.gcl_variant == 2 && p.node == NODE_LARGE && throughput(in.CI) && throughput(in.CX);
     const long long inner = p.msum ? in.CI : in.A, all = p.msum ? in.CI + in.CX : in.E;
```

Result: no change. 3732 reaction-steps/s, median of 6 (+0.8%).
